# baurst/liso

Hardware: AMD Instinct MI355X
Metric: LISO train-step frames/sec (120k-pt clouds) (higher is better)
Workload: dtype bf16 (detector, BASELINE configs[2]) + f32 via bf16x3 MFMA (SLIM); north_star's 1e-3 on logits / flow is met by `parity_leg` (f32 via bf16x3 MFMA everywhere) and `fp32_exact_leg`, not by the bf16 detector

## Files before the change

include/liso_pillars.h:

```cpp
#ifndef LISO_PILLARS_H
#define LISO_PILLARS_H

#include <stddef.h>
#include <stdint.h>

#ifdef __cplusplus
extern "C" {
#endif

#define LISO_PFN_OUT 64
#define LISO_PILLARS_MAX_BATCH 32
#define LISO_PFN_STATS_DOUBLES 80

typedef struct {
    float x_min, y_min, z_min;
    float vx, vy, vz;
    int gx, gy;
    int max_points;
    int max_voxels;
    int n_channels;
} liso_pillar_cfg;

size_t liso_pillars_voxelize_workspace_bytes(const liso_pillar_cfg* cfg, int batch, int n_total);

int liso_pillars_voxelize_f32(const float* points, const int* offsets_host, int batch, const liso_pillar_cfg* cfg,
                              int* coors, int* num_points, int* slots, int* num_voxels, int* cell_to_voxel,
                              void* workspace, size_t workspace_bytes, void* stream);

size_t liso_pfn_decorate_workspace_bytes(int batch, int max_voxels);
int liso_pfn_decorate_f32(const float* points, const liso_pillar_cfg* cfg, int batch, const int* coors, const int* num_points,
                          const int* slots, const int* num_voxels, int* pt_off, float* feat, int* voxel_cell, void* workspace,
                          size_t workspace_bytes, void* stream);

size_t liso_pfn_partials_bytes(void);
int liso_pfn_bn_prepare_f32(const float* feat, const int* pt_off, const liso_pillar_cfg* cfg, int batch, const int* num_voxels,
                            const float* weight, const float* gamma, const float* beta, float* running_mean,
                            float* running_var, float momentum, float eps, int training, float* bn_out, double* moments,
                            void* partials, void* stream);

int liso_pfn_forward_scatter(const float* feat, const int* pt_off, const int* voxel_cell, const liso_pillar_cfg* cfg, int batch,
                             const int* cell_to_voxel, const float* weight, const float* bn_out, void* canvas, int out_bf16,
                             float* occupancy, void* stream);

int liso_pfn_forward_rows(const float* feat, const int* pt_off, const int* voxel_cell, const liso_pillar_cfg* cfg, int batch,
                          const int* cell_to_voxel, const float* weight, const float* bn_out, void* rows, int out_bf16, int row_base,
                          int* cell_to_row, float* occupancy, void* stream);

int liso_pfn_backward(const float* feat, const int* pt_off, const int* voxel_cell, const liso_pillar_cfg* cfg, int batch,
                      const int* num_voxels, const float* weight, const float* gamma, const float* bn_out,
                      const double* moments, int training, const void* grad_canvas, int grad_bf16, float* grad_weight,
                      float* grad_gamma, float* grad_beta, void* partials, void* stream);

#ifdef __cplusplus
}
#endif
#endif
```

liso_amd/_lib.py:

```python
import ctypes
import os

import torch

_HERE = os.path.dirname(os.path.abspath(__file__))
LIB_PATH = os.path.join(_HERE, "libliso_hip.so")

_lib = None


class LisoHipError(RuntimeError):
    pass


_ERRORS = {-1: "LISO_EINVAL (bad pointer/size)", -2: "LISO_EWORKSPACE (workspace too small)",
           -3: "LISO_ELAUNCH (HIP launch failed)", -4: "LISO_GROUND_ELENGTH (int(67 / delta_R) > 255)"}


def _preload_torch_hip_runtime():
    tl = os.path.join(os.path.dirname(torch.__file__), "lib", "libamdhip64.so")
    if os.path.exists(tl):
        ctypes.CDLL(tl, mode=ctypes.RTLD_GLOBAL)


def lib():
    global _lib
    if _lib is None:
        if not os.path.exists(LIB_PATH):
            raise LisoHipError(
                f"{LIB_PATH} not found: build it with `python -c 'import __graft_entry__ as g; g.build()'` "
                "or `make -C liso_amd/csrc`.  liso_amd has no CPU fallback for device ops.")
        _preload_torch_hip_runtime()
        _lib = ctypes.CDLL(LIB_PATH)
        _declare(_lib)
    return _lib


def check(code, what):
    if code != 0:
        raise LisoHipError(f"{what} failed: {_ERRORS.get(code, code)}")


def stream_ptr(device=None):
    return ctypes.c_void_p(torch.cuda.current_stream(device).cuda_stream)


def ptr(t):
    return ctypes.c_void_p(t.data_ptr())


def multi_copy(pairs):
    import torch

    fast = []
    for d, s_ in pairs:
        if (d.is_cuda and s_.is_cuda and d.device == s_.device and d.dtype == s_.dtype and d.shape == s_.shape and d.is_contiguous()
                and s_.is_contiguous() and (not fast or fast[0][0].device == d.device)):
            if d.numel() and d.data_ptr() != s_.data_ptr():
                fast.append((d, s_))
        else:
            d.copy_(s_, non_blocking=True)
    if len(fast) == 1:
        fast[0][0].copy_(fast[0][1], non_blocking=True)
    elif fast:
        n = len(fast)
        dst = (ctypes.c_void_p * n)(*[d.data_ptr() for d, _ in fast])
        src = (ctypes.c_void_p * n)(*[s_.data_ptr() for _, s_ in fast])
        nb = (ctypes.c_size_t * n)(*[d.numel() * d.element_size() for d, _ in fast])
        with torch.cuda.device(fast[0][0].device):
            check(lib().liso_multi_copy(n, dst, src, nb, stream_ptr()), "multi_copy")


def copy_blocks(jobs):
    import torch

    n = len(jobs)
    if n == 0:
        return
    dst = (ctypes.c_void_p * n)()
    src = (ctypes.c_void_p * n)()
    rows = (ctypes.c_uint * n)()
    rb = (ctypes.c_uint * n)()
    ds = (ctypes.c_size_t * n)()
    ss = (ctypes.c_size_t * n)()

    def rows_view(t):
        assert t.dtype == torch.float32 and t.is_cuda
        if t.dim() == 1:
            assert t.stride(0) == 1 or t.numel() <= 1
            return 1, t.numel(), t.numel()
        inner = 1
        for k in range(t.dim() - 1, 0, -1):
            assert t.shape[k] == 1 or t.stride(k) == inner, (tuple(t.shape), t.stride())
            inner *= t.shape[k]
        return t.shape[0], inner, (t.stride(0) if t.shape[0] > 1 else inner)

    for i, (d, s_) in enumerate(jobs):
        assert tuple(d.shape) == tuple(s_.shape), (tuple(d.shape), tuple(s_.shape))
        r, c, dstr = rows_view(d)
        r2, c2, sstr = rows_view(s_)
        assert (r, c) == (r2, c2)
        dst[i], src[i], rows[i], rb[i], ds[i], ss[i] = d.data_ptr(), s_.data_ptr(), r, 4 * c, 4 * dstr, 4 * sstr
    with torch.cuda.device(jobs[0][0].device):
        check(lib().liso_multi_copy_rows(n, dst, src, rows, rb, ds, ss, stream_ptr()), "multi_copy_rows")


def require_cuda(*tensors):
    for t in tensors:
        if not t.is_cuda:
            raise LisoHipError("device op called with a CPU tensor; liso_amd has no CPU fallback")


_vp, _i, _f, _sz, _lg = ctypes.c_void_p, ctypes.c_int, ctypes.c_float, ctypes.c_size_t, ctypes.c_long
_d = ctypes.c_double

SIGNATURES = {
    "liso_iou3d_overlap_bev_f32": (_i, [_vp, _i, _vp, _i, _vp, _vp]),
    "liso_iou3d_iou_bev_f32": (_i, [_vp, _i, _vp, _i, _vp, _vp]),
    "liso_iou3d_nms_workspace_bytes": (_sz, [_i]),
    "liso_iou3d_nms_f32": (_i, [_vp, _i, _f, _vp, _vp, _vp, _sz, _vp]),
    "liso_iou3d_nms_normal_f32": (_i, [_vp, _i, _f, _vp, _vp, _vp, _sz, _vp]),
    "liso_iou3d_iou_bev_cpu_f32": (_i, [_vp, _i, _vp, _i, _vp]),
    "liso_pillars_voxelize_workspace_bytes": (_sz, [_vp, _i, _i]),
    "liso_pillars_voxelize_f32": (_i, [_vp, _vp, _i, _vp, _vp, _vp, _vp, _vp, _vp, _vp, _sz, _vp]),
    "liso_pfn_partials_bytes": (_sz, []),
    "liso_pfn_decorate_workspace_bytes": (_sz, [_i, _i]),
    "liso_pfn_decorate_f32": (_i, [_vp, _vp, _i, _vp, _vp, _vp, _vp, _vp, _vp, _vp, _vp, _sz, _vp]),
    "liso_pfn_bn_prepare_f32": (_i, [_vp, _vp, _vp, _i, _vp, _vp, _vp, _vp, _vp, _vp, _f, _f, _i, _vp, _vp, _vp, _vp]),
    "liso_pfn_forward_scatter": (_i, [_vp, _vp, _vp, _vp, _i, _vp, _vp, _vp, _vp, _i, _vp, _vp]),
    "liso_pfn_forward_rows": (_i, [_vp, _vp, _vp, _vp, _i, _vp, _vp, _vp, _vp, _i, _i, _vp, _vp, _vp]),
    "liso_pfn_backward": (_i, [_vp, _vp, _vp, _vp, _i, _vp, _vp, _vp, _vp, _vp, _i, _vp, _i, _vp, _vp, _vp, _vp, _vp]),
    "liso_kabsch_workspace_bytes": (_sz, [_vp]),
    "liso_kabsch_trafos_f32": (_i, [_vp, _vp, _vp, _vp, _vp, _vp, _vp, _vp, _vp, _vp, _vp, _sz, _vp]),
    "liso_kabsch_trafos_counted_f32": (_i, [_vp, _vp, _vp, _vp, _vp, _vp, _vp, _vp, _vp, _vp, _vp, _vp, _sz, _vp]),
    "liso_symm_ortho_fwd_f64": (_i, [_vp, _i, _vp, _vp, _vp, _vp, _vp]),
    "liso_symm_ortho_bwd_f64": (_i, [_vp, _vp, _vp, _vp, _i, _vp, _vp]),
    "liso_weighted_moments_workspace_bytes": (_sz, [_i]),
    "liso_weighted_moments_fwd_f32": (_i, [_vp, _vp, _vp, _i, ctypes.c_long, _vp, _vp, _sz, _vp]),
    "liso_weighted_moments_bwd_f32": (_i, [_vp, _vp, _vp, _i, ctypes.c_long, _vp, _vp, _vp, _vp, _vp]),
    "liso_bev_dynamic_flow_workspace_bytes": (_sz, [_i, _i, _i]),
    "liso_bev_dynamic_flow_f32": (_i, [_vp, _i, _vp, _vp, _vp, _i, _vp, _i, _i, _i, _i, _vp, _vp, _vp, _sz, _vp]),
    "liso_odom_inverse_minus_eye_f64": (_i, [_vp, _i, _vp, _vp]),
    "liso_fit_box_z_workspace_bytes": (_sz, [_i, _i]),
    "liso_fit_box_z_f32": (_i, [_vp, _i, _i, _vp, _i, _vp, _i, _vp, _i, _f, _vp, _vp, _vp, _vp, _sz, _vp]),
    "liso_dbscan_components": (_i, [_vp, _vp, _vp, _vp, _vp, _vp, _vp, _vp, _vp]),
    "liso_dbscan_labels": (_i, [_vp, _vp, _vp, _vp, _vp, _vp, _vp, _vp, _vp, _vp]),
    "liso_region_props": (_i, [_vp, _i, _i, _i, _i, _vp, _vp, _vp]),
    "liso_region_props_workspace_bytes": (_sz, [_i, _i, _i, _i]),
    "liso_region_props_ws": (_i, [_vp, _i, _i, _i, _i, _vp, _vp, _vp, _sz, _vp]),
    "liso_corr_lookup_fwd_f32": (_i, [_vp, _vp, _vp, _vp, _vp, _vp]),
    "liso_corr_lookup_fwd_tiled_f32": (_i, [_vp, _vp, _vp, _vp, _vp, _vp]),
    "liso_corr_lookup_bwd_dvol_f32": (_i, [_vp, _vp, _vp, _vp, _vp]),
    "liso_corr_pyramid_fwd_f32": (_i, [_vp, _vp, _vp, _vp]),
    "liso_corr_pyramid_bwd_f32": (_i, [_vp, _vp, _vp, _vp]),
    "liso_corr_bwd_features_workspace_bytes": (_sz, [_vp]),
    "liso_corr_bwd_features_f32": (_i, [_vp, _i, _vp, _vp, _vp, _vp, _vp, _vp, _sz, _vp]),
    "liso_rows_combine_f32": (_i, [_lg, _i, _vp, _lg, _vp, _lg, _vp, _lg, _vp, _lg, _vp, _lg, _i, _vp]),
    "liso_gru_out_rows_train_f32": (_i, [_lg, _i, _vp, _lg, _vp, _vp, _lg, _vp, _lg, _vp]),
    "liso_gru_out_rows_bwd_f32": (_i, [_lg, _i, _vp, _lg, _vp, _vp, _lg, _vp, _lg, _vp, _lg, _vp, _vp, _vp]),
    "liso_gru_in_rows_bwd_f32": (_i, [_lg, _i, _vp, _lg, _vp, _lg, _vp, _vp, _vp, _lg, _vp, _lg, _vp, _vp]),
    "liso_raft_state_step_train_f32": (_i, [_i, _i, _vp, _vp, _vp, _vp, _vp, _vp, _vp, _vp, _vp]),
    "liso_raft_pack_output_grads_f32": (_i, [_lg, _i, _vp, _vp, _vp, _vp]),
    "liso_nearest_point_loss_fwd_f32": (_i, [_vp] * 8),
    "liso_nearest_point_loss_bwd_f32": (_i, [_vp] * 9),
    "liso_slim_decode_weights_fwd": (_i, [_vp] * 6 + [_i] + [_vp] * 4),
    "liso_slim_decode_weights_bwd": (_i, [_vp] * 9),
    "liso_slim_decode_points_fwd": (_i, [_vp] * 9),
    "liso_slim_decode_points_bwd": (_i, [_vp] * 11),
    "liso_slim_loss_workspace_bytes": (_sz, []),
    "liso_slim_static_points_loss_fwd": (_i, [_i, ctypes.c_long, _vp, _i, _vp, _vp, _vp, _vp, _vp, _vp, _sz, _vp]),
    "liso_slim_static_points_loss_bwd": (_i, [_i, ctypes.c_long, _vp, _i, _vp, _vp, _vp, _vp, _vp, _vp, _vp, _vp, _vp]),
    "liso_slim_knn_queries": (_i, [_i, _i, ctypes.c_long, _i, _vp, _i, _vp, _vp, _vp, _vp, _vp]),
    "liso_slim_nearest_point_loss_fwd": (_i, [_vp, _vp, _i, _vp, _vp, _vp, _i, _vp, _vp, _vp, _vp, _vp, _sz, _vp]),
    "liso_slim_nearest_point_loss_bwd": (_i, [_vp, _vp, _i, _vp, _vp, _vp, _i, _vp, _vp, _vp, _vp, _vp, _vp, _vp]),
    "liso_bev_gather_fwd_f32": (_i, [_vp, _vp, ctypes.c_long, _i, ctypes.c_float, _vp, _vp]),
    "liso_bev_gather_bwd_f32": (_i, [_vp, _vp, _vp, _vp, ctypes.c_long, _i, _vp, _vp, _vp]),
    "liso_gru_in_fwd_f32": (_i, [_vp, _vp, _vp, ctypes.c_long, _vp, _vp, _vp, _vp, _vp]),
    "liso_gru_in_bwd_f32": (_i, [_vp, _vp, ctypes.c_long, _vp, _vp, _vp, _vp, _vp, _vp, ctypes.c_long, _vp, _vp]),
    "liso_gru_out_fwd_f32": (_i, [ctypes.c_long, _vp, _vp, _vp, _vp, _vp]),
    "liso_gru_out_bwd_f32": (_i, [ctypes.c_long, _vp, _vp, _vp, _vp, _vp, _vp, _vp, _vp]),
    "liso_gru_in_rows_f32": (_i, [ctypes.c_long, _i, _vp, ctypes.c_long, _vp, ctypes.c_long, _vp, _vp, ctypes.c_long, _vp]),
    "liso_gru_out_rows_f32": (_i, [ctypes.c_long, _i, _vp, ctypes.c_long, _vp, _vp, ctypes.c_long, _vp]),
    "liso_multi_copy": (_i, [_i, _vp, _vp, _vp, _vp]),
    "liso_bev_lin_index": (_i, [_vp, _i, _vp, _i, ctypes.c_long, _i, _i, _vp, _vp]),
    "liso_channel_extrema_workspace_bytes": (_sz, []),
    "liso_channel_extrema_f32": (_i, [_vp, ctypes.c_long, _i, _i, _vp, _vp, _sz, _vp]),
    "liso_bev_plan_tile_lin": (_i, [_vp, _i, ctypes.c_long, _i, _i, _i, _i, _vp, _vp]),
    "liso_bev_plan_rank": (_i, [_vp, _vp, ctypes.c_long, _vp, _vp, _vp]),
    "liso_bev_plan_expand": (_i, [_vp, _vp, _vp, _i, ctypes.c_long, _i, _i, _i, _i, _vp, _vp, _vp, _vp]),
    "liso_raft_state_step_f32": (_i, [_i, _i, _vp, ctypes.c_long, _vp, _vp, _vp, _vp]),
    "liso_raft_upsample_scratch_bytes": (_sz, [_vp]),
    "liso_raft_upsample_outputs_fwd_f32": (_i, [_vp] * 5),
    "liso_raft_upsample_outputs_bwd_f32": (_i, [_vp, _vp, _vp, _sz, _vp, _vp, _vp]),
    "liso_centerloss_workspace_bytes": (_sz, [_vp]),
    "liso_centerloss_fwd_f32": (_i, [_vp] * 17 + [_sz, _vp]),
    "liso_centerloss_bwd_f32": (_i, [_vp] * 21),
    "liso_render_center_targets_f32": (_i, [_vp] * 12),
    "liso_conv_pack_weights_batched": (_i, [_vp, _i, _vp]),
    "liso_conv_pack_weights_placed": (_i, [_vp, _i, _i, _vp]),
    "liso_conv_in_finalize": (_i, [_vp, _i, _i, _i, _i, ctypes.c_long, _vp, _vp, _f, _vp, _vp]),
    "liso_residual_affine_relu_f32": (_i, [_vp, _vp, _vp, _i, _i, _vp, _vp, _vp, _i, _i, _vp, _i, ctypes.c_long, _i, _vp]),
    "liso_scan_workspace_bytes": (_sz, [_i, ctypes.c_long]),
    "liso_scan_inclusive_i32": (_i, [_vp, _i, ctypes.c_long, _vp, _vp, _sz, _vp]),
    "liso_mine_boxes_from_regions": (_i, [_vp, _i, _i, _vp, _i, _vp, _i, _f, _f, _vp, _vp, _vp, _vp, _vp, _vp]),
    "liso_mine_filter_compact": (_i, [_vp] * 21),
    "liso_mine_box_motion": (_i, [_vp, _i, _i, _vp, _vp, _vp, _vp]),
    "liso_mine_nms_workspace_bytes": (_sz, [_i, _i]),
    "liso_mine_nms_prepare": (_i, [_i, _i, _i] + [_vp] * 11 + [_sz, _vp]),
    "liso_mine_nms_finish": (_i, [_i, _i, _i] + [_vp] * 16),
    "liso_adamw_step_f32": (_i, [_vp, _vp, _vp, _vp, _sz] + [ctypes.c_double] * 5 + [ctypes.c_long, _vp]),
    "liso_adamw_step_scaled_f32": (_i, [_vp, _vp, _vp, _vp, _sz] + [ctypes.c_double] * 6 + [ctypes.c_long, _vp]),
    "liso_adamw_pack_table_plan": (_i, [_vp, _i, _sz, _vp, _vp]),
    "liso_adamw_pack_table_fill": (_i, [_vp, _i, _sz, _vp, _sz]),
    "liso_adamw_step_packed_f32": (_i, [_vp, _vp, _vp, _vp, _sz] + [ctypes.c_double] * 6 + [ctypes.c_long, _vp, _i, _vp]),
    "liso_grad_nonfinite_f32": (_i, [_vp, _sz, _vp, _vp]),
    "liso_adamw_step_amp_f32": (_i, [_vp, _vp, _vp, _vp, _sz] + [ctypes.c_double] * 6 + [_vp, _vp]),
    "liso_loss_scale_update": (_i, [_vp, ctypes.c_double, ctypes.c_double, _i, _vp]),
    "liso_rmsprop_step_f32": (_i, [_vp, _vp, _vp, _sz] + [ctypes.c_double] * 4 + [_vp]),
    "liso_multi_copy_rows": (_i, [_i, _vp, _vp, _vp, _vp, _vp, _vp, _vp]),
    "liso_gather_f32": (_i, [_i, _vp, _vp, _vp, _vp]),
    "liso_bn_workspace_bytes": (_sz, [_i]),
    "liso_bn_relu_fwd": (_i, [_vp, _i, ctypes.c_long, _i, _vp, _vp, _vp, _vp, _f, _f, _i, _i, _vp, _vp, _vp, _sz, _vp]),
    "liso_in_workspace_bytes": (_sz, [_i, _i]),
    "liso_in_relu_fwd": (_i, [_vp, _i, _i, ctypes.c_long, _i, _vp, _vp, _f, _i, _vp, _vp, _vp, _sz, _vp]),
    "liso_in_relu_bwd": (_i, [_vp, _vp, _i, _i, ctypes.c_long, _i, _vp, _vp, _i, _vp, _vp, _vp, _vp, _sz, _vp]),
    "liso_in_relu_bwd_sum": (_i, [_vp, _vp, _i, _i, ctypes.c_long, _i, _vp, _vp, _i, _vp, _vp, _vp, _vp, _sz, _vp]),
    "liso_bn_relu_bwd": (_i, [_vp, _vp, _i, ctypes.c_long, _i, _vp, _vp, _i, _i, _vp, _vp, _vp, _vp, _sz, _vp]),
    "liso_bn_relu_bwd_strided": (_i, [_vp, ctypes.c_long, _vp, ctypes.c_long, _i, ctypes.c_long, _i, _vp, _vp, _i, _i, _vp, ctypes.c_long, _vp, _vp, _vp, _sz, _vp]),
    "liso_bn_relu_bwd_chained": (_i, [_vp, ctypes.c_long, _vp, ctypes.c_long, _i, ctypes.c_long, _i, _vp, _vp, _i, _i, _vp, ctypes.c_long, _vp, _vp, _vp, _sz, _vp, _vp]),
    "liso_bn_multi_workspace_bytes": (_sz, [_vp, _i, _i]),
    "liso_bn_relu_bwd_multi": (_i, [_vp, ctypes.c_long, _vp, ctypes.c_long, _vp, ctypes.c_long, _i, ctypes.c_long, _vp, _i, _i, _i, _vp, ctypes.c_long,
                                    _vp, _sz, _vp, _vp, _vp]),
    "liso_bn_relu_bwd_multi_check": (_i, [_vp, _i, _i, _i, ctypes.c_long, ctypes.c_long, ctypes.c_long, ctypes.c_long, ctypes.c_long, _vp]),
    "liso_knn_workspace_bytes": (_sz, [_vp, _i]),
    "liso_knn_build_f32": (_i, [_vp, _vp, _i, _i, _vp, _sz, _vp]),
    "liso_knn_sorted_ids": (_i, [_vp, _vp, _i, _vp, _vp]),
    "liso_knn_query_f32": (_i, [_vp, _vp, _vp, _vp, _i, _vp, _i, _i, _vp, _vp, _i, _vp]),
    "liso_conv_packed_bytes": (_sz, [_i, _i, _i, _i]),
    "liso_conv_pack_weights": (_i, [_vp, _i, _i, _i, _i, _i, _i, _i, _vp, _vp]),
    "liso_conv_stats_rows": (_i, [_vp]),
    "liso_conv_kernel_kind": (_i, [_vp]),
    "liso_conv_forward": (_i, [_vp] * 10),
    "liso_conv_set_option": (_i, [_i, _i]),
    "liso_conv_forward_sparse": (_i, [_vp] * 11),
    "liso_conv_plan_info": (_i, [_vp, _vp]),
    "liso_conv_wgrad_workspace_bytes": (_sz, [_vp]),
    "liso_conv_wgrad": (_i, [_vp, _vp, _vp, _vp, _vp, _i, _i, _vp, _vp, _vp, _sz, _vp]),
    "liso_conv_wgrad_deferred": (_i, [_vp, _vp, _vp, _vp, _vp, _i, _i, _vp, _vp, _vp, _sz, _vp, _vp]),
    "liso_conv_wgrad_reduce": (_i, [_vp, _vp]),
    "liso_conv_wgrad_sparse_workspace_bytes": (_sz, [_vp]),
    "liso_conv_wgrad_sparse_f32": (_i, [_vp, _vp, _vp, _vp, _i, _vp, _vp, _vp, _sz, _vp]),
    "liso_conv_wgrad_smallci_workspace_bytes": (_sz, [_i, _i, _i, _i, _i]),
    "liso_conv_wgrad_smallci_f32": (_i, [_vp, ctypes.c_long, _vp, ctypes.c_long, _i, _i, _i, _i, _i, _vp, _vp, _vp, _sz, _vp]),
    "liso_sparse_conv_stat_groups": (_i, [_i, _i, _i]),
    "liso_sparse_conv_workspace_bytes": (_sz, [_i, _i, _i, _i, _i, _i, _i]),
    "liso_sparse_conv_forward": (_i, [_vp, ctypes.c_long, _i, _vp, _vp, _vp, _i, _i, _i, _i, _i, _i, _i, _vp, _vp, _vp, _vp, _vp, _sz, _vp]),
    "liso_sparse_conv_forward_rows": (_i, [_vp, ctypes.c_long, _i, _vp, ctypes.c_long, _vp, _vp, _vp, _i, _i, _i, _i, _i, _i, _i, _vp, _vp, _vp, _vp, _vp,
                                           _sz, _vp]),
    "liso_sparse_conv_dgrad": (_i, [_vp, ctypes.c_long, _i, _vp, _vp, _i, _i, _i, _i, _i, _i, _vp, ctypes.c_long, _vp, _vp, _sz, _i, _vp]),
    "liso_sparse_stem_workspace_bytes": (_sz, [_i, _i, _i, _i]),
    "liso_sparse_stem_forward_f32": (_i, [_vp, ctypes.c_long, _vp, _vp, _vp, _i, _i, _i, _i, _i, _vp, _vp, _vp, _vp, _sz, _vp]),
    "liso_conv_bn_finalize": (_i, [_vp, _i, _i, _i, ctypes.c_long, _vp, _vp, _vp, _vp, _vp, _f, _f, _vp, _vp]),
    "liso_conv_bn_finalize_merged": (_i, [_vp, _i, _i, _i, ctypes.c_long, _vp, _vp, _vp, _vp, _vp, _f, _f, _vp, _vp, _vp, _i, _i, _vp]),
    "liso_points_in_boxes_workspace_bytes": (_sz, [_vp]),
    "liso_points_in_boxes_f32": (_i, [_vp] * 9 + [_sz, _vp]),
    "liso_match_greedy_f32": (_i, [_vp, ctypes.c_long, ctypes.c_long, _i, _i, _vp, _f, _vp, _vp, _vp, _vp, _vp, _vp, _vp]),
    "liso_fit_boxes_closeness_workspace_bytes": (_sz, [ctypes.c_long, _i]),
    "liso_fit_boxes_closeness_f32": (_i, [_vp, ctypes.c_long, _i, _vp, _vp, _i, _f, _vp, _vp, _vp, _sz, _vp]),
    "liso_bike_rollout_fwd_f32": (_i, [_i, _i, _vp, _vp, _vp, _vp, _f, _f, _f, _vp, _vp]),
    "liso_bike_rollout_bwd_f32": (_i, [_i, _i, _vp, _vp, _vp, _f, _f, _f, _vp, _vp, _vp, _vp, _vp, _vp]),
    "liso_smooth_tracks_jerk_f32": (_i, [_vp, _vp, _i, _i, _i, _f, _f, _vp, _vp]),
    "liso_flow_metrics_state_bytes": (_sz, []),
    "liso_flow_metrics_result_bytes": (_sz, []),
    "liso_flow_metrics_reset": (_i, [_vp, _vp]),
    "liso_flow_metrics_update": (_i, [_vp, _lg, _vp, _lg, _vp, _lg, _i, _vp, _lg, _vp, _lg, _vp, _lg, _vp, _vp, _vp, _vp, _i, _vp, _vp]),
    "liso_flow_metrics_read": (_i, [_vp, _vp, _vp]),
    "liso_det_nms_workspace_bytes": (_sz, [_i, _i]),
    "liso_det_nms_order": (_i, [_i, _i, _vp, _vp, _vp, _f, _vp, _vp, _vp, _sz, _vp]),
    "liso_det_nms_select": (_i, [_i, _i, _vp, _vp, _vp, _f, _i, _i, _vp, _vp, _vp]),
    "liso_det_nms_gather": (_i, [_i, _i, _i, _vp, _vp, _vp, _i, _vp]),
    "liso_ground_jcp_workspace_bytes": (_sz, [_vp]),
    "liso_ground_jcp_f32": (_i, [_vp, _vp, _vp, _vp, _vp, _sz, _vp]),
    "liso_ground_jcp_stages_f32": (_i, [_vp, _vp, _vp, _vp, _vp, _sz, _i, _i, _vp]),
    "liso_ground_cone_f32": (_i, [_i, _i, _i, _vp, _vp, ctypes.c_double, ctypes.c_double, _vp, _vp, _vp]),
    "liso_ground_compact_workspace_bytes": (_sz, [_i, _i]),
    "liso_ground_compact_f32": (_i, [_i, _i, _i, _vp, _vp, _vp, _vp, _vp, _vp, _sz, _vp]),
    "liso_bev_free_mask_workspace_bytes": (_sz, [_i, _i]),
    "liso_bev_free_mask": (_i, [_vp, ctypes.c_long, _i, _i, _i, _vp, _vp, _vp, _sz, _vp]),
    "liso_bev_select_free_cells": (_i, [_vp, _vp, _i, _i, _vp, _i, _vp, _vp]),
    "liso_snippet_paste": (_i, [_vp, ctypes.c_long, _vp, _vp, _vp, _vp, ctypes.c_double, ctypes.c_double, _i, _vp, _vp, _vp, _vp]),
    "liso_sample_transform_f32": (_i, [_i, _i, _i] + [_vp] * 7),
    "liso_sample_transform_poses_f64": (_i, [_i, _vp, _vp, _i, _vp, _i, _vp]),
    "liso_bev_crop_workspace_bytes": (_sz, [_i, _i]),
    "liso_bev_crop_f32": (_i, [_vp] * 14 + [_sz, _vp]),
    "liso_bev_point_maps_workspace_bytes": (_sz, [_i, _i, _i, _i]),
    "liso_bev_point_maps_f32": (_i, [_i] * 5 + [_vp] * 6 + [ctypes.c_double] + [_vp] * 5 + [_sz, _vp]),
    "liso_box_has_points_f32": (_i, [_i] * 4 + [_vp] * 7),
    "liso_filter_boxes": (_i, [_vp] * 6 + [_i] + [_vp] * 3),
    "liso_object_velocity_f64": (_i, [_i, _i] + [_vp] * 5),
    "liso_ignore_region_mask": (_i, [_i] * 4 + [ctypes.c_double] * 2 + [_vp] * 6),
    "liso_render_center_targets_ex_f32": (_i, [_vp] * 15),
    "liso_snippet_cut_workspace_bytes": (_sz, [_i, _i, _i]),
    "liso_snippet_cut_f32": (_i, [_i, _i, _i, _vp, _vp, _vp, _i, _vp, _vp, _lg] + [_vp] * 5 + [_sz, _vp]),
    "liso_track_sequences_workspace_bytes": (_sz, [_i, _i, _i, _i]),
    "liso_track_sequences": (_i, [_i] * 4 + [_vp] * 7 + [ctypes.c_double] + [_vp] * 10 + [_sz, _vp]),
    "liso_track_mining_workspace_bytes": (_sz, [_i] * 5),
    "liso_select_tracks": (_i, [_i] * 5 + [_vp] * 7 + [_i, _f, _d, _d, _i, _d, _d, _i, _d] + [_vp] * 13 + [_vp, _sz, _vp]),
    "liso_refine_tracks_apply": (_i, [_i] * 3 + [_vp] * 12 + [_i, _i, _d] + [_vp] * 7 + [_vp]),
    "liso_export_tracks": (_i, [_i] * 6 + [_vp] * 11 + [_i] + [_vp] * 13 + [_vp, _sz, _vp]),
    "liso_frame_prep_workspace_bytes": (_sz, [_vp]),
    "liso_prepare_tracker_frames": (_i, [_vp] * 27 + [_sz, _vp]),
}


CONV_MAX_TAPS, CONV_MAX_CLASSES, CONV_BF16, CONV_F32X3, CONV_F32, CONV_F16 = 49, 4, 0, 1, 2, 3
ELEM_F32, ELEM_BF16, ELEM_F16 = 0, 1, 2
_ELEM_CODES = {torch.float32: ELEM_F32, torch.bfloat16: ELEM_BF16, torch.float16: ELEM_F16}
LOSS_SCALE_STATE_BYTES = 32


def elem_code(dtype):
    code = _ELEM_CODES.get(dtype)
    if code is None:
        raise TypeError(f"no device kernel takes {dtype} tensors (float32, bfloat16 or float16)")
    return code


def is_half(dtype):
    return elem_code(dtype) != ELEM_F32


def lane_channels(dtype):
    return 8 if is_half(dtype) else 4
CONV_OPT_SHARED_GPU = 1
CONV_OPT_ROLES_CUS = 2


class ConvDesc(ctypes.Structure):
    _fields_ = [("batch", _i), ("hi", _i), ("wi", _i), ("ci", _i), ("x_pix_stride", _i), ("ho", _i), ("wo", _i), ("co", _i),
                ("y_pix_stride", _i), ("y_ch_off", _i), ("hv", _i), ("wv", _i), ("isy", _i), ("isx", _i), ("osy", _i), ("osx", _i),
                ("n_classes", _i), ("class_tap_begin", _i * (CONV_MAX_CLASSES + 1)), ("class_ooy", _i * CONV_MAX_CLASSES),
                ("class_oox", _i * CONV_MAX_CLASSES), ("n_taps", _i), ("tap_dy", _i * CONV_MAX_TAPS), ("tap_dx", _i * CONV_MAX_TAPS),
                ("tap_w", _i * CONV_MAX_TAPS), ("w_taps", _i), ("mode", _i), ("out_f32", _i), ("in_relu", _i), ("out_relu", _i),
                ("in_affine_batch_stride", _i), ("wgrad_co", _i)]


class ConvPackPlacedJob(ctypes.Structure):
    _fields_ = [("src", _vp), ("dst", _vp), ("d0", _i), ("d1", _i), ("kh", _i), ("kw", _i), ("transposed", _i), ("for_dgrad", _i),
                ("mode", _i), ("K", _i), ("N", _i), ("k_offset", _i), ("n_offset", _i)]


class AdamwPackDest(ctypes.Structure):
    _fields_ = [("dst", _vp), ("for_dgrad", _i), ("mode", _i), ("K", _i), ("N", _i), ("k_offset", _i), ("n_offset", _i)]


class AdamwPackItem(ctypes.Structure):
    _fields_ = [("offset", _sz), ("d0", _i), ("d1", _i), ("kh", _i), ("kw", _i), ("transposed", _i), ("n_dest", _i),
                ("dest", AdamwPackDest * 2), ("mirror", _vp), ("mirror_row_stride", _sz)]


class ConvPackJob(ctypes.Structure):
    _fields_ = [("src", _vp), ("dst", _vp), ("d0", _i), ("d1", _i), ("kh", _i), ("kw", _i), ("transposed", _i), ("for_dgrad", _i),
                ("mode", _i)]


class WgradReduceJob(ctypes.Structure):
    _fields_ = [("slab", _vp), ("bias_slab", _vp), ("dw", _vp), ("dbias", _vp), ("cip", ctypes.c_long), ("cop", ctypes.c_long),
                ("splits", _i), ("bias_rows", _i), ("taps", _i), ("ci", _i), ("co", _i), ("transposed", _i)]


BN_MAX_GROUPS = 4


class BnGroup(ctypes.Structure):
    _fields_ = [("c_off", _i), ("c", _i), ("gamma", _vp), ("stats", _vp), ("grad_gamma", _vp), ("grad_beta", _vp)]


class KnnGrid(ctypes.Structure):
    _fields_ = [("x_min", _f), ("y_min", _f), ("cell", _f), ("nx", _i), ("ny", _i), ("z_min", _f), ("z_cell", _f), ("nz", _i)]


class CenterLossCfg(ctypes.Structure):
    _fields_ = [("batch", _i), ("h", _i), ("w", _i), ("res_x", _f), ("res_y", _f), ("z_min", _f), ("z_max", _f),
                ("sup_weight", _f), ("rot_reg_weight", _f)]


class NpLossCfg(ctypes.Structure):
    _fields_ = [("batch", _i), ("n", ctypes.c_long), ("n_b", ctypes.c_long), ("ext", _f * 4), ("fov_mode", _i), ("delta", _f)]


class SlimDecodeCfg(ctypes.Structure):
    _fields_ = [("samples", _i), ("n", ctypes.c_long), ("h", _i), ("w", _i), ("logit_mode", _i * 4), ("static_flow_zero", _i),
                ("dynamic_flow_zero", _i), ("overwrite_flow", _i), ("overwrite_logits", _i), ("non_rigid", _i), ("use_static_aggr", _i),
                ("dyn_grad_scale", _f), ("ext_lo", ctypes.c_double * 2), ("ext_span", ctypes.c_double * 2)]


class SlimDecodeOut(ctypes.Structure):
    FIELDS = ("dis_logit", "dis", "logits", "probs", "staticness", "dynamicness", "groundness", "dyn_flow", "stat_flow", "agg_flow", "saf_flow")
    _fields_ = [(k, _vp) for k in FIELDS] + [("flags", _vp)]


class SlimNpLossCfg(ctypes.Structure):
    _fields_ = [("samples", _i), ("clouds", _i), ("n", ctypes.c_long), ("n_b", ctypes.c_long), ("ext", _f * 4), ("fov_mode", _i), ("delta", _f)]


class BoxPtsCfg(ctypes.Structure):
    _fields_ = [("batch", _i), ("n", ctypes.c_long), ("k", _i), ("point_stride", _i), ("precision", _i), ("dims_bloat", _f)]


class FramePrepCfg(ctypes.Structure):
    _fields_ = [("n_seq", _i), ("max_frames", _i), ("max_box", _i), ("cap", _i), ("n_points", ctypes.c_long), ("point_stride", _i),
                ("n_fov_points", ctypes.c_long), ("fov_stride", _i), ("bev_range_x", _f), ("bev_range_y", _f), ("drop_on_bev_boundaries", _i),
                ("min_points_in_box", _i), ("fov_min_points", _i), ("align", _i), ("no_align_below_m", _d), ("full_align_above_m", _d)]


class GruCfg(ctypes.Structure):
    _fields_ = [("batch", _i), ("ch", _i), ("cx", _i), ("hw", ctypes.c_long)]


class UpsampleCfg(ctypes.Structure):
    _fields_ = [("n_it", _i), ("batch2", _i), ("dirs", _i), ("h", _i), ("w", _i), ("factor", _i), ("flow_scale", _f)]


class MineFilterCfg(ctypes.Structure):
    _fields_ = [("batch", _i), ("k", _i), ("min_points", _i), ("aspect_ratio_max", ctypes.c_double), ("max_box_len_m", ctypes.c_double),
                ("min_box_area_m2", ctypes.c_double), ("min_box_volume_m3", ctypes.c_double), ("park_invalid", _i)]


class DetGatherField(ctypes.Structure):
    _fields_ = [("src", _vp), ("dst", _vp), ("row_elems", _i), ("elem_bytes", _i), ("pad_bits", ctypes.c_uint64)]


class GroundCfg(ctypes.Structure):
    _fields_ = [("batch", _i), ("n_max", _i), ("point_stride", _i), ("width", _i), ("height", _i),
# ... 93 lines not shown
```

liso_amd/csrc/pillars.hip:

```cpp
#include <hip/hip_runtime.h>
#include <stdlib.h>
#include "zero_fill.h"
#include <cstring>
#include <hip/hip_bf16.h>
#include <limits.h>
#include <stdint.h>

#include "../../include/liso_iou3d.h"
#include "../../include/liso_conv.h"
#include "../../include/liso_pillars.h"
#include "dev_common.h"

namespace {

using liso_dev::check_launch;

constexpr int kTile = 1024;
constexpr int kOut = LISO_PFN_OUT;
constexpr int kFP = 12;
constexpr int kMaxPts = 32;
constexpr int kPfnThreads = 256;
constexpr int kPfnGrid = 1024;

struct BatchInfo {
// ... 97 lines not shown
            coors[v * 4 + 1] = 0;
            coors[v * 4 + 2] = within / cfg.gy;
            coors[v * 4 + 3] = within % cfg.gy;
            const int c = count[cell];
            num_points[v] = c < cfg.max_points ? c : cfg.max_points;
        }
    }
    if (tile == bi.tile_off[b + 1] - 1 && threadIdx.x == 0) {
        int tot = base_s;
        for (int w = 0; w < kTile / 64; w++) tot += wsum[w];
        num_voxels[b] = tot < cfg.max_voxels ? tot : cfg.max_voxels;
    }
}

constexpr int kScanTile = 1024;
__global__ __launch_bounds__(kScanTile) void cell_scan_block_kernel(const int* __restrict__ count, size_t cells, int* __restrict__ seg_off,
                                                                    int* __restrict__ block_tot) {
    __shared__ int wsum[kScanTile / 64];
    const size_t i = (size_t)blockIdx.x * kScanTile + threadIdx.x;
    const int lane = threadIdx.x & 63, wave = threadIdx.x >> 6;
    const int v = i < cells ? count[i] : 0;
    int incl = v;
#pragma unroll
    for (int o = 1; o < 64; o <<= 1) {
        const int t = __shfl_up(incl, o);
        if (lane >= o) incl += t;
    }
    if (lane == 63) wsum[wave] = incl;
    __syncthreads();
    int base = 0;
    for (int w = 0; w < wave; w++) base += wsum[w];
    if (i < cells) seg_off[i] = base + incl - v;
    if (threadIdx.x == kScanTile - 1) block_tot[blockIdx.x] = base + incl;
}

__global__ __launch_bounds__(1024) void cell_scan_tot_kernel(int* __restrict__ block_tot, int nblk) {
    __shared__ int wsum[16];
    const int t = threadIdx.x, lane = t & 63, wave = t >> 6;
    int v[4], tot = 0;
#pragma unroll
    for (int k = 0; k < 4; k++) {
        const int q = t * 4 + k;
        v[k] = q < nblk ? block_tot[q] : 0;
        tot += v[k];
    }
    int incl = tot;
#pragma unroll
    for (int o = 1; o < 64; o <<= 1) {
        const int up = __shfl_up(incl, o);
        if (lane >= o) incl += up;
    }
    if (lane == 63) wsum[wave] = incl;
    __syncthreads();
    int base = 0;
    for (int w = 0; w < wave; w++) base += wsum[w];
    int run = base + incl - tot;
#pragma unroll
    for (int k = 0; k < 4; k++) {
        const int q = t * 4 + k;
        if (q < nblk) block_tot[q] = run;
        run += v[k];
    }
}

__global__ __launch_bounds__(256) void seg_fill_kernel(const int* __restrict__ cell_of_point, int n_total, const int* __restrict__ seg_off,
                                                       const int* __restrict__ block_tot, const int* __restrict__ pos_in_cell,
                                                       int* __restrict__ seg) {
    const int i = blockIdx.x * blockDim.x + threadIdx.x;
    if (i >= n_total) return;
    const int c = cell_of_point[i];
    if (c < 0) return;
    seg[seg_off[c] + block_tot[c / kScanTile] + pos_in_cell[i]] = i;
}

constexpr int kSlotRegs = 16;
__device__ __forceinline__ void voxel_slots_one(const int* __restrict__ coors, const int* __restrict__ num_voxels, int max_voxels, int gx, int gy,
                                                const int* __restrict__ seg_off, const int* __restrict__ block_tot,
                                                const int* __restrict__ count, const int* __restrict__ seg, int max_points,
                                                int* __restrict__ slots, long v, int lane) {
    const int b = (int)(v / max_voxels), ord = (int)(v % max_voxels);
    if (ord >= num_voxels[b]) return;
    const int c = (b * gx + coors[v * 4 + 2]) * gy + coors[v * 4 + 3];
    const int off = seg_off[c] + block_tot[c / kScanTile], n = count[c];
    int* out = slots + (size_t)v * max_points;
    if (n <= 64) {
        const int e = lane < n ? seg[off + lane] : 0x7fffffff;
        int r = 0;
        for (int k = 0; k < n; k++) r += __shfl(e, k) < e ? 1 : 0;
        if (lane < n && r < max_points) out[r] = e;
        return;
    }
    int last = -1;
    const int rounds = min(max_points, n);
    if (n <= 64 * kSlotRegs) {
        int x[kSlotRegs];
#pragma unroll
        for (int u = 0; u < kSlotRegs; u++) x[u] = lane + 64 * u < n ? seg[off + lane + 64 * u] : 0x7fffffff;
        for (int r = 0; r < rounds; r++) {
            int m = 0x7fffffff;
#pragma unroll
            for (int u = 0; u < kSlotRegs; u++) m = (x[u] > last && x[u] < m) ? x[u] : m;
#pragma unroll
            for (int o = 32; o > 0; o >>= 1) m = min(m, __shfl_xor(m, o));
            if (lane == 0) out[r] = m;
            last = m;
        }
        return;
    }
    for (int r = 0; r < rounds; r++) {
        int m = 0x7fffffff;
        for (int j = lane; j < n; j += 64) {
            const int x = seg[off + j];
            m = (x > last && x < m) ? x : m;
        }
#pragma unroll
        for (int o = 32; o > 0; o >>= 1) m = min(m, __shfl_xor(m, o));
        if (lane == 0) out[r] = m;
        last = m;
    }
}

__global__ __launch_bounds__(256) void voxel_slots_kernel(const int* __restrict__ coors, const int* __restrict__ num_voxels, int max_voxels,
                                                          int batch, int gx, int gy, const int* __restrict__ seg_off,
                                                          const int* __restrict__ block_tot, const int* __restrict__ count,
                                                          const int* __restrict__ seg, int max_points, int* __restrict__ slots) {
    const int lane = threadIdx.x & 63;
    for (long v = (long)blockIdx.x * 4 + (threadIdx.x >> 6); v < (long)batch * max_voxels; v += (long)gridDim.x * 4)
        voxel_slots_one(coors, num_voxels, max_voxels, gx, gy, seg_off, block_tot, count, seg, max_points, slots, v, lane);
}

struct PfnGeom {
    float vx, vy, x_off, y_off, z_off;
};

__device__ __forceinline__ PfnGeom pfn_geom(const liso_pillar_cfg& c) {
    PfnGeom g;
    g.vx = c.vx; g.vy = c.vy;
    g.x_off = c.vx / 2 + c.x_min;
    g.y_off = c.vy / 2 + c.y_min;
    g.z_off = c.vz / 2 + c.z_min;
    return g;
}

constexpr int kGroup = 4;
constexpr int kStage = kGroup * kMaxPts;

__device__ __forceinline__ int kept_points(const int* __restrict__ num_points, const int* __restrict__ num_voxels, int max_voxels,
                                           int rows, int v) {
    if (v >= rows) return 0;
    const int b = v / max_voxels;
    return (v - b * max_voxels) < num_voxels[b] ? num_points[v] : 0;
}

__global__ __launch_bounds__(1024) void pfn_scan_block_kernel(const int* __restrict__ num_points, const int* __restrict__ num_voxels,
                                                              int max_voxels, int rows, int* __restrict__ pt_off,
                                                              int* __restrict__ block_tot) {
    __shared__ int wsum[16];
    const int i = blockIdx.x * 1024 + threadIdx.x;
    const int lane = threadIdx.x & 63, wave = threadIdx.x >> 6;
    const int v = kept_points(num_points, num_voxels, max_voxels, rows, i);
    int incl = v;
    for (int off = 1; off < 64; off <<= 1) {
        const int t = __shfl_up(incl, off);
        if (lane >= off) incl += t;
    }
    if (lane == 63) wsum[wave] = incl;
    __syncthreads();
    int base = 0;
    for (int w = 0; w < wave; w++) base += wsum[w];
    if (i < rows) pt_off[i] = base + incl - v;
    if (threadIdx.x == 1023) block_tot[blockIdx.x] = base + incl;
}

__global__ __launch_bounds__(1024) void pfn_scan_tot_kernel(int* __restrict__ block_tot, int nblocks) {
    __shared__ int wsum[16];
    const int lane = threadIdx.x & 63, wave = threadIdx.x >> 6;
    const int v = (int)threadIdx.x < nblocks ? block_tot[threadIdx.x] : 0;
    int incl = v;
    for (int off = 1; off < 64; off <<= 1) {
        const int t = __shfl_up(incl, off);
        if (lane >= off) incl += t;
    }
    if (lane == 63) wsum[wave] = incl;
    __syncthreads();
    int base = 0;
    for (int w = 0; w < wave; w++) base += wsum[w];
    if ((int)threadIdx.x < nblocks) block_tot[threadIdx.x] = base + incl - v;
    if ((int)threadIdx.x == nblocks - 1) block_tot[nblocks] = base + incl;
}

__global__ __launch_bounds__(1024) void pfn_scan_add_kernel(int* __restrict__ pt_off, int rows, const int* __restrict__ block_tot,
                                                            int nblocks) {
    const int i = blockIdx.x * 1024 + threadIdx.x;
    if (i < rows) pt_off[i] += block_tot[blockIdx.x];
    if (i == 0) pt_off[rows] = block_tot[nblocks];
}

template <int C>
__global__ __launch_bounds__(256) void pfn_decorate_kernel(const float* __restrict__ pts, liso_pillar_cfg cfg, int rows,
                                                           const int* __restrict__ coors, const int* __restrict__ num_points,
                                                           const int* __restrict__ slots, const int* __restrict__ num_voxels,
                                                           const int* __restrict__ pt_off, float* __restrict__ feat,
                                                           int* __restrict__ voxel_cell) {
#pragma clang fp contract(off)
    constexpr int F = C + 6;
    const long t = (long)blockIdx.x * blockDim.x + threadIdx.x;
    const int v = (int)(t >> 5), s = (int)(t & 31);
    if (v >= rows) return;
    const int num = kept_points(num_points, num_voxels, cfg.max_voxels, rows, v);
    const int xi = coors[v * 4 + 2], yi = coors[v * 4 + 3];
    if (s == 0) voxel_cell[v] = num > 0 ? ((v / cfg.max_voxels) * cfg.gx + xi) * cfg.gy + yi : -1;
    float p[C];
#pragma unroll
    for (int k = 0; k < C; k++) p[k] = 0.f;
    if (s < num) {
        const int idx = slots[(size_t)v * cfg.max_points + s];
        const float* q = pts + (size_t)idx * C;
        if constexpr (C == 4) {
            const float4 tt = *reinterpret_cast<const float4*>(q);
            p[0] = tt.x; p[1] = tt.y; p[2] = tt.z; p[3] = tt.w;
        } else {
#pragma unroll
            for (int k = 0; k < C; k++) p[k] = q[k];
        }
    }
    float sx = p[0], sy = p[1], sz = p[2];
#pragma unroll
    for (int o = 16; o > 0; o >>= 1) {
        sx += __shfl_xor(sx, o);
        sy += __shfl_xor(sy, o);
        sz += __shfl_xor(sz, o);
    }
    if (s >= num) return;
    const PfnGeom g = pfn_geom(cfg);
    const float fn = (float)num;
    const float mx = sx / fn, my = sy / fn, mz = sz / fn;
    const float fcx = p[0] - ((float)yi * g.vx + g.x_off);
    const float fcy = p[1] - ((float)xi * g.vy + g.y_off);
    const float fcz = p[2] - (0.f + g.z_off);
    float f[kFP];
#pragma unroll
    for (int k = 0; k < kFP; k++) f[k] = 0.f;
    f[0] = fcx; f[1] = fcy; f[2] = fcz;
#pragma unroll
    for (int k = 3; k < C; k++) f[k] = p[k];
    f[C + 0] = p[0] - mx; f[C + 1] = p[1] - my; f[C + 2] = p[2] - mz;
    f[C + 3] = fcx; f[C + 4] = fcy; f[C + 5] = fcz;
    f[F] = 1.f;
    float4* row = reinterpret_cast<float4*>(feat + ((size_t)pt_off[v] + s) * kFP);
    row[0] = make_float4(f[0], f[1], f[2], f[3]);
    row[1] = make_float4(f[4], f[5], f[6], f[7]);
    row[2] = make_float4(f[8], f[9], f[10], f[11]);
}

template <int C>
__global__ __launch_bounds__(kPfnThreads) void pfn_stats_kernel(const float* __restrict__ feat, const int* __restrict__ pt_off,
                                                                int rows, double* __restrict__ partials) {
    constexpr int F = C + 6, D = F + 1, NP = D * (D + 1) / 2;
    __shared__ __attribute__((aligned(16))) float tile[kPfnThreads / 64][64][kFP];
    __shared__ double red[kPfnThreads / 64][LISO_PFN_STATS_DOUBLES];
    const int lane = threadIdx.x & 63, wave = threadIdx.x >> 6;
    int pj[2] = {0, 0}, pk[2] = {0, 0};
    {
        int idx = 0;
        for (int j = 0; j < D; j++)
            for (int k = j; k < D; k++, idx++) {
                if (idx == lane) { pj[0] = j; pk[0] = k; }
                if (idx == lane + 64) { pj[1] = j; pk[1] = k; }
            }
    }
    const long n = pt_off[rows];
    const long waves = (long)gridDim.x * (kPfnThreads / 64);
    const long per = ((n + waves - 1) / waves + 63) / 64 * 64;
    const long w_id = (long)blockIdx.x * (kPfnThreads / 64) + wave;
    const long r0 = w_id * per, r1 = r0 + per < n ? r0 + per : n;
    double acc0 = 0.0, acc1 = 0.0;
    for (long base = r0; base < r1; base += 64) {
        const int cnt = (int)(r1 - base < 64 ? r1 - base : 64);
        const float4* src = reinterpret_cast<const float4*>(feat + (size_t)base * kFP);
        float4* dst = reinterpret_cast<float4*>(&tile[wave][0][0]);
        for (int i = lane; i < cnt * 3; i += 64) dst[i] = src[i];
        __builtin_amdgcn_wave_barrier();
        for (int s = 0; s < cnt; s++) {
            const float* f = tile[wave][s];
            acc0 += (double)f[pj[0]] * (double)f[pk[0]];
            if (lane + 64 < NP) acc1 += (double)f[pj[1]] * (double)f[pk[1]];
        }
        __builtin_amdgcn_wave_barrier();
    }
    red[wave][lane] = acc0;
    if (lane + 64 < LISO_PFN_STATS_DOUBLES) red[wave][lane + 64] = lane + 64 < NP ? acc1 : 0.0;
    __syncthreads();
    if (threadIdx.x < LISO_PFN_STATS_DOUBLES) {
        double s = 0.0;
        for (int w = 0; w < kPfnThreads / 64; w++) s += red[w][threadIdx.x];
        partials[(size_t)blockIdx.x * LISO_PFN_STATS_DOUBLES + threadIdx.x] = threadIdx.x < NP ? s : 0.0;
    }
}

__device__ __forceinline__ int pair_index(int j, int k, int D) {
    return j * D - j * (j - 1) / 2 + (k - j);
}

template <int C>
__global__ __launch_bounds__(1024) void pfn_bn_finalize_kernel(const double* __restrict__ partials, int nblocks,
                                                               const int* __restrict__ num_voxels, int batch,
                                                               int max_points, const float* __restrict__ weight,
                                                               const float* __restrict__ gamma,
                                                               const float* __restrict__ beta,
                                                               float* __restrict__ running_mean,
                                                               float* __restrict__ running_var, float momentum,
                                                               float eps, float* __restrict__ bn_out,
                                                               double* __restrict__ moments) {
    constexpr int F = C + 6, D = F + 1;
    constexpr int NS = LISO_PFN_STATS_DOUBLES, CH = 1024 / NS;
    __shared__ double part[CH][NS];
    __shared__ double mom[NS];
    const int e = threadIdx.x % NS, chunk = threadIdx.x / NS;
    if (chunk < CH) {
        double s = 0.0;
        const int per = (nblocks + CH - 1) / CH;
        const int lo = chunk * per, hi = lo + per < nblocks ? lo + per : nblocks;
        int blk = lo;
        for (; blk + 16 <= hi; blk += 16) {
            double v[16];
#pragma unroll
            for (int j = 0; j < 16; j++) v[j] = partials[(size_t)(blk + j) * NS + e];
#pragma unroll
            for (int j = 0; j < 16; j++) s += v[j];
        }
        for (; blk < hi; blk++) s += partials[(size_t)blk * NS + e];
        part[chunk][e] = s;
    }
    __syncthreads();
    if (threadIdx.x < NS) {
        double t = 0.0;
        for (int c = 0; c < CH; c++) t += part[c][threadIdx.x];
        mom[threadIdx.x] = t;
        moments[threadIdx.x] = t;
    }
    __syncthreads();
    __shared__ double rows_sq[kOut][F + 1], rows_sum[kOut][F + 1];
    if (threadIdx.x < kOut * F) {
        const int c = threadIdx.x / F, j = threadIdx.x % F;
        const double wj = (double)weight[c * F + j];
        double q = 0.0;
        for (int k = 0; k < F; k++) {
            const int a = j <= k ? j : k, bb = j <= k ? k : j;
            q += wj * (double)weight[c * F + k] * mom[pair_index(a, bb, D)];
        }
        rows_sq[c][j] = q;
        rows_sum[c][j] = wj * mom[pair_index(j, D - 1, D)];
    }
    __syncthreads();
    if (threadIdx.x < kOut) {
        const int c = threadIdx.x;
        long long P = 0;
        for (int b = 0; b < batch; b++) P += num_voxels[b];
        const double M = (double)P * (double)max_points;
        double sum = 0.0, sq = 0.0;
        for (int j = 0; j < F; j++) {
            sum += rows_sum[c][j];
            sq += rows_sq[c][j];
        }
        double mean = 0.0, var = 0.0;
        if (M > 0.0) {
            mean = sum / M;
            var = sq / M - mean * mean;
            if (var < 0.0) var = 0.0;
        }
        const double invstd = 1.0 / sqrt(var + (double)eps);
        const float scale = (float)((double)gamma[c] * invstd);
        bn_out[c] = scale;
        bn_out[kOut + c] = (float)((double)beta[c] - mean * (double)gamma[c] * invstd);
        bn_out[2 * kOut + c] = (float)mean;
        bn_out[3 * kOut + c] = (float)invstd;
        if (M > 1.0) {
            const double mo = (double)momentum;
            running_mean[c] = (float)((1.0 - mo) * (double)running_mean[c] + mo * mean);
            running_var[c] = (float)((1.0 - mo) * (double)running_var[c] + mo * (var * M / (M - 1.0)));
        }
    }
}

__global__ void pfn_bn_eval_kernel(const float* __restrict__ gamma, const float* __restrict__ beta,
                                   const float* __restrict__ running_mean, const float* __restrict__ running_var,
                                   float eps, float* __restrict__ bn_out) {
    const int c = threadIdx.x;
    if (c >= kOut) return;
    const float invstd = 1.f / sqrtf(running_var[c] + eps);
    bn_out[c] = gamma[c] * invstd;
    bn_out[kOut + c] = beta[c] - running_mean[c] * gamma[c] * invstd;
    bn_out[2 * kOut + c] = running_mean[c];
    bn_out[3 * kOut + c] = invstd;
}

template <typename T> __device__ __forceinline__ void store_out(T* p, float v);
template <> __device__ __forceinline__ void store_out<float>(float* p, float v) { *p = v; }
template <> __device__ __forceinline__ void store_out<__hip_bfloat16>(__hip_bfloat16* p, float v) { *p = __float2bfloat16(v); }
template <typename T> __device__ __forceinline__ float load_in(const T* p);
template <> __device__ __forceinline__ float load_in<float>(const float* p) { return *p; }
template <> __device__ __forceinline__ float load_in<__hip_bfloat16>(const __hip_bfloat16* p) { return __bfloat162float(*p); }
template <> __device__ __forceinline__ void store_out<_Float16>(_Float16* p, float v) { *p = (_Float16)v; }
template <> __device__ __forceinline__ float load_in<_Float16>(const _Float16* p) { return (float)*p; }

__device__ __forceinline__ void stage_rows(const float* __restrict__ feat, const int* __restrict__ pt_off, int rows, int v0, int lane,
                                           float (*frow)[kFP], int (&off)[kGroup + 1]) {
    int o = 0;
    if (lane <= kGroup) { const int v = v0 + lane; o = pt_off[v < rows ? v : rows]; }
#pragma unroll
    for (int g = 0; g <= kGroup; g++) off[g] = __shfl(o, g);
    const int total = off[kGroup] - off[0];
    const float4* src = reinterpret_cast<const float4*>(feat + (size_t)off[0] * kFP);
    float4* dst = reinterpret_cast<float4*>(&frow[0][0]);
    for (int i = lane; i < total * 3; i += 64) dst[i] = src[i];
}

constexpr int kCellsPerBlock = 256;

template <int C, typename OutT, bool ROWS>
__global__ __launch_bounds__(kPfnThreads) void pfn_forward_kernel(const float* __restrict__ feat, const int* __restrict__ pt_off,
                                                                  const int* __restrict__ voxel_cell, int rows, int max_points,
                                                                  long total_cells, int zero_blocks,
                                                                  const int* __restrict__ cell_to_voxel,
                                                                  const float* __restrict__ weight, const float* __restrict__ bn,
                                                                  OutT* __restrict__ canvas, float* __restrict__ occupancy,
                                                                  int* __restrict__ map_out, int row_base) {
    constexpr int F = C + 6;
    constexpr int kChunks = kOut * (int)sizeof(OutT) / 16;
    __shared__ __attribute__((aligned(16))) float frow[kPfnThreads / 64][kStage][kFP];
    __shared__ int vox[kCellsPerBlock];
    const int tid = threadIdx.x, lane = tid & 63, wave = tid >> 6;
    const int pillar_blocks = (int)gridDim.x - zero_blocks;
    if ((int)blockIdx.x >= pillar_blocks) {
        const long cell0 = (long)((int)blockIdx.x - pillar_blocks) * kCellsPerBlock;
        const long cell = cell0 + tid;
        int v1 = 0;
        if (cell < total_cells) {
            v1 = cell_to_voxel[cell];
            occupancy[cell] = v1 > 0 ? 1.f : 0.f;
            if constexpr (ROWS) map_out[cell] = v1 > 0 ? v1 + row_base : 0;
        }
        if constexpr (ROWS) return;
        vox[tid] = v1;
        __syncthreads();
        const uint4 z = make_uint4(0u, 0u, 0u, 0u);
        uint4* base = reinterpret_cast<uint4*>(canvas + (size_t)cell0 * kOut);
        for (int id = tid; id < kCellsPerBlock * kChunks; id += kPfnThreads) {
            const int cl = id / kChunks;
            if (cell0 + cl < total_cells && vox[cl] == 0) base[id] = z;
        }
        return;
    }
    float w[F];
#pragma unroll
    for (int k = 0; k < F; k++) w[k] = weight[lane * F + k];
    const float scale = bn[lane], shift = bn[kOut + lane];
    const float pad_val = fmaxf(shift, 0.f);
    const int wave_id = (int)blockIdx.x * (kPfnThreads / 64) + wave;
    const int n_waves = pillar_blocks * (kPfnThreads / 64);
    for (int v0 = wave_id * kGroup; v0 < rows; v0 += n_waves * kGroup) {
        int off[kGroup + 1];
        stage_rows(feat, pt_off, rows, v0, lane, frow[wave], off);
        int cell_l = -1;
        if (lane < kGroup && v0 + lane < rows) cell_l = voxel_cell[v0 + lane];
        __builtin_amdgcn_wave_barrier();
#pragma unroll
        for (int g = 0; g < kGroup; g++) {
            const int num = off[g + 1] - off[g];
            const int cell = __shfl(cell_l, g);
            if (num <= 0 || cell < 0) continue;
            float best = num < max_points ? pad_val : 0.f;
            const int r0 = off[g] - off[0];
            for (int s = 0; s < num; s++) {
                const float4* f4 = reinterpret_cast<const float4*>(frow[wave][r0 + s]);
                const float4 a = f4[0], b = f4[1], c4 = f4[2];
                const float f[kFP] = {a.x, a.y, a.z, a.w, b.x, b.y, b.z, b.w, c4.x, c4.y, c4.z, c4.w};
                float x = 0.f;
#pragma unroll
                for (int k = 0; k < F; k++) x = fmaf(w[k], f[k], x);
                best = fmaxf(best, fmaxf(fmaf(x, scale, shift), 0.f));
            }
            store_out<OutT>(canvas + (size_t)(ROWS ? v0 + g : cell) * kOut + lane, best);
        }
        __builtin_amdgcn_wave_barrier();
    }
}

template <int C, typename GT>
__global__ __launch_bounds__(kPfnThreads) void pfn_backward_kernel(const float* __restrict__ feat, const int* __restrict__ pt_off,
                                                                   const int* __restrict__ voxel_cell, int rows, int max_points,
                                                                   const float* __restrict__ weight, const float* __restrict__ bn,
                                                                   const GT* __restrict__ grad_canvas,
                                                                   float* __restrict__ partials) {
    constexpr int F = C + 6, NA = F + 2;
    __shared__ __attribute__((aligned(16))) float frow[kPfnThreads / 64][kStage][kFP];
    __shared__ float red[kPfnThreads / 64][NA][kOut];
    const int lane = threadIdx.x & 63, wave = threadIdx.x >> 6;
    float w[F], acc[NA];
#pragma unroll
    for (int k = 0; k < F; k++) w[k] = weight[lane * F + k];
#pragma unroll
    for (int k = 0; k < NA; k++) acc[k] = 0.f;
    const float scale = bn[lane], shift = bn[kOut + lane], mean = bn[2 * kOut + lane], invstd = bn[3 * kOut + lane];
    const float pad_val = fmaxf(shift, 0.f);
    const int wave_id = (int)blockIdx.x * (kPfnThreads / 64) + wave;
    const int n_waves = (int)gridDim.x * (kPfnThreads / 64);
    for (int v0 = wave_id * kGroup; v0 < rows; v0 += n_waves * kGroup) {
        int off[kGroup + 1];
        stage_rows(feat, pt_off, rows, v0, lane, frow[wave], off);
        int cell_l = -1;
        if (lane < kGroup && v0 + lane < rows) cell_l = voxel_cell[v0 + lane];
        __builtin_amdgcn_wave_barrier();
#pragma unroll
        for (int g = 0; g < kGroup; g++) {
            const int num = off[g + 1] - off[g];
            const int cell = __shfl(cell_l, g);
            if (num <= 0 || cell < 0) continue;
            const int r0 = off[g] - off[0];
            float best = -1.f, best_x = 0.f;
            int best_s = -1;
            for (int s = 0; s < num; s++) {
                const float* f = frow[wave][r0 + s];
                float x = 0.f;
#pragma unroll
                for (int k = 0; k < F; k++) x = fmaf(w[k], f[k], x);
                const float y = fmaxf(fmaf(x, scale, shift), 0.f);
                if (y > best) { best = y; best_s = s; best_x = x; }
            }
            if (num < max_points && pad_val > best) { best = pad_val; best_s = -1; best_x = 0.f; }
            const float gy = load_in<GT>(grad_canvas + (size_t)cell * kOut + lane);
            const float dz = best > 0.f ? gy : 0.f;
            if (best_s >= 0) {
                const float* f = frow[wave][r0 + best_s];
#pragma unroll
                for (int k = 0; k < F; k++) acc[k] = fmaf(dz, f[k], acc[k]);
            }
            acc[F] += dz;
            acc[F + 1] = fmaf(dz, (best_x - mean) * invstd, acc[F + 1]);
        }
        __builtin_amdgcn_wave_barrier();
    }
#pragma unroll
    for (int k = 0; k < NA; k++) red[wave][k][lane] = acc[k];
    __syncthreads();
    for (int idx = threadIdx.x; idx < NA * kOut; idx += kPfnThreads) {
        const int k = idx / kOut, c = idx % kOut;
        float s = 0.f;
        for (int wv = 0; wv < kPfnThreads / 64; wv++) s += red[wv][k][c];
        partials[((size_t)blockIdx.x * NA + k) * kOut + c] = s;
    }
}

template <int NA>
__global__ __launch_bounds__(1024) void pfn_backward_reduce_kernel(const float* __restrict__ partials, int nblocks,
                                                                   double* __restrict__ tot) {
    __shared__ double part[16][kOut];
    const int k = blockIdx.x, c = threadIdx.x & 63, chunk = threadIdx.x >> 6;
    const int per = (nblocks + 15) / 16;
    const int lo = chunk * per, hi = lo + per < nblocks ? lo + per : nblocks;
    double s = 0.0;
    {
        int blk = lo;
        for (; blk + 8 <= hi; blk += 8) {
            float v[8];
#pragma unroll
            for (int j = 0; j < 8; j++) v[j] = partials[((size_t)(blk + j) * NA + k) * kOut + c];
#pragma unroll
            for (int j = 0; j < 8; j++) s += (double)v[j];
        }
        for (; blk < hi; blk++) s += (double)partials[((size_t)blk * NA + k) * kOut + c];
    }
    part[chunk][c] = s;
    __syncthreads();
    if (chunk == 0) {
        double t = 0.0;
        for (int q = 0; q < 16; q++) t += part[q][c];
        tot[k * kOut + c] = t;
    }
}

template <int C>
__global__ __launch_bounds__(64) void pfn_backward_finalize_kernel(const double* __restrict__ tot,
                                                                   const int* __restrict__ num_voxels, int batch,
                                                                   int max_points, const float* __restrict__ weight,
                                                                   const float* __restrict__ gamma,
                                                                   const float* __restrict__ bn,
                                                                   const double* __restrict__ moments, int training,
                                                                   float* __restrict__ grad_weight,
                                                                   float* __restrict__ grad_gamma,
                                                                   float* __restrict__ grad_beta) {
    constexpr int F = C + 6, D = F + 1;
    const int c = threadIdx.x;
    if (c >= kOut) return;
    const double dbeta = tot[F * kOut + c], dgamma = tot[(F + 1) * kOut + c];
    grad_beta[c] = (float)dbeta;
    grad_gamma[c] = (float)dgamma;
    const double invstd = (double)bn[3 * kOut + c], mean = (double)bn[2 * kOut + c];
    const double gi = (double)gamma[c] * invstd;
    if (!training) {
        for (int k = 0; k < F; k++) grad_weight[c * F + k] = (float)(gi * tot[k * kOut + c]);
        return;
    }
    long long P = 0;
    for (int b = 0; b < batch; b++) P += num_voxels[b];
    const double M = (double)P * (double)max_points;
    double w[F];
    for (int k = 0; k < F; k++) w[k] = (double)weight[c * F + k];
    for (int k = 0; k < F; k++) {
        const double Fk = moments[pair_index(k, D - 1, D)];
        double xf = 0.0;
        for (int j = 0; j < F; j++) {
            const int a = j <= k ? j : k, bb = j <= k ? k : j;
            xf += w[j] * moments[pair_index(a, bb, D)];
        }
        const double xhat_f = invstd * (xf - mean * Fk);
        const double dw = M > 0.0 ? gi * (tot[k * kOut + c] - dbeta / M * Fk - dgamma / M * xhat_f) : 0.0;
        grad_weight[c * F + k] = (float)dw;
    }
}

inline bool cfg_ok(const liso_pillar_cfg* c, int batch) {
    return c && batch >= 1 && batch <= LISO_PILLARS_MAX_BATCH && c->gx > 0 && c->gy > 0 && c->max_points >= 1 &&
           c->max_points <= kMaxPts && c->max_voxels >= 1 && c->n_channels >= 3 && c->n_channels <= 5;
}

inline BatchInfo make_batch(const int* off, int batch) {
    BatchInfo bi;
    bi.tile_off[0] = 0;
    for (int b = 0; b <= LISO_PILLARS_MAX_BATCH; b++) bi.off[b] = off[b <= batch ? b : batch];
    for (int b = 0; b < LISO_PILLARS_MAX_BATCH; b++) {
        const int n = b < batch ? off[b + 1] - off[b] : 0;
        bi.tile_off[b + 1] = bi.tile_off[b] + (n + kTile - 1) / kTile;
    }
    return bi;
}

inline int pfn_grid(int rows) {
    const int need = (rows + kPfnThreads / 64 - 1) / (kPfnThreads / 64);
    return need < kPfnGrid ? (need > 0 ? need : 1) : kPfnGrid;
}

}

extern "C" {

size_t liso_pillars_voxelize_workspace_bytes(const liso_pillar_cfg* cfg, int batch, int n_total) {
    if (!cfg_ok(cfg, batch) || n_total < 0) return 0;
    const size_t cells = (size_t)batch * cfg->gx * cfg->gy;
    const size_t tiles = (size_t)(n_total + kTile - 1) / kTile + batch;
    if (cells > (size_t)4096 * kScanTile) return 0;
    return (3 * cells + 3 * (size_t)n_total + tiles + 64 + 4096) * sizeof(int) + 256;
}

int liso_pillars_voxelize_f32(const float* points, const int* offsets_host, int batch, const liso_pillar_cfg* cfg,
                              int* coors, int* num_points, int* slots, int* num_voxels, int* cell_to_voxel,
                              void* workspace, size_t workspace_bytes, void* stream) {
    if (!cfg_ok(cfg, batch) || !offsets_host) return LISO_EINVAL;
    const int n_total = offsets_host[batch];
    if (n_total < 0 || offsets_host[0] != 0) return LISO_EINVAL;
    for (int b = 0; b < batch; b++)
        if (offsets_host[b + 1] < offsets_host[b]) return LISO_EINVAL;
    if (!coors || !num_points || !slots || !num_voxels || !cell_to_voxel || !workspace || (n_total > 0 && !points))
        return LISO_EINVAL;
    if ((size_t)batch * cfg->gx * cfg->gy > (size_t)4096 * kScanTile) return LISO_EINVAL;
    if (workspace_bytes < liso_pillars_voxelize_workspace_bytes(cfg, batch, n_total)) return LISO_EWORKSPACE;
    hipStream_t st = (hipStream_t)stream;
    const size_t cells = (size_t)batch * cfg->gx * cfg->gy;
    int* count = (int*)workspace;
    int* first_enc = count + cells;
    int* cell_of_point = first_enc + cells;
    int* tile_count = cell_of_point + n_total;
    const size_t tiles_cap = (size_t)(n_total + kTile - 1) / kTile + batch;
    int* seg_off = tile_count + tiles_cap + 32;
    int* pos_in_cell = seg_off + cells;
    int* seg = pos_in_cell + n_total;
    int* block_tot = seg + n_total;
    const BatchInfo bi = make_batch(offsets_host, batch);
    const int tiles = bi.tile_off[batch];
    if (liso_zero::zero_async(count, 2 * cells * sizeof(int), st) != hipSuccess) return LISO_ELAUNCH;
    if (liso_zero::zero_async(cell_to_voxel, cells * sizeof(int), st) != hipSuccess) return LISO_ELAUNCH;
    if (liso_zero::zero_async(num_voxels, batch * sizeof(int), st) != hipSuccess) return LISO_ELAUNCH;
    if (n_total == 0) return LISO_OK;
    const int nb = (n_total + 255) / 256;
    hipLaunchKernelGGL(assign_kernel, dim3(nb), dim3(256), 0, st, points, n_total, cfg->n_channels, bi, batch, *cfg,
                       cell_of_point, count, first_enc, pos_in_cell);
    hipLaunchKernelGGL(tile_count_kernel, dim3(tiles), dim3(kTile), 0, st, cell_of_point, first_enc, bi, batch,
                       tile_count);
    hipLaunchKernelGGL(rank_kernel, dim3(tiles), dim3(kTile), 0, st, cell_of_point, first_enc, count, bi, batch, *cfg,
                       tile_count, coors, num_points, cell_to_voxel, num_voxels);
    const int scan_blocks = (int)((cells + kScanTile - 1) / kScanTile);
    cell_scan_block_kernel<<<scan_blocks, kScanTile, 0, st>>>(count, cells, seg_off, block_tot);
    cell_scan_tot_kernel<<<1, 1024, 0, st>>>(block_tot, scan_blocks);
    seg_fill_kernel<<<nb, 256, 0, st>>>(cell_of_point, n_total, seg_off, block_tot, pos_in_cell, seg);
    const long n_wave = (long)batch * cfg->max_voxels;
    voxel_slots_kernel<<<(unsigned)((n_wave + 3) / 4), 256, 0, st>>>(coors, num_voxels, cfg->max_voxels, batch, cfg->gx, cfg->gy, seg_off,
                                                                   block_tot, count, seg, cfg->max_points, slots);
    return check_launch();
}

size_t liso_pfn_partials_bytes(void) {
    const size_t stats = (size_t)kPfnGrid * LISO_PFN_STATS_DOUBLES * sizeof(double);
    const size_t bwd = (size_t)kPfnGrid * (11 + 2) * kOut * sizeof(float) + (11 + 2) * kOut * sizeof(double);
    return stats > bwd ? stats : bwd;
}

size_t liso_pfn_decorate_workspace_bytes(int batch, int max_voxels) {
    if (batch < 1 || max_voxels < 1) return 0;
    return ((size_t)(batch * (long)max_voxels + 1023) / 1024 + 2) * sizeof(int);
}

int liso_pfn_decorate_f32(const float* points, const liso_pillar_cfg* cfg, int batch, const int* coors, const int* num_points,
                          const int* slots, const int* num_voxels, int* pt_off, float* feat, int* voxel_cell, void* workspace,
                          size_t workspace_bytes, void* stream) {
    if (!cfg_ok(cfg, batch) || !coors || !num_points || !slots || !num_voxels || !pt_off || !feat || !voxel_cell || !workspace)
        return LISO_EINVAL;
    if (workspace_bytes < liso_pfn_decorate_workspace_bytes(batch, cfg->max_voxels)) return LISO_EWORKSPACE;
    const int rows = batch * cfg->max_voxels;
    const int nsb = (rows + 1023) / 1024;
    if (nsb > 1024) return LISO_EINVAL;
    hipStream_t st = (hipStream_t)stream;
    int* block_tot = (int*)workspace;
    pfn_scan_block_kernel<<<nsb, 1024, 0, st>>>(num_points, num_voxels, cfg->max_voxels, rows, pt_off, block_tot);
    pfn_scan_tot_kernel<<<1, 1024, 0, st>>>(block_tot, nsb);
    pfn_scan_add_kernel<<<nsb, 1024, 0, st>>>(pt_off, rows, block_tot, nsb);
    const unsigned grid = (unsigned)(((long)rows * 32 + 255) / 256);
    switch (cfg->n_channels) {
        case 3: pfn_decorate_kernel<3><<<grid, 256, 0, st>>>(points, *cfg, rows, coors, num_points, slots, num_voxels, pt_off, feat, voxel_cell); break;
        case 4: pfn_decorate_kernel<4><<<grid, 256, 0, st>>>(points, *cfg, rows, coors, num_points, slots, num_voxels, pt_off, feat, voxel_cell); break;
        default: pfn_decorate_kernel<5><<<grid, 256, 0, st>>>(points, *cfg, rows, coors, num_points, slots, num_voxels, pt_off, feat, voxel_cell); break;
    }
    return check_launch();
}

int liso_pfn_bn_prepare_f32(const float* feat, const int* pt_off, const liso_pillar_cfg* cfg, int batch, const int* num_voxels,
                            const float* weight, const float* gamma, const float* beta, float* running_mean,
                            float* running_var, float momentum, float eps, int training, float* bn_out, double* moments,
                            void* partials, void* stream) {
    if (!cfg_ok(cfg, batch) || !gamma || !beta || !running_mean || !running_var || !bn_out) return LISO_EINVAL;
    hipStream_t st = (hipStream_t)stream;
    if (!training) {
        pfn_bn_eval_kernel<<<1, 64, 0, st>>>(gamma, beta, running_mean, running_var, eps, bn_out);
        return check_launch();
    }
    if (!feat || !pt_off || !num_voxels || !weight || !moments || !partials) return LISO_EINVAL;
    const int rows = batch * cfg->max_voxels;
    const int grid = kPfnGrid;
#define LISO_PREP(CC)                                                                                                     \
    do {                                                                                                                  \
        pfn_stats_kernel<CC><<<grid, kPfnThreads, 0, st>>>(feat, pt_off, rows, (double*)partials);                           \
        pfn_bn_finalize_kernel<CC><<<1, 1024, 0, st>>>((const double*)partials, grid, num_voxels, batch, cfg->max_points,    \
                                                      weight, gamma, beta, running_mean, running_var, momentum, eps, bn_out, \
                                                      moments);                                                           \
    } while (0)
    switch (cfg->n_channels) {
        case 3: LISO_PREP(3); break;
        case 4: LISO_PREP(4); break;
        default: LISO_PREP(5); break;
    }
#undef LISO_PREP
    return check_launch();
}

static int pfn_forward_launch(const float* feat, const int* pt_off, const int* voxel_cell, const liso_pillar_cfg* cfg, int batch,
                              const int* cell_to_voxel, const float* weight, const float* bn_out, void* canvas, int out_bf16,
                              float* occupancy, int* map_out, int row_base, bool compact, void* stream) {
    if (!cfg_ok(cfg, batch) || !feat || !pt_off || !voxel_cell || !cell_to_voxel || !weight || !bn_out || !canvas || !occupancy)
        return LISO_EINVAL;
    if (out_bf16 != LISO_ELEM_F32 && out_bf16 != LISO_ELEM_BF16 && out_bf16 != LISO_ELEM_F16) return LISO_EINVAL;
    hipStream_t st = (hipStream_t)stream;
    const long cells = (long)batch * cfg->gx * cfg->gy;
    const int rows = batch * cfg->max_voxels;
    const int zero_blocks = (int)((cells + kCellsPerBlock - 1) / kCellsPerBlock);
    const int groups = (rows + kGroup - 1) / kGroup;
    int pfn_blocks = (groups + kPfnThreads / 64 - 1) / (kPfnThreads / 64);
    if (pfn_blocks > 4096) pfn_blocks = 4096;
    const unsigned grid = (unsigned)(zero_blocks + pfn_blocks);
#define LISO_FWD_(CC, T, R) pfn_forward_kernel<CC, T, R><<<grid, kPfnThreads, 0, st>>>(feat, pt_off, voxel_cell, rows, cfg->max_points, cells, zero_blocks, cell_to_voxel, weight, bn_out, (T*)canvas, occupancy, map_out, row_base)
#define LISO_FWD(CC, T) do { if (compact) LISO_FWD_(CC, T, true); else LISO_FWD_(CC, T, false); } while (0)
    switch (cfg->n_channels * 3 + out_bf16) {
        case 9: LISO_FWD(3, float); break;
        case 10: LISO_FWD(3, __hip_bfloat16); break;
        case 11: LISO_FWD(3, _Float16); break;
        case 12: LISO_FWD(4, float); break;
        case 13: LISO_FWD(4, __hip_bfloat16); break;
        case 14: LISO_FWD(4, _Float16); break;
        case 15: LISO_FWD(5, float); break;
        case 16: LISO_FWD(5, __hip_bfloat16); break;
        default: LISO_FWD(5, _Float16); break;
    }
#undef LISO_FWD
#undef LISO_FWD_
    return check_launch();
}

int liso_pfn_forward_scatter(const float* feat, const int* pt_off, const int* voxel_cell, const liso_pillar_cfg* cfg, int batch,
                             const int* cell_to_voxel, const float* weight, const float* bn_out, void* canvas, int out_bf16,
                             float* occupancy, void* stream) {
    return pfn_forward_launch(feat, pt_off, voxel_cell, cfg, batch, cell_to_voxel, weight, bn_out, canvas, out_bf16, occupancy, nullptr,
                              0, false, stream);
}

int liso_pfn_forward_rows(const float* feat, const int* pt_off, const int* voxel_cell, const liso_pillar_cfg* cfg, int batch,
                          const int* cell_to_voxel, const float* weight, const float* bn_out, void* rows, int out_bf16, int row_base,
                          int* cell_to_row, float* occupancy, void* stream) {
    if (!cell_to_row || row_base < 0 || (long)row_base + (long)batch * (cfg ? cfg->max_voxels : 0) >= (1L << 31)) return LISO_EINVAL;
    return pfn_forward_launch(feat, pt_off, voxel_cell, cfg, batch, cell_to_voxel, weight, bn_out, rows, out_bf16, occupancy, cell_to_row,
                              row_base, true, stream);
}

int liso_pfn_backward(const float* feat, const int* pt_off, const int* voxel_cell, const liso_pillar_cfg* cfg, int batch,
                      const int* num_voxels, const float* weight, const float* gamma, const float* bn_out,
                      const double* moments, int training, const void* grad_canvas, int grad_bf16, float* grad_weight,
                      float* grad_gamma, float* grad_beta, void* partials, void* stream) {
    if (!cfg_ok(cfg, batch) || !feat || !pt_off || !voxel_cell || !num_voxels || !weight || !gamma || !bn_out || !grad_canvas ||
        !grad_weight || !grad_gamma || !grad_beta || !partials || (training && !moments))
        return LISO_EINVAL;
    if (grad_bf16 != LISO_ELEM_F32 && grad_bf16 != LISO_ELEM_BF16 && grad_bf16 != LISO_ELEM_F16) return LISO_EINVAL;
    hipStream_t st = (hipStream_t)stream;
    const int rows = batch * cfg->max_voxels;
    const int grid = pfn_grid((rows + kGroup - 1) / kGroup);
#define LISO_BWD(CC, T)                                                                                              \
    do {                                                                                                             \
        constexpr int NA_ = CC + 8;                                                                                  \
        double* tot_ = (double*)((float*)partials + (size_t)kPfnGrid * (11 + 2) * kOut);                             \
        pfn_backward_kernel<CC, T><<<grid, kPfnThreads, 0, st>>>(feat, pt_off, voxel_cell, rows, cfg->max_points,     \
                                                                 weight, bn_out, (const T*)grad_canvas,             \
                                                                 (float*)partials);                                  \
        pfn_backward_reduce_kernel<NA_><<<NA_, 1024, 0, st>>>((const float*)partials, grid, tot_);                    \
        pfn_backward_finalize_kernel<CC><<<1, 64, 0, st>>>(tot_, num_voxels, batch, cfg->max_points, weight, gamma,   \
                                                           bn_out, moments, training, grad_weight, grad_gamma,       \
                                                           grad_beta);                                               \
    } while (0)
    switch (cfg->n_channels * 3 + grad_bf16) {
        case 9: LISO_BWD(3, float); break;
        case 10: LISO_BWD(3, __hip_bfloat16); break;
        case 11: LISO_BWD(3, _Float16); break;
        case 12: LISO_BWD(4, float); break;
        case 13: LISO_BWD(4, __hip_bfloat16); break;
        case 14: LISO_BWD(4, _Float16); break;
        case 15: LISO_BWD(5, float); break;
        case 16: LISO_BWD(5, __hip_bfloat16); break;
        default: LISO_BWD(5, _Float16); break;
    }
#undef LISO_BWD
    return check_launch();
}

}
```

liso_amd/networks/pcl_to_feature_grid/pcl_to_feature_grid.py:

```python
import ctypes

import numpy as np
import torch
from torch import nn

from liso_amd import _lib as L


class PFNLayer(nn.Module):

    def __init__(self, in_channels, out_channels, norm_cfg):
        super().__init__()
        self.units = out_channels
        self.norm = nn.BatchNorm1d(out_channels, eps=norm_cfg["eps"], momentum=norm_cfg["momentum"])
        self.linear = nn.Linear(in_channels, out_channels, bias=False)


class PillarFeatureNet(nn.Module):

    def __init__(self, in_channels, feat_channels, voxel_size, point_cloud_range, norm_cfg):
        super().__init__()
        assert len(feat_channels) == 1, "the LISO call site uses a single PFN layer (pcl_to_feature_grid.py:41-48)"
        self.in_channels = in_channels + 6
        self.pfn_layers = nn.ModuleList([PFNLayer(self.in_channels, feat_channels[0], norm_cfg)])
        self.voxel_size = voxel_size
        self.point_cloud_range = point_cloud_range


def voxelize_raw(points, offsets, pcfg):
    L.require_cuda(points)
    lib = L.lib()
    dev = points.device
    B = len(offsets) - 1
    n_total = int(offsets[-1])
    rows = B * pcfg.max_voxels
    i32 = dict(dtype=torch.int32, device=dev)
    coors = torch.empty((rows, 4), **i32)
    num_points = torch.empty((rows,), **i32)
    slots = torch.empty((rows, pcfg.max_points), **i32)
    num_voxels = torch.empty((B,), **i32)
    cell_to_voxel = torch.empty((B * pcfg.gx * pcfg.gy,), **i32)
    ws_bytes = lib.liso_pillars_voxelize_workspace_bytes(ctypes.byref(pcfg), B, n_total)
    ws = torch.empty(ws_bytes, dtype=torch.uint8, device=dev)
    off = (ctypes.c_int * (B + 1))(*[int(o) for o in offsets])
    with torch.cuda.device(dev):
        L.check(lib.liso_pillars_voxelize_f32(L.ptr(points), off, B, ctypes.byref(pcfg), L.ptr(coors),
                                              L.ptr(num_points), L.ptr(slots), L.ptr(num_voxels),
                                              L.ptr(cell_to_voxel), L.ptr(ws), ws_bytes, L.stream_ptr()),
                "pillars_voxelize")
    return coors, num_points, slots, num_voxels, cell_to_voxel


def decorate_rows(points, pcfg, B, coors, num_points, slots, num_voxels):
    lib = L.lib()
    dev = points.device
    rows = B * pcfg.max_voxels
    pt_off = torch.empty(rows + 1, dtype=torch.int32, device=dev)
    feat = torch.empty((max(points.shape[0], 1), 12), dtype=torch.float32, device=dev)
    voxel_cell = torch.empty(rows, dtype=torch.int32, device=dev)
    nbytes = lib.liso_pfn_decorate_workspace_bytes(B, pcfg.max_voxels)
    ws = torch.empty(nbytes, dtype=torch.uint8, device=dev)
    with torch.cuda.device(dev):
        L.check(L.TIMER.launch("pfn_decorate", lambda: lib.liso_pfn_decorate_f32(
            L.ptr(points), ctypes.byref(pcfg), B, L.ptr(coors), L.ptr(num_points), L.ptr(slots), L.ptr(num_voxels), L.ptr(pt_off),
            L.ptr(feat), L.ptr(voxel_cell), L.ptr(ws), nbytes, L.stream_ptr()), units=points.shape[0] * (points.shape[1] * 4 + 48)), "pfn_decorate")
    return pt_off, feat, voxel_cell


def pillar_prep(points, offsets, pcfg):
    B = len(offsets) - 1
    coors, num_points, slots, num_voxels, cell_to_voxel = voxelize_raw(points, offsets, pcfg)
    pt_off, feat, voxel_cell = decorate_rows(points, pcfg, B, coors, num_points, slots, num_voxels)
    return pt_off, feat, voxel_cell, num_voxels, cell_to_voxel


def _pfn_statistics(weight, gamma, beta, running_mean, running_var, points, offsets, pcfg, training, momentum, eps, prep):
    L.require_cuda(points, weight)
    lib = L.lib()
    dev = points.device
    B = len(offsets) - 1
    if prep is None:
        prep = pillar_prep(points, offsets, pcfg)
    pt_off, feat, _, num_voxels, _ = prep
    weight = weight.contiguous().float()
    with torch.cuda.device(dev):
        bn_out = torch.empty(4 * 64, dtype=torch.float32, device=dev)
        moments = torch.empty(80, dtype=torch.float64, device=dev)
        partials = torch.empty(lib.liso_pfn_partials_bytes(), dtype=torch.uint8, device=dev)
        L.check(lib.liso_pfn_bn_prepare_f32(L.ptr(feat), L.ptr(pt_off), ctypes.byref(pcfg), B, L.ptr(num_voxels),
                                            L.ptr(weight), L.ptr(gamma), L.ptr(beta), L.ptr(running_mean),
                                            L.ptr(running_var), float(momentum), float(eps), int(training),
                                            L.ptr(bn_out), L.ptr(moments), L.ptr(partials), L.stream_ptr()), "pfn_bn_prepare")
    return prep, weight, bn_out, moments


class _PillarFeatureScatter(torch.autograd.Function):

    @staticmethod
    def forward(ctx, weight, gamma, beta, running_mean, running_var, points, offsets, pcfg, training, momentum, eps,
                out_dtype, out=None, prep=None):
        code = L.elem_code(out_dtype)
        lib = L.lib()
        dev = points.device
        B = len(offsets) - 1
        prep, weight, bn_out, moments = _pfn_statistics(weight, gamma, beta, running_mean, running_var, points, offsets, pcfg, training,
                                                        momentum, eps, prep)
        pt_off, feat, voxel_cell, num_voxels, cell_to_voxel = prep
        with torch.cuda.device(dev):
            st = L.stream_ptr()
            if out is not None:
                canvas, occupancy = out
                assert canvas.shape == (B, pcfg.gx, pcfg.gy, 64) and canvas.dtype == out_dtype and canvas.is_contiguous()
                assert occupancy.shape == (B, 1, pcfg.gx, pcfg.gy) and occupancy.is_contiguous()
            else:
                canvas = torch.empty((B, pcfg.gx, pcfg.gy, 64), dtype=out_dtype, device=dev)
                occupancy = torch.empty((B, 1, pcfg.gx, pcfg.gy), dtype=torch.float32, device=dev)
            L.check(L.TIMER.launch("pfn_forward_scatter", lambda: lib.liso_pfn_forward_scatter(
                L.ptr(feat), L.ptr(pt_off), L.ptr(voxel_cell), ctypes.byref(pcfg), B, L.ptr(cell_to_voxel), L.ptr(weight),
                L.ptr(bn_out), L.ptr(canvas), code, L.ptr(occupancy), st),
                units=points.numel() * 4 + canvas.numel() * canvas.element_size() + occupancy.numel() * 4),
                "pfn_forward_scatter")
        ctx.save_for_backward(feat, pt_off, voxel_cell, num_voxels, weight, gamma, bn_out, moments)
        ctx.pcfg, ctx.B, ctx.training = pcfg, B, bool(training)
        ctx.mark_non_differentiable(occupancy)
        return canvas.permute(0, 3, 1, 2), occupancy

    @staticmethod
    def backward(ctx, grad_canvas, _grad_occ):
        feat, pt_off, voxel_cell, num_voxels, weight, gamma, bn_out, moments = ctx.saved_tensors
        lib = L.lib()
        dev = feat.device
        g = grad_canvas.permute(0, 2, 3, 1)
        if g.dtype not in (torch.float32, torch.bfloat16, torch.float16):
            g = g.float()
        g = g.contiguous()
        F = weight.shape[1]
        gw = torch.empty((64, F), dtype=torch.float32, device=dev)
        gg = torch.empty(64, dtype=torch.float32, device=dev)
        gb = torch.empty(64, dtype=torch.float32, device=dev)
        partials = torch.empty(lib.liso_pfn_partials_bytes(), dtype=torch.uint8, device=dev)
        with torch.cuda.device(dev):
            L.check(lib.liso_pfn_backward(L.ptr(feat), L.ptr(pt_off), L.ptr(voxel_cell), ctypes.byref(ctx.pcfg), ctx.B,
                                          L.ptr(num_voxels), L.ptr(weight), L.ptr(gamma), L.ptr(bn_out), L.ptr(moments),
                                          int(ctx.training), L.ptr(g), L.elem_code(g.dtype), L.ptr(gw), L.ptr(gg),
                                          L.ptr(gb), L.ptr(partials), L.stream_ptr()), "pfn_backward")
        return gw, gg, gb, None, None, None, None, None, None, None, None, None, None, None


@torch.no_grad()
def pillar_rows(weight, gamma, beta, running_mean, running_var, points, offsets, pcfg, training, momentum, eps, out_dtype, out=None,
                prep=None):
    from liso_amd.utils.mfma_conv import PillarCanvas

    code = L.elem_code(out_dtype)
    lib = L.lib()
    dev = points.device
    B = len(offsets) - 1
    prep, weight, bn_out, _ = _pfn_statistics(weight, gamma, beta, running_mean, running_var, points, offsets, pcfg, training, momentum,
                                              eps, prep)
    pt_off, feat, voxel_cell, num_voxels, cell_to_voxel = prep
    if out is None:
        out = PillarCanvas.empty(B, (pcfg.gx, pcfg.gy), pcfg.max_voxels, out_dtype, dev)
    R = B * pcfg.max_voxels
    assert tuple(out.shape) == (B, 64, pcfg.gx, pcfg.gy) and out.dtype == out_dtype and out.max_voxels == pcfg.max_voxels
    assert out.row_base + R <= out.rows.shape[0]
    rows = out.rows[out.row_base:out.row_base + R]
    with torch.cuda.device(dev):
        st = L.stream_ptr()
        cells = B * pcfg.gx * pcfg.gy
        L.check(L.TIMER.launch("pfn_forward_scatter", lambda: lib.liso_pfn_forward_rows(
            L.ptr(feat), L.ptr(pt_off), L.ptr(voxel_cell), ctypes.byref(pcfg), B, L.ptr(cell_to_voxel), L.ptr(weight),
            L.ptr(bn_out), L.ptr(rows), code, out.row_base, L.ptr(out.cell_map), L.ptr(out.occupancy), st),
            units=points.numel() * 4 + cells * 12),
            "pfn_forward_rows")
    return out


class PointsPillarFeatureNetWrapper(nn.Module):
    def __init__(self, cfg) -> None:
        super().__init__()
        self.cfg = cfg
        z_cut = cfg.data.setdefault("z_pillar_cutoff_value", 5.0)
        assert z_cut > 0.0, z_cut
        half = np.append(np.array(cfg.data.bev_range_m) / 2.0, z_cut)
        pc_range = np.concatenate([-half, half], axis=0)
        voxel_size = np.append(np.array(cfg.data.bev_range_m) / np.array(cfg.data.img_grid_size), 2 * z_cut)
        self.max_num_points, self.max_voxels = 20, 40000
        if "use_lidar_intensity" in cfg.data:
            num_input_channels = [3, 4][cfg.data.use_lidar_intensity]
        else:
            num_input_channels = 3
        if cfg.data.setdefault("num_point_channels", None):
            num_input_channels = int(cfg.data.num_point_channels)
            assert num_input_channels in (3, 4, 5), num_input_channels
        self.num_input_channels = num_input_channels
        crf = cfg.network.centerpoint.setdefault("channel_reduction_factor", 1)
        assert 64 // crf == 64, "the fused gfx950 PFN kernel is built for 64 output channels"
        self.pts_voxel_encoder = PillarFeatureNet(
            in_channels=num_input_channels, feat_channels=[64 // crf], voxel_size=voxel_size,
            point_cloud_range=pc_range, norm_cfg={"type": "BN1d", "eps": 0.001, "momentum": 0.01})
        self.voxel_size, self.pc_range = voxel_size, pc_range
        self.grid = tuple(int(g) for g in cfg.data.img_grid_size)
        self.out_dtype = torch.float32

    def _pcfg(self, n_channels):
        c = L.PillarCfg()
        c.x_min, c.y_min, c.z_min = (float(np.float32(v)) for v in self.pc_range[:3])
        c.vx, c.vy, c.vz = (float(np.float32(v)) for v in self.voxel_size)
        c.gx, c.gy = self.grid
        c.max_points, c.max_voxels, c.n_channels = self.max_num_points, self.max_voxels, n_channels
        return c

    @staticmethod
    def _cat(points):
        assert isinstance(points, (list, tuple)), type(points)
        offsets = [0]
        for p in points:
            assert p.dim() == 2, p.shape
            offsets.append(offsets[-1] + p.shape[0])
        cat = torch.cat([p.float() for p in points], dim=0).contiguous()
        return cat, offsets

    @torch.no_grad()
    def voxelize(self, points):
        cat, offsets = self._cat(points)
        pcfg = self._pcfg(cat.shape[1])
        return self._compact(cat, pcfg, len(points), voxelize_raw(cat, offsets, pcfg))

    @staticmethod
    def _compact(cat, pcfg, B, vox):
        coors, num_points, slots, num_voxels, _ = vox
        nv = num_voxels.cpu().tolist()
        rows = torch.cat([torch.arange(b * pcfg.max_voxels, b * pcfg.max_voxels + nv[b], device=cat.device)
                          for b in range(B)])
        sl = slots[rows].long()
        valid = torch.arange(pcfg.max_points, device=cat.device)[None, :] < num_points[rows][:, None]
        vox = torch.where(valid[..., None], cat[sl.clamp(min=0, max=max(cat.shape[0] - 1, 0))],
                          torch.zeros((), device=cat.device))
        return vox, num_points[rows], coors[rows]

    @torch.no_grad()
    def prepare(self, pts):
        cat, offsets = self._cat(pts)
        return (cat, offsets, pillar_prep(cat, offsets, self._pcfg(cat.shape[1])))

    def extract_pts_feat(self, pts, out=None, prep=None, compact=False):
        L.elem_code(self.out_dtype)
        if prep is not None:
            cat, offsets, prep = prep
        else:
            cat, offsets = self._cat(pts)
        C = cat.shape[1]
        assert C == self.num_input_channels, (C, self.num_input_channels)
        lyr = self.pts_voxel_encoder.pfn_layers[0]
        training = self.training and lyr.norm.training
        if training and lyr.norm.track_running_stats:
            lyr.norm.num_batches_tracked += 1
        if compact:
            assert not torch.is_grad_enabled(), "the compact canvas has no backward: inference only"
            canvas = pillar_rows(lyr.linear.weight, lyr.norm.weight, lyr.norm.bias, lyr.norm.running_mean, lyr.norm.running_var, cat,
                                 offsets, self._pcfg(C), training, lyr.norm.momentum, lyr.norm.eps, self.out_dtype, out, prep)
            return canvas, canvas.occupancy
        x, occ = _PillarFeatureScatter.apply(lyr.linear.weight, lyr.norm.weight, lyr.norm.bias, lyr.norm.running_mean,
                                             lyr.norm.running_var, cat, offsets, self._pcfg(C), training,
                                             lyr.norm.momentum, lyr.norm.eps, self.out_dtype, out, prep)
        return x, occ

    def forward(self, pcl_t0, img_t0=None, out=None, prep=None, compact=False):
        return self.extract_pts_feat(pcl_t0, out=out, prep=prep, compact=compact)
```

liso_amd/trainer.py:

```python
import collections
import contextlib
import ctypes
import os

import torch
import torch.distributed as dist

from liso_amd import _lib as L

from liso_amd.losses.centerpoint_loss import centerpoint_loss, rotation_vec_on_unit_circle
from liso_amd.networks.simple_net.simple_net import BoxLearner
from liso_amd.utils import graph_capture as GC
from liso_amd.utils import tensor_tree as TT


def get_optimizer_scheduler(cfg, box_predictor, total_steps=None, flat=False):
    if flat:
        from liso_amd.utils.flat_adamw import FlatAdamW

        opt = FlatAdamW(box_predictor.parameters(), lr=cfg.optimization.learning_rate, weight_decay=0.01)
    else:
        opt = torch.optim.AdamW(box_predictor.parameters(), lr=cfg.optimization.learning_rate, weight_decay=0.01)
    common = dict(optimizer=opt, max_lr=cfg.optimization.learning_rate, pct_start=0.4, base_momentum=0.85, max_momentum=0.95,
                  div_factor=10.0)
    source = cfg.data.setdefault("train_on_box_source", "gt")
    if source == "gt":
        sched = torch.optim.lr_scheduler.OneCycleLR(total_steps=(total_steps or cfg.optimization.num_training_steps) + 2, **common)
    elif source == "mined":
        assert cfg.optimization.rounds.active, "assuming this"
        rounds = cfg.optimization.rounds
        sched = torch.optim.lr_scheduler.OneCycleLR(
            total_steps=(total_steps or rounds.steps_per_round * rounds.drop_net_weights_every_nth_round) + 2, final_div_factor=10,
            **common)
    else:
        raise NotImplementedError(source)
    return opt, sched


def get_slim_optimizer_scheduler(slim_cfg, params, flat=False):
    from liso_amd.utils.learning_rate import get_polynomial_decay_schedule_with_warmup

    if slim_cfg.optimizer == "rmsprop" and flat:
        from liso_amd.utils.flat_adamw import FlatRMSprop

        opt = FlatRMSprop(list(params), lr=slim_cfg.learning_rate.initial)
    elif slim_cfg.optimizer == "rmsprop":
        opt = torch.optim.RMSprop(params, lr=slim_cfg.learning_rate.initial)
    elif slim_cfg.optimizer == "adam":
        opt = torch.optim.Adam(params, lr=slim_cfg.learning_rate.initial)
    else:
        raise AssertionError("only rmsprop/adam supported")
    sched = get_polynomial_decay_schedule_with_warmup(
        optimizer=opt, num_warmup_steps=slim_cfg.learning_rate.warm_up.step_length,
        num_training_steps=slim_cfg.iterations.train, lr_end=slim_cfg.learning_rate.initial * 0.05)
    return opt, sched


def gather_gradients(device, params, add=False):
    jobs = []
    for p_, flat in params:
        g = p_.grad
        p_.grad = flat
        if g is None or g is flat:
            continue
        if add or g.dtype != torch.float32 or g.stride() != flat.stride() or g.shape != flat.shape:
            flat.add_(g) if add else flat.copy_(g)
            continue
        jobs.append((g, flat))
    if not jobs:
        return []
    n = len(jobs)
    src = (ctypes.c_void_p * n)(*[g.data_ptr() for g, _ in jobs])
    dst = (ctypes.c_void_p * n)(*[f.data_ptr() for _, f in jobs])
    cnt = (ctypes.c_size_t * n)(*[g.numel() for g, _ in jobs])
    with torch.cuda.device(device):
        L.check(L.lib().liso_gather_f32(n, src, dst, cnt, L.stream_ptr()), "gather_f32")
    return [g for g, _ in jobs]


_SIDE_STREAMS = {}


def side_stream(device, role, priority=0):
    key = (device.index if device.index is not None else torch.cuda.current_device(), role)
    if key not in _SIDE_STREAMS:
        _SIDE_STREAMS[key] = (torch.cuda.Stream(device=device, priority=priority), priority)
    st, made_with = _SIDE_STREAMS[key]
    assert priority == made_with, f"side stream {role!r} exists with priority {made_with}, requested with {priority}"
    return st


def _prepare_device(device, exact):
    from liso_amd.utils import mfma_conv as MC

    if exact is not None:
        MC.set_fp32_mode("exact" if exact else "x3")
    if device.type == "cuda":
        MC._sparse_flag(device)


def _broadcast_replicas(net):
    for t in list(net.parameters()) + list(net.buffers()):
        dist.broadcast(t.data, src=0)


@contextlib.contextmanager
def _captured_training_pass(tr, canvases, second_half=False):
    from liso_amd.utils import mfma_conv as MC

    if not second_half:
        tr._flat_grad.zero_()
        for c in canvases:
            c.grad = None
        opt_packs = getattr(tr, "_opt_packs", None) if MC.optimizer_packs_enabled() else None
        if opt_packs is not None:
            tr._step_packs = dict(opt_packs.panels)
            if opt_packs.leftover_jobs:
                tr._step_packs.update(MC.batched_pack(opt_packs.leftover_jobs))
            tr._step_merged = opt_packs.merged
        else:
            tr._step_packs = MC.batched_pack(tr._pack_jobs) if tr._pack_jobs else None
            tr._step_merged = None
    MC.set_step_packs(tr._step_packs, getattr(tr, "_step_merged", None))
    gathered = tr._gather_params or []
    for p_, _ in gathered:
        p_.grad = None
    try:
        yield
    finally:
        MC.set_step_packs(None)
        tr._gather_keepalive = gather_gradients(tr.device, gathered, second_half)


class DetectorTrainer:
    def __init__(self, cfg, device, compute_dtype=torch.float32, total_steps=None, fused_loss=None, use_graph=False, exact=None,
                 grad_buckets=None, loss_scale="default"):
        from liso_amd.losses import fused_centerpoint

        self.cfg, self.device = cfg, device
        _prepare_device(device, exact)
        self.use_graph = bool(use_graph) and device.type == "cuda"
        self._graph, self._graph2, self._graph_sig = None, None, None
        self._opt_packs = None
        self.fused_loss = (fused_centerpoint.supports(cfg) and device.type == "cuda") if fused_loss is None else fused_loss
        self.net = BoxLearner(cfg).to(device)
        self.net.model.set_compute_dtype(compute_dtype)
        if self.use_graph and not self.fused_loss:
            from liso_amd.utils.graph_safety import require_node_replay

            require_node_replay("DetectorTrainer(use_graph=True) without the fused loss")
        self.model = self.net
        self.world = dist.get_world_size() if dist.is_available() and dist.is_initialized() else 1
        self.optimizer, self.lr_scheduler = get_optimizer_scheduler(cfg, self.net, total_steps, flat=device.type == "cuda")
        self.loss_scaler = None
        if loss_scale == "default":
            loss_scale = "dynamic" if compute_dtype == torch.float16 else None
        if loss_scale is not None:
            if compute_dtype != torch.float16:
                raise ValueError(f"loss scaling is for fp16 training (compute_dtype {compute_dtype})")
            if device.type != "cuda":
                raise ValueError("fp16 training runs on the device kernels only")
            from liso_amd.utils.loss_scale import DeviceLossScale

            if loss_scale == "dynamic":
                self.loss_scaler = DeviceLossScale(device)
            elif isinstance(loss_scale, (int, float)) and not isinstance(loss_scale, bool):
                self.loss_scaler = DeviceLossScale(device, init_scale=float(loss_scale), dynamic=False)
            else:
                raise ValueError(f"loss_scale: 'dynamic', a number or None, got {loss_scale!r}")
            self.optimizer.loss_scale = self.loss_scaler
        if self.world > 1 and not self.use_graph:
            self.model = torch.nn.parallel.DistributedDataParallel(
                self.net, device_ids=[device.index] if device.type == "cuda" else None, bucket_cap_mb=64,
                broadcast_buffers=False, gradient_as_bucket_view=device.type != "cuda")
        self.n_grad_buckets = 1
        if self.use_graph:
            self._flat_grad = self.optimizer.flat_grad
            if self.world > 1:
                _broadcast_replicas(self.net)
                self.optimizer.grad_scale = 1.0 / self.world
                self._setup_gradient_buckets(grad_buckets)
            elif grad_buckets == 2:
                self._setup_gradient_buckets(2)
        from liso_amd.networks.centerpoint.fused_bn import defer_batch_counters
        self._bn_counters = defer_batch_counters(self.net.model.rpn) + defer_batch_counters(self.net.model.center_head)

    def _setup_gradient_buckets(self, grad_buckets):
        from liso_amd.utils import mfma_conv as MC

        rpn = self.net.model.rpn
        if grad_buckets is None:
            grad_buckets = int(os.environ.get("LISO_GRAD_BUCKETS", "2"))
        if grad_buckets < 2 or len(rpn.blocks) < 2 or not hasattr(self.optimizer, "offsets"):
            return
        first = next(rpn.blocks[1].parameters())
        split = self.optimizer.offsets[id(first)]
        order = [id(p_) for p_ in self.net.parameters() if p_.requires_grad]
        assert all(self.optimizer.offsets[i] < split for i in order[:order.index(id(first))])
        assert all(self.optimizer.offsets[i] >= split for i in order[order.index(id(first)):])
        self._bucket_split = int(split)
        self._grad_cut = MC.GradCut()
        self.n_grad_buckets = 2

    def _reduce_gradients(self, rest_of_backward):
        if getattr(self, "skip_collective", False):
            rest_of_backward()
            return
        if self.n_grad_buckets < 2:
            rest_of_backward()
            dist.all_reduce(self._flat_grad)
            return
        w1 = dist.all_reduce(self._flat_grad[self._bucket_split:], async_op=True)
        rest_of_backward()
        w2 = dist.all_reduce(self._flat_grad[:self._bucket_split], async_op=True)
        w1.wait()
        w2.wait()

    def loss(self, pcls, targets, canvas=None):
        if self.model.training:
            from liso_amd.networks.centerpoint.fused_bn import step_batch_counters
            step_batch_counters(self._bn_counters)
        cfg = self.cfg
        sup = cfg.loss.supervised.supervised_on_clusters
        gt_maps = {a: targets[a] for a in sup.attrs}
        mask = targets["center_bool_mask"]
        if self.fused_loss:
            from liso_amd.losses.fused_centerpoint import fused_centerpoint_loss

            _, _, raw, _ = self.model(None, pcls, None, centermaps_gt=None, decode=False, canvas=canvas)
            total, losses = fused_centerpoint_loss(
                cfg=cfg, raw_box_maps=raw, gt_maps=gt_maps, gt_center_mask=mask,
                ignore_region_is_true_mask=targets.get("ignore_region_is_true_mask", None),
                pillar_center_coors_m=self.net.pillar_center_coors_m)
            return total, losses, None
        pred_boxes, decoded, activated, aux = self.model(None, pcls, None, centermaps_gt=None)
        ignore = targets.get("ignore_region_is_true_mask", torch.zeros_like(mask))
        losses = centerpoint_loss(loss_cfg=cfg.loss, raw_activated_pred_box_maps=activated, decoded_pred_box_maps=decoded,
                                  gt_maps=gt_maps, gt_center_mask=mask,
                                  rotation_loss_weights_map=torch.ones_like(gt_maps["probs"]),
                                  box_prediction_cfg=cfg.box_prediction, ignore_region_is_true_mask=ignore)
        total = 0.0
        for v in losses.values():
            total = total + sup.weight * v
        rr = cfg.box_prediction.rotation_representation
        if rr.method == "vector":
            total = total + rotation_vec_on_unit_circle(activated) * rr.regul_weight
        return total, losses, pred_boxes

    def step(self, pcls, targets, prep=None):
        self.model.train()
        if self.use_graph:
            return self._graph_step(pcls, targets, prep)
        self.optimizer.zero_grad(set_to_none=True)
        total, losses, _ = self.loss(pcls, targets)
        self._backward(total)
        self.optimizer.step()
        self.lr_scheduler.step()
        return total.detach()

    def _backward(self, total):
        if self.loss_scaler is None:
            total.backward()
        else:
            total.backward(self.loss_scaler.seed)

    def loss_scale_stats(self):
        return None if self.loss_scaler is None else self.loss_scaler.stats()

    def eager_pass(self, pcls, targets):
        self.model.train()
        saved = [p.grad for p in self.net.parameters()]
        for p in self.net.parameters():
            p.grad = None
        ctx = self.model.no_sync() if hasattr(self.model, "no_sync") else contextlib.nullcontext()
        with GC.frozen_buffers(self.net, keep=lambda k, v: "running" in k or "num_batches" in k), ctx:
            total, _, _ = self.loss(pcls, targets)
            self._backward(total)
        for p, g in zip(self.net.parameters(), saved):
            p.grad = g
        return total.detach()

    def _pillars(self, pcls, out=None, prep=None):
        return self.net.model.pfn(pcl_t0=pcls, img_t0=None, out=out, prep=prep)

    def _capture(self, pcls, targets):
        from liso_amd.utils import mfma_conv as MC

        dev = self.device
        with GC.frozen_buffers(self.net) as restore:
            with torch.no_grad():
                bev, occ = self._pillars(pcls)
            self._static_bev = bev.detach().clone().requires_grad_(True)
            self._static_occ = occ.detach().clone()
            self._static_targets = {k: v.to(dev).clone() for k, v in targets.items()}
            side = side_stream(dev, "flow")
            self._graph2, self._pack_jobs, self._gather_params = None, [], None
            cut = self._grad_cut if self.n_grad_buckets == 2 else None
            rpn = self.net.model.rpn

            def body(part=None):
                with _captured_training_pass(self, [self._static_bev], second_half=part == 2):
                    MC.set_direct_grads(True, keep_touched=part == 2)
                    try:
                        if part in (None, 1):
                            rpn.grad_cut = cut
                            try:
                                total, _, _ = self.loss(None, self._static_targets, canvas=(self._static_bev, self._static_occ))
                            finally:
                                rpn.grad_cut = None
                            self._backward(total)
                            self._body_loss = total.detach()
                        if cut is not None and part in (None, 2):
                            cut.finish()
                    finally:
                        MC.set_direct_grads(False, keep_touched=True)
                return self._body_loss

            def after_first_pass():
                in_place = MC.direct_touched()
                outside = {id(p_) for p_ in self.net.model.pfn.parameters()}
                self._gather_params = [(p_, p_.grad) for p_ in self.net.parameters()
                                       if p_.requires_grad and p_.grad is not None and id(p_) not in in_place and id(p_) not in outside]

            if self._opt_packs is not None:
                self._opt_packs.ensure_current()
            GC.warm_up(body, side, pack_jobs=self._pack_jobs, after_first=after_first_pass, restore=restore)
            self._attach_optimizer_packs(MC.recorded_merged_jobs())
            if cut is None:
                self._graph, self._static_loss = GC.capture(body, side)
            else:
                self._graph, self._static_loss = GC.capture(lambda: body(1), side)
                self._graph2, _ = GC.capture(lambda: body(2), side, pool=self._graph.pool())

    def _attach_optimizer_packs(self, merged_jobs):
        from liso_amd.utils import mfma_conv as MC
        from liso_amd.utils.flat_adamw import FlatAdamW

        if self._opt_packs is not None or not MC.optimizer_packs_enabled() or not self._pack_jobs:
            return
        if not isinstance(self.optimizer, FlatAdamW) or self.optimizer.loss_scale is not None:
            return
        from liso_amd.utils.optimizer_packs import OptimizerPacks

        self._opt_packs = OptimizerPacks(self.optimizer, self._pack_jobs, merged_jobs)
        self.optimizer.attach_packs(self._opt_packs)

    def _graph_step(self, pcls, targets, prep=None):
        tsig = targets.shapes() if isinstance(targets, _BatchedTargets) else tuple((k, tuple(v.shape), v.dtype) for k, v in sorted(targets.items()))
        from liso_amd.utils import mfma_conv as MC

        sig = (len(pcls), tsig, MC.optimizer_packs_enabled())
        if self._graph is None or sig != self._graph_sig:
            self._graph = None
            self._capture(pcls, targets)
            self._graph_sig = sig
        bev, occ = self._pillars(pcls, out=(self._static_bev.detach().permute(0, 2, 3, 1), self._static_occ), prep=prep)
        with torch.no_grad():
            stage = []
            if isinstance(targets, _BatchedTargets):
                off = {}
                for t in targets.per_sample:
                    for k, v in t.items():
                        o = off.get(k, 0)
                        stage.append((self._static_targets[k][o:o + v.shape[0]], v))
                        off[k] = o + v.shape[0]
            else:
                for k, v in targets.items():
                    stage.append((self._static_targets[k], v))
            L.multi_copy(stage)
        if self._opt_packs is not None and sig[2]:
            self._opt_packs.ensure_current()
        self._graph.replay()

        def rest_of_backward():
            if self._graph2 is not None:
                self._graph2.replay()
            if bev.requires_grad:
                bev.backward(self._static_bev.grad)

        if self.world > 1:
            self._reduce_gradients(rest_of_backward)
        else:
            rest_of_backward()
        self.optimizer.step()
        self.lr_scheduler.step()
        return self._static_loss.clone()


class SlimTrainer:

    def __init__(self, cfg, device, num_train_samples=1000, use_graph=False, exact=None):
        from liso_amd.slim.model.slim import SLIM

        _prepare_device(device, exact)
        self.cfg, self.slim_cfg, self.device = cfg, cfg.SLIM, device
        self.net = SLIM(cfg, num_train_samples=num_train_samples).to(device)
        self.model = self.net
        self.use_graph = bool(use_graph) and device.type == "cuda"
        self.world = dist.get_world_size() if dist.is_available() and dist.is_initialized() else 1
        if self.world > 1 and not self.use_graph:
            self.model = torch.nn.parallel.DistributedDataParallel(
                self.net, device_ids=[device.index] if device.type == "cuda" else None, bucket_cap_mb=64,
                broadcast_buffers=False, gradient_as_bucket_view=True)
        flat = device.type == "cuda" and self.model is self.net
        self.optimizer, self.lr_scheduler = get_slim_optimizer_scheduler(self.slim_cfg, self.net.parameters(), flat=flat)
        self._flat_opt = hasattr(self.optimizer, "flat_grad")
        import numpy as np
        half = 0.5 * np.array(cfg.data.bev_range_m, dtype=np.float32)
        self.bev_extent = np.concatenate([-half, half], axis=0)
        self._graph, self._graph_sig = None, None
        if self.use_graph:
            from liso_amd.utils.graph_safety import require_node_replay

            require_node_replay("SlimTrainer(use_graph=True)")
            self.net.raft_network.defer_update_block_wgrad = "direct"
            params = [p for p in self.net.parameters() if p.requires_grad]
            if self._flat_opt:
                self._flat_grad = self.optimizer.flat_grad
            else:
                self._flat_grad = torch.zeros(sum(p.numel() for p in params), dtype=torch.float32, device=device)
                off = 0
                for p in params:
                    p.grad = self._flat_grad[off:off + p.numel()].view_as(p)
                    off += p.numel()
            outside = {id(p) for p in self.net.raft_network.pp_layer.parameters()} if hasattr(self.net.raft_network, "pp_layer") else set()
            self._gather_params = [(p, p.grad) for p in params if id(p) not in outside]
            if self.world > 1:
                _broadcast_replicas(self.net)

    def _inputs(self, sample_t0, sample_t1):
        pc1, m1 = sample_t0["pcl_ta"]["pcl"].to(self.device), sample_t0["pcl_ta"]["pcl_is_valid"].to(self.device)
        pc2, m2 = sample_t1["pcl_ta"]["pcl"].to(self.device), sample_t1["pcl_ta"]["pcl_is_valid"].to(self.device)
        return pc1, m1, pc2, m2

    def loss(self, sample_t0, sample_t1, all_valid=None, canvases=None, gather_plan=None):
        from liso_amd.slim.slim_loss.knn_graph import KnnIndex
        from liso_amd.slim.slim_loss.slim_loss_adaptor import selfsupervisedSlimSingleScaleLoss

        pc1, m1, pc2, m2 = self._inputs(sample_t0, sample_t1)
        if all_valid is None:
            all_valid = (bool(m1.all()), bool(m2.all()))
        ext = [float(v) for v in self.bev_extent]
        idx1 = [KnnIndex(pc1[b][:, :3], extent=ext, all_rows_finite=True) for b in range(pc1.shape[0])] if all_valid[0] else None
        idx2 = [KnnIndex(pc2[b][:, :3], extent=ext, all_rows_finite=True) for b in range(pc2.shape[0])] if all_valid[1] else None
        if canvases is None:
            preds_fw, preds_bw = self.model(sample_t0, sample_t1, None)
        else:
            preds_fw, preds_bw = self.model(sample_t0, sample_t1, None, canvases=canvases, gather_plan=gather_plan)
        kw = dict(moving_thresh_module=self.net.moving_dynamicness_threshold, loss_cfg=self.slim_cfg.losses.unsupervised,
                  model_cfg=self.slim_cfg.model, bev_extent=self.bev_extent, metrics_collector={})
        stacked = getattr(self.net, "stacked_predictions", None)
        if stacked is not None and not self.slim_cfg.model.use_static_aggr_flow_for_aggr_flow:
            sfw, sbw, n_it = stacked
            rep = lambda t: t.repeat(n_it, *([1] * (t.dim() - 1)))
            total = n_it * selfsupervisedSlimSingleScaleLoss(
                pc1=rep(pc1), valid_mask_pc1=rep(m1), pc2=rep(pc2), valid_mask_pc2=rep(m2), pred_fw=sfw, pred_bw=sbw,
                knn_index_pc1=None if idx1 is None else idx1 * n_it, knn_index_pc2=None if idx2 is None else idx2 * n_it, **kw)
            return total, preds_fw, preds_bw
        total = torch.zeros(1, device=self.device)
        for pfw, pbw in zip(preds_fw, preds_bw):
            total = total + selfsupervisedSlimSingleScaleLoss(pc1=pc1, valid_mask_pc1=m1, pc2=pc2, valid_mask_pc2=m2, pred_fw=pfw,
                                                              pred_bw=pbw, knn_index_pc1=idx1, knn_index_pc2=idx2, **kw)
        return total, preds_fw, preds_bw

    def step(self, sample_t0, sample_t1, eager=False, update=True):
        self.model.train()
        if self.use_graph and not eager:
            return self._graph_step(sample_t0, sample_t1)
        total, _, _ = self.loss(sample_t0, sample_t1)
        if self.use_graph:
            self._flat_grad.zero_()
        else:
            self.optimizer.zero_grad(set_to_none=True)
        if not update:
            with self.model.no_sync() if hasattr(self.model, "no_sync") else contextlib.nullcontext():
                total.backward()
            return total.detach()
        total.backward()
        self._reduce_and_update()
        return total.detach()

    def eval_model(self, val_batches, max_iterations=None):
        from liso_amd.slim.validation import run_eval_on_this_dataset

        was_training = self.net.training
        self.net.eval()
        try:
            return run_eval_on_this_dataset(self.net, val_batches, max_iterations=max_iterations)
        finally:
            self.net.train(was_training)

    def _reduce_and_update(self):
        if self.use_graph and self.world > 1:
            dist.all_reduce(self._flat_grad)
            self._flat_grad.div_(self.world)
        self.optimizer.step()
        self.lr_scheduler.step()

    def _capture(self, sample_t0, sample_t1, all_valid):
        self._static = TT.tree_map((sample_t0, sample_t1), lambda t: t.to(self.device).clone())
        s0, s1 = self._static
        with GC.frozen_buffers(self.net) as restore:
            with torch.no_grad():
                canv = self._pillars(sample_t0, sample_t1)
            self._static_canv = tuple(c.detach().clone() for c in canv)
            leaves = [self._static_canv[i].requires_grad_(True) for i in (0, 2)]
            self._static_plan = None
            meta = getattr(self.net, "gather_plan_meta", None)
            if meta is None:
                with torch.no_grad():
                    self.net(s0, s1, None, canvases=self._static_canv)
                meta = getattr(self.net, "gather_plan_meta", None)
            if meta is not None:
                self._static_plan = self.net.build_gather_plan(s0, s1, *meta)
                self._static_plan.lin64
            thr = self.net.moving_dynamicness_threshold
            defer = self.world > 1 and bool(self.slim_cfg.model.use_static_aggr_flow_for_aggr_flow)
            self._thr_items = None

            def body():
                with _captured_training_pass(self, leaves):
                    thr._defer = [] if defer else None
                    try:
                        total, _, _ = self.loss(s0, s1, all_valid, canvases=self._static_canv, gather_plan=self._static_plan)
                        total.backward()
                    finally:
                        self._thr_items, thr._defer = thr._defer, None
                return total.detach()

            self._pack_jobs = []
            self._graph, self._static_loss = GC.capture(body, side_stream(self.device, "flow"), warm_ups=2, pack_jobs=self._pack_jobs,
                                                        restore=restore)

    def capture(self, sample_t0, sample_t1):
        _, m1, _, m2 = self._inputs(sample_t0, sample_t1)
        all_valid = (bool(m1.all()), bool(m2.all()))
        sig = (TT.tree_signature((sample_t0, sample_t1)), all_valid)
        if self._graph is None or sig != self._graph_sig:
            self._graph = None
            self._capture(sample_t0, sample_t1, all_valid)
            self._graph_sig = sig
            return True
        return False

    def _pillars(self, sample_t0, sample_t1):
        from liso_amd.slim.model.slim import get_network_input_pcls

        dev = self.device
        return self.net.raft_network.encode_pillars(get_network_input_pcls(self.cfg, sample_t0, "ta", to_device=dev),
                                                    get_network_input_pcls(self.cfg, sample_t1, "ta", to_device=dev))

    def _graph_step(self, sample_t0, sample_t1):
        if not self.capture(sample_t0, sample_t1):
            TT.tree_copy_(self._static, (sample_t0, sample_t1))
        canv = self._pillars(sample_t0, sample_t1)
        with torch.no_grad():
            for d, c in zip(self._static_canv, canv):
                d.copy_(c.detach(), non_blocking=True)
            if self._static_plan is not None:
                fresh = self.net.build_gather_plan(sample_t0, sample_t1, *self.net.gather_plan_meta)
                for name in ("lin", "sorted_lin", "order", "seg_rank"):
                    getattr(self._static_plan, name).copy_(getattr(fresh, name), non_blocking=True)
                self._static_plan.lin64.copy_(fresh.lin, non_blocking=True)
        self._graph.replay()
        if self._thr_items:
            with torch.no_grad():
                self.net.moving_dynamicness_threshold.apply_deferred(self._thr_items)
        live = [(canv[i], self._static_canv[i].grad) for i in (0, 2) if canv[i].requires_grad]
        if live:
            torch.autograd.backward([c for c, _ in live], [g for _, g in live])
        self._reduce_and_update()
        return self._static_loss.clone()


class _Prefetched:
    __slots__ = ("pair", "flow", "done", "targets", "boxes", "cluster_count")

    def __init__(self, pair, flow, done, targets=None, boxes=None, cluster_count=None):
        self.pair, self.flow, self.done = pair, flow, done
        self.targets, self.boxes, self.cluster_count = targets, boxes, cluster_count

    def is_for(self, pair):
        return self.pair[0] is pair[0] and self.pair[1] is pair[1]


class _BatchedTargets(dict):

    def __init__(self, per_sample):
        super().__init__()
        self.per_sample = list(per_sample)
        for k in self.per_sample[0]:
            dict.__setitem__(self, k, None)

    def __getitem__(self, k):
        v = dict.__getitem__(self, k)
        if v is None:
            v = torch.cat([t[k] for t in self.per_sample], dim=0)
            dict.__setitem__(self, k, v)
        return v

    def get(self, k, default=None):
        return self[k] if k in self else default

    def items(self):
        return [(k, self[k]) for k in self.keys()]

    def values(self):
        return [self[k] for k in self.keys()]

    def shapes(self):
        rows = {k: sum(t[k].shape[0] for t in self.per_sample) for k in self.per_sample[0]}
        return tuple((k, (rows[k],) + tuple(v.shape[1:]), v.dtype) for k, v in sorted(self.per_sample[0].items()))


class LisoLoopTrainer:

    def __init__(self, cfg, device, compute_dtype=torch.float32, total_steps=None, slim_state_dict=None, use_graph=False,
                 overlap=False, infer_batch=2, flow_ahead=0, exact=None):
        from liso_amd.networks.flow_cluster_detector.flow_cluster_detector import FlowClusterDetector
        from liso_amd.slim.model.slim import SLIM

        self.cfg, self.device = cfg, device
        _prepare_device(device, exact)
        self.use_graph = bool(use_graph) and device.type == "cuda"
        self._graph_infer = self.use_graph and use_graph in (True, "infer")
        self._graph_det = self.use_graph and use_graph in (True, "detector")
        self._graph_mine = self.use_graph and use_graph is True
        sync = lambda: torch.cuda.synchronize(device)
        self._infer_graphs, self._mine_graphs = GC.GraphLRU(sync), GC.GraphLRU(sync)
        tcfg = cfg.data.tracking_cfg
        self.infer_point_bucket = int(tcfg.setdefault("infer_point_bucket", 8192))
        self.max_infer_graphs = int(tcfg.setdefault("max_infer_graphs", 8))
        self.max_mine_graphs = int(tcfg.setdefault("max_mine_graphs", 6))
        self.mine_capture_budget = int(tcfg.setdefault("mine_capture_budget", 24))
        self.mine_capture_window = int(tcfg.setdefault("mine_capture_window", 400))
        self.mine_captures, self.mine_eager_fallbacks = 0, 0
        self._mine_calls, self._mine_capture_calls, self._mine_fallback_warned = 0, [], False
        self._views = collections.OrderedDict()
        self.overlap = bool(overlap) and device.type == "cuda"
        self.infer_batch, self.flow_ahead = int(infer_batch), int(flow_ahead)
        self.box_capacity, self.capacity_overflows = int(cfg.data.tracking_cfg.setdefault("flow_cluster_capacity", 64)), 0
        self._flow_stream, self._mine_stream, self._main_used_static = None, None, None
        self._inputs_ready = None
        self._flows, self._mined = [], []
        self.slim = SLIM(cfg, num_train_samples=1000).to(device)
        if slim_state_dict is not None:
            self.slim.load_state_dict(slim_state_dict)
        self.slim.eval()
        for p_ in self.slim.parameters():
            p_.requires_grad_(False)
        self.cluster_detector = FlowClusterDetector(cfg).to(device)
        self.detector = DetectorTrainer(cfg, device, compute_dtype=compute_dtype, total_steps=total_steps, use_graph=self._graph_det)
        if device.type == "cuda":
            self._flow_stream = side_stream(device, "flow")
            self._mine_stream = side_stream(device, "mine0", priority=-1)
            n_mine = max(1, int(os.environ.get("LISO_MINE_STREAMS", "1")))
            self._mine_streams = [self._mine_stream] + [side_stream(device, f"mine{k}", priority=-1) for k in range(1, n_mine)]
            self._mine_turn = 0
        self.infer_cus = 0
        if device.type == "cuda" and self.overlap:
            n_cu = torch.cuda.get_device_properties(device).multi_processor_count
            self.infer_cus = int(os.environ.get("LISO_INFER_CUS", str(n_cu // 2)))
            if self.infer_cus >= n_cu:
                self.infer_cus = 0
        self._pillar_prep = None
        self._prep_ahead = os.environ.get("LISO_PREP_AHEAD", "1") != "0"
        self.pre_nms, self.post_nms = tcfg.max_num_boxes_before_nms, tcfg.max_num_boxes_after_nms
        self.nms_iou = cfg.setdefault("nms_iou_threshold", 0.1)

    @torch.no_grad()
    def mine_boxes(self, sample_t0, sample_t1):
        flow = self._infer_flow(sample_t0, sample_t1)
        _, boxes = self._targets_from_flow(sample_t0, flow)
        return boxes, flow

    _stack_samples = staticmethod(TT.tree_stack)

    def _pad_loss_cloud(self, sample):
        pa, bk = sample["pcl_ta"], self.infer_point_bucket
        n = pa["pcl"].shape[1]
        pad = (-n) % bk if bk > 1 else 0
# ... 382 lines not shown
```

liso_amd/utils/mfma_conv.py:

```python
import ctypes
import os
import weakref

import torch

from liso_amd import _lib as L


def on_device(x):
    if not x.is_cuda:
        return False
    L.elem_code(x.dtype)
    return True


class ConvSpec:

    def __init__(self, kh, kw, stride=1, padding=0, transposed=False):
        self.kh, self.kw, self.stride, self.padding, self.transposed = int(kh), int(kw), int(stride), int(padding), bool(transposed)

    @staticmethod
    def of(conv):
        st = conv.stride[0] if isinstance(conv.stride, (tuple, list)) else conv.stride
        pd = conv.padding[0] if isinstance(conv.padding, (tuple, list)) else conv.padding
# ... 415 lines not shown
    B, ho, wo, co = gv.shape
    _, ci, hi, wi = x_shape
    out_dtype = out_dtype or dy.dtype
    out_f32 = out_dtype == torch.float32
    build = gather_desc if spec.transposed else scatter_desc
    d = build(spec, B, ho, wo, co, gps, hi, wi, ci, ci, 0, mode, out_f32, False, False)
    alloc = torch.zeros if getattr(d, "sparse_output", False) else torch.empty
    if not spec.transposed and ((ho - 1) * spec.stride - spec.padding + spec.kh < hi or (wo - 1) * spec.stride - spec.padding + spec.kw < wi):
        alloc = torch.zeros
    dx = alloc((B, hi, wi, ci), dtype=out_dtype, device=dy.device)
    if packed is None:
        packed = pack_weights(weight, spec, True, mode)
    with torch.cuda.device(dy.device):
        L.check(L.TIMER.launch(_timer_name(mode, "dgrad", d), lambda: L.lib().liso_conv_forward(
            ctypes.byref(d), L.ptr(gv), L.ptr(packed), None, None, None, L.ptr(dx), None, None, L.stream_ptr()), units=_flops(d), nbytes=_bytes(d)),
            "conv_dgrad")
    return dx.permute(0, 3, 1, 2)


class WgradReduceJob:

    def __init__(self, job, ws, dw, db, device):
        self.job, self.ws, self.dw, self.db, self.device, self.done = job, ws, dw, db, device, False

    def ride(self):
        assert not self.done
        self.done = True
        return ctypes.byref(self.job)

    def flush(self):
        if not self.done:
            self.done = True
            with torch.cuda.device(self.device):
                L.check(L.lib().liso_conv_wgrad_reduce(ctypes.byref(self.job), L.stream_ptr()), "conv_wgrad_reduce")


_DEFER_WGRAD_REDUCE = True


def set_deferred_wgrad_reduce(on):
    global _DEFER_WGRAD_REDUCE
    prev, _DEFER_WGRAD_REDUCE = _DEFER_WGRAD_REDUCE, bool(on)
    return prev


def conv_wgrad(x, dy, weight_shape, spec, in_scale=None, in_shift=None, in_relu=False, want_bias=True, out_dw=None, out_db=None,
               co_true=None, defer_reduce=False):
    L.require_cuda(x, dy)
    if (x.shape[1] == 4 and x.dtype == torch.float32 and not spec.transposed and spec.stride == 1 and spec.kh == spec.kw and spec.kh in (5, 7)
            and spec.padding == spec.kh // 2 and in_scale is None and tuple(weight_shape[1:]) == (4, spec.kh, spec.kw)):
        res = _conv_wgrad_smallci(x, dy, weight_shape, spec, want_bias, out_dw, out_db, co_true)
        if res is not None:
            return (*res, None) if defer_reduce else res
    mode = _mode(x.dtype)
    if dy.dtype != x.dtype:
        dy = dy.to(x.dtype)
    if co_true is None:
        co_true = dy.shape[1]
        dy, _ = _pad_out_channels(dy, None, spec, _vec(mode))
    xv, xps = as_nhwc(x, _vec(mode))
    gv, gps = as_nhwc(dy, _vec(mode))
    B, hi, wi, ci = xv.shape
    _, ho, wo, co = gv.shape
    build = scatter_desc if spec.transposed else gather_desc
    d = build(spec, B, hi, wi, ci, xps, ho, wo, co, co, 0, mode, True, in_relu, False)
    if co != co_true:
        d = L.ConvDesc.from_buffer_copy(d)
        d.wgrad_co = co_true
    lib = L.lib()
    nbytes = lib.liso_conv_wgrad_workspace_bytes(ctypes.byref(d))
    if nbytes == 0:
        return None
    ws = torch.empty(nbytes, dtype=torch.uint8, device=x.device)
    dw = out_dw if out_dw is not None else torch.empty(weight_shape, dtype=torch.float32, device=x.device)
    db = (out_db if out_db is not None else torch.empty(co_true, dtype=torch.float32, device=x.device)) if want_bias else None
    args = (ctypes.byref(d), L.ptr(xv), L.ptr(in_scale) if in_scale is not None else None,
            L.ptr(in_shift) if in_shift is not None else None, L.ptr(gv), gps, int(spec.transposed), L.ptr(dw),
            L.ptr(db) if db is not None else None, L.ptr(ws), nbytes)
    with torch.cuda.device(x.device):
        if defer_reduce:
            job = L.WgradReduceJob()
            L.check(L.TIMER.launch(_timer_name(mode, "wgrad"), lambda: lib.liso_conv_wgrad_deferred(*args, ctypes.byref(job), L.stream_ptr()),
                                   units=_flops(d), nbytes=_bytes(d, True)), "conv_wgrad_deferred")
            return dw, db, WgradReduceJob(job, ws, dw, db, x.device)
        L.check(L.TIMER.launch(_timer_name(mode, "wgrad"), lambda: lib.liso_conv_wgrad(*args, L.stream_ptr()),
                               units=_flops(d), nbytes=_bytes(d, True)), "conv_wgrad")
    return dw, db


def _conv_wgrad_smallci(x, dy, weight_shape, spec, want_bias, out_dw, out_db, co_true):
    if dy.dtype != torch.float32:
        dy = dy.float()
    xv, xps = as_nhwc(x, 4)
    gv, gps = as_nhwc(dy, 4)
    B, hi, wi, _ = xv.shape
    co = co_true if co_true is not None else gv.shape[3]
    if gv.shape[1:3] != (hi, wi) or weight_shape[0] != co:
        return None
    lib = L.lib()
    nbytes = lib.liso_conv_wgrad_smallci_workspace_bytes(B, hi, wi, co, spec.kh)
    if nbytes == 0:
        return None
    ws = torch.empty(nbytes, dtype=torch.uint8, device=x.device)
    dw = out_dw if out_dw is not None else torch.empty(weight_shape, dtype=torch.float32, device=x.device)
    db = (out_db if out_db is not None else torch.empty(co, dtype=torch.float32, device=x.device)) if want_bias else None
    with torch.cuda.device(x.device):
        L.check(L.TIMER.launch("conv_wgrad_smallci", lambda: lib.liso_conv_wgrad_smallci_f32(
            L.ptr(xv), xps, L.ptr(gv), gps, B, hi, wi, co, spec.kh, L.ptr(dw), L.ptr(db) if db is not None else None, L.ptr(ws), nbytes,
            L.stream_ptr()), units=2.0 * B * hi * wi * co * 4 * spec.kh * spec.kw), "conv_wgrad_smallci")
    return dw, db


def conv_wgrad_sparse(x, occupancy, dy, weight_shape, spec, want_bias=True):
    L.require_cuda(x, dy, occupancy)
    if x.dtype != torch.float32 or spec.transposed or occupancy.dtype != torch.float32:
        return None
    if dy.dtype != torch.float32:
        dy = dy.float()
    xv, xps = as_nhwc(x, 4)
    gv, gps = as_nhwc(dy, 4)
    B, hi, wi, ci = xv.shape
    _, ho, wo, co = gv.shape
    occ = occupancy.contiguous()
    if occ.numel() != B * hi * wi:
        return None
    d = gather_desc(spec, B, hi, wi, ci, xps, ho, wo, co, co, 0, _mode(x.dtype), True, False, False)
    lib = L.lib()
    nbytes = lib.liso_conv_wgrad_sparse_workspace_bytes(ctypes.byref(d))
    if nbytes == 0:
        return None
    ws = torch.empty(nbytes, dtype=torch.uint8, device=x.device)
    dw = torch.empty(weight_shape, dtype=torch.float32, device=x.device)
    db = torch.empty(co, dtype=torch.float32, device=x.device) if want_bias else None
    with torch.cuda.device(x.device):
        L.check(L.TIMER.launch("conv_wgrad_sparse", lambda: lib.liso_conv_wgrad_sparse_f32(
            ctypes.byref(d), L.ptr(xv), L.ptr(occ), L.ptr(gv), gps, L.ptr(dw), L.ptr(db) if db is not None else None, L.ptr(ws), nbytes,
            L.stream_ptr()), units=_flops(d), nbytes=_bytes(d, True)), "conv_wgrad_sparse")
    return dw, db


def supported(x, weight, spec):
    if not x.is_cuda or x.dtype not in (torch.bfloat16, torch.float16, torch.float32):
        return False
    vec = L.lane_channels(x.dtype)
    ci = x.shape[1]
    co = weight.shape[1] if spec.transposed else weight.shape[0]
    if ci % vec or spec.kh * spec.kw > L.CONV_MAX_TAPS:
        return False
    if spec.transposed and (spec.kh != spec.stride or spec.padding != 0):
        return False
    return co >= 1


class BnFold:

    def __init__(self, groups, relu=True, training=True):
        self.groups, self.relu, self.training = list(groups), bool(relu), bool(training)
        self._ss = None
        self.deferred = None
        self.merged = None

    @property
    def channels(self):
        return sum(g["gamma"].shape[0] for g in self.groups)

    def scale_shift(self):
        if self._ss is None:
            if len(self.groups) == 1:
                st, C = self.groups[0]["stats"], self.groups[0]["gamma"].shape[0]
                self._ss = (st[:C], st[C:2 * C])
            else:
                self._ss = (torch.cat([g["stats"][:g["gamma"].shape[0]] for g in self.groups]).contiguous(),
                            torch.cat([g["stats"][g["gamma"].shape[0]:2 * g["gamma"].shape[0]] for g in self.groups]).contiguous())
        return self._ss

    def use_merged(self, buf, total):
        assert total == self.channels and buf.numel() == 5 * total
        self.merged = (buf, total)
        self._ss = (buf[:total], buf[total:2 * total])

    def group(self, k):
        return BnFold([self.groups[k]], self.relu, self.training)

    @staticmethod
    def cat(folds):
        assert all(f.relu == folds[0].relu and f.training == folds[0].training for f in folds)
        return BnFold([g for f in folds for g in f.groups], folds[0].relu, folds[0].training)

    def params(self):
        return [t for g in self.groups for t in (g["gamma"], g["beta"])]


def merged_stats_wanted(taps):
    return _JOINT_BN_BACKWARD and all(d[1].training or not d[1].track_running_stats for _, _, d in taps)


def finalize_bn(stats_partial, n_pixels, bn, stats_shift=None, channel_offset=0, merged=None):
    C = bn.num_features
    stats = torch.empty(4 * C, dtype=torch.float32, device=stats_partial.device)
    rows, _, cop = stats_partial.shape
    mom = bn.momentum if bn.momentum is not None else 0.1
    track = bn.track_running_stats and bn.training
    part = ctypes.c_void_p(stats_partial.data_ptr() + 4 * channel_offset)
    with torch.cuda.device(stats_partial.device):
        args = (part, rows, C, cop, int(n_pixels), L.ptr(stats_shift) if stats_shift is not None else None,
                L.ptr(bn.weight), L.ptr(bn.bias), L.ptr(bn.running_mean) if track else None, L.ptr(bn.running_var) if track else None,
                float(mom), float(bn.eps), L.ptr(stats))
        if merged is not None:
            buf, total, off = merged
            L.check(L.lib().liso_conv_bn_finalize_merged(*args, L.ptr(buf), ctypes.c_void_p(buf.data_ptr() + 16 * total), total, off,
                                                         L.stream_ptr()), "conv_bn_finalize_merged")
        else:
            L.check(L.lib().liso_conv_bn_finalize(*args, L.stream_ptr()), "conv_bn_finalize")
    return BnFold([{"stats": stats, "gamma": bn.weight, "beta": bn.bias}], True, True)


def eval_bn_fold(bn, relu=True):
    with torch.no_grad():
        invstd = torch.rsqrt(bn.running_var.float() + bn.eps)
        scale = bn.weight.detach().float() * invstd
        shift = bn.bias.detach().float() - bn.running_mean.float() * scale
        stats = torch.cat([scale, shift, bn.running_mean.float(), invstd]).contiguous()
    return BnFold([{"stats": stats, "gamma": bn.weight, "beta": bn.bias}], relu, False)


_DIRECT_GRADS = False
_DIRECT_TOUCHED = set()


def set_direct_grads(on, keep_touched=False):
    global _DIRECT_GRADS
    _DIRECT_GRADS = bool(on)
    if not keep_touched:
        _DIRECT_TOUCHED.clear()


def direct_touched():
    return set(_DIRECT_TOUCHED)


def _direct_target(p):
    if not _DIRECT_GRADS or not isinstance(p, torch.nn.Parameter):
        return None
    g = p.grad
    if g is None or g.dtype != torch.float32 or not g.is_contiguous() or g.shape != p.shape or id(p) in _DIRECT_TOUCHED:
        return None
    _DIRECT_TOUCHED.add(id(p))
    return g


def _bn_backward_prelude(gs, x_raw, groups, table=None):
    vec, views = L.lane_channels(x_raw.dtype), []
    for t in (x_raw, *gs):
        if t.dtype != x_raw.dtype:
            t = t.to(x_raw.dtype)
        v, s = _rows_view(t, vec)
        if table is not None and (v is None or (views and v.shape != views[0][0].shape)):
            return None
        views.append((v, s) if v is not None else (t.permute(0, 2, 3, 1).contiguous(), t.shape[1]))
    dev, lib = x_raw.device, L.lib()
    targets = []
    for grp in groups:
        C = grp["gamma"].shape[0]
        tg, tb = _direct_target(grp["gamma"]), _direct_target(grp["beta"])
        direct = tg is not None and tb is not None
        targets.append((tg if direct else torch.empty(C, dtype=torch.float32, device=dev),
                        tb if direct else torch.empty(C, dtype=torch.float32, device=dev), direct))
    if table is None:
        tab, nbytes = None, lib.liso_bn_workspace_bytes(groups[0]["gamma"].shape[0])
    else:
        tab = (L.BnGroup * len(groups))()
        for row, grp, (off, c), (gg, gb, _) in zip(tab, groups, table, targets):
            row.c_off, row.c = off, c
            row.gamma, row.stats, row.grad_gamma, row.grad_beta = grp["gamma"].data_ptr(), grp["stats"].data_ptr(), gg.data_ptr(), gb.data_ptr()
        nbytes = lib.liso_bn_multi_workspace_bytes(tab, len(groups), len(gs))
    return views, targets, tab, torch.empty(nbytes, dtype=torch.uint8, device=dev)


def _bn_backward_group(g, x_raw, grp, relu, training, out=None, job=None):
    C = grp["gamma"].shape[0]
    ((xv, xs), (gv, gs)), ((gg, gb, direct),), _, ws = _bn_backward_prelude([g], x_raw, [grp])
    M = xv.numel() // C
    dxv, ds = _rows_view(out, L.lane_channels(xv.dtype)) if out is not None else (None, 0)
    if dxv is None:
        dxv, ds = torch.empty(xv.shape, dtype=xv.dtype, device=xv.device), C
    if (xs, gs, ds) == (C, C, C):
        xs = gs = ds = 0
    riding = job is not None and not job.done
    with torch.cuda.device(xv.device):
        L.check(L.TIMER.launch("bn_bwd", lambda: L.lib().liso_bn_relu_bwd_chained(
            L.ptr(gv), gs, L.ptr(xv), xs, L.elem_code(xv.dtype), M, C, L.ptr(grp["gamma"]), L.ptr(grp["stats"]), int(training), int(relu),
            L.ptr(dxv), ds, L.ptr(gg), L.ptr(gb), L.ptr(ws), ws.numel(), job.ride() if riding else None, L.stream_ptr()),
            units=5 * M * C * xv.element_size()), "bn_relu_bwd_chained")
    return dxv.permute(0, 3, 1, 2), (None if direct else gg), (None if direct else gb)


_JOINT_BN_BACKWARD = True


def set_joint_bn_backward(on):
    global _JOINT_BN_BACKWARD
    prev, _JOINT_BN_BACKWARD = _JOINT_BN_BACKWARD, bool(on)
    return prev


def bn_group_table(Cs, vec):
    if not 1 <= len(Cs) <= L.BN_MAX_GROUPS:
        return None
    table, off = [], 0
    for c in Cs:
        if c <= 0 or c > 256 or c % vec:
            return None
        table.append((off, c))
        off += c
    return table


def _bn_backward_grouped(gs, x_raw, fold, jobs=()):
    Cs = [grp["gamma"].shape[0] for grp in fold.groups]
    table = bn_group_table(Cs, L.lane_channels(x_raw.dtype))
    if table is None or x_raw.shape[1] != sum(Cs) or not 1 <= len(gs) <= 2:
        return None
    pre = _bn_backward_prelude(gs, x_raw, fold.groups, table)
    if pre is None:
        return None
    ((xv, xs), (ga, gsa), *second), targets, tab, ws = pre
    gb, gsb = second[0] if second else (None, 0)
    M, Ct = xv.numel() // xv.shape[3], xv.shape[3]
    dxv = torch.empty(xv.shape, dtype=xv.dtype, device=xv.device)
    riding = [j for j in jobs if not j.done][:2]
    with torch.cuda.device(xv.device):
        L.check(L.TIMER.launch("bn_bwd", lambda: L.lib().liso_bn_relu_bwd_multi(
            L.ptr(ga), gsa, L.ptr(gb) if gb is not None else None, gsb, L.ptr(xv), xs, L.elem_code(xv.dtype), M, tab, len(Cs),
            int(fold.training), int(fold.relu), L.ptr(dxv), Ct, L.ptr(ws), ws.numel(), *[j.ride() for j in riding], *[None] * (2 - len(riding)),
            L.stream_ptr()), units=(3 + 2 * len(gs)) * M * Ct * xv.element_size()), "bn_relu_bwd_multi")
    return dxv.permute(0, 3, 1, 2), [None if direct else t for gg, gb_, direct in targets for t in (gg, gb_)]


def _bn_backward(gs, x_raw, fold, jobs=(), out=None, shared=False):
    jobs = [j for j in jobs if j is not None]
    Cs = [grp["gamma"].shape[0] for grp in fold.groups]
    assert out is None or (len(gs), len(Cs)) == (1, 1)
    if len(gs) <= 2 and (shared or (len(Cs) > 1 and sum(Cs) > 256 and _JOINT_BN_BACKWARD)):
        res = _bn_backward_grouped(gs, x_raw, fold, jobs)
        if res is not None:
            return res
    if len(gs) > 1:
        dx, grads = None, [None] * (2 * len(Cs))
        for g in gs:
            d, gr = _bn_backward([g], x_raw, fold, jobs)
            dx = d if dx is None else dx + d
            grads = [b if a is None else (a if b is None else a + b) for a, b in zip(grads, gr)]
        return dx, grads
    g, job = gs[0], next((j for j in jobs if not j.done), None)
    if len(Cs) == 1:
        dx, gg, gb = _bn_backward_group(g, x_raw, fold.groups[0], fold.relu, fold.training, out=out, job=job)
        return dx, [gg, gb]
    if sum(Cs) > 256:
        B, _, H, W = x_raw.shape
        dx_full = torch.empty((B, H, W, sum(Cs)), dtype=x_raw.dtype, device=x_raw.device).permute(0, 3, 1, 2)
        grads, a = [], 0
        for k, C in enumerate(Cs):
            dx, gr = _bn_backward([g[:, a:a + C]], x_raw[:, a:a + C], fold.group(k), jobs, out=dx_full[:, a:a + C])
            if dx.data_ptr() != dx_full[:, a:a + C].data_ptr():
                dx_full[:, a:a + C].copy_(dx)
            grads += gr
            a += C
        return dx_full, grads
    if fold.merged is not None:
        buf, total = fold.merged
        gam, stats = buf[4 * total:], buf[:4 * total]
    else:
        gam = torch.cat([grp["gamma"].detach() for grp in fold.groups])
        stats = torch.cat([grp["stats"][k * c:(k + 1) * c] for k in range(4) for grp, c in zip(fold.groups, Cs)])
    dx, gg, gb = _bn_backward_group(g, x_raw, {"gamma": gam, "beta": None, "stats": stats}, fold.relu, fold.training, job=job)
    grads, a = [], 0
    for c in Cs:
        grads += [gg[a:a + c], gb[a:a + c]]
        a += c
    return dx, grads


class _SharedFold(torch.autograd.Function):
    @staticmethod
    def forward(ctx, x_raw, node, n, *fold_params):
        ctx.node, ctx.n, ctx.n_fold_params = node, n, len(fold_params)
        ctx.save_for_backward(x_raw)
        return tuple(torch.ops.aten.alias(x_raw) for _ in range(n))

    @staticmethod
    def backward(ctx, *gs):
        (x_raw,) = ctx.saved_tensors
        fold, jobs = ctx.node["fold"], ctx.node["jobs"]
        gs = [g for g in gs if g is not None]
        try:
            dx, grads = _bn_backward(gs, x_raw, fold, jobs, shared=True) if gs else (None, [None] * ctx.n_fold_params)
        finally:
            for j in jobs:
                j.flush()
            jobs.clear()
        return (dx, None, None, *grads)


def shared_fold(x_raw, fold, n=2):
    vec = L.lane_channels(x_raw.dtype)
    if (not _JOINT_BN_BACKWARD or fold is None or not fold.training or fold.deferred is not None or not torch.is_grad_enabled()
            or not x_raw.requires_grad or not x_raw.is_cuda or _rows_view(x_raw, vec)[0] is None
            or bn_group_table([g["gamma"].shape[0] for g in fold.groups], vec) is None):
        return None
    node = {"fold": fold, "jobs": []}
    outs = _SharedFold.apply(x_raw, node, int(n), *fold.params())
    held = BnFold(fold.groups, fold.relu, fold.training)
    held._ss, held.merged, held.deferred = fold.scale_shift(), fold.merged, node
    return list(outs), held


class _FusedConv(torch.autograd.Function):
    @staticmethod
    def forward(ctx, x_raw, weight, bias, meta, *fold_params):
        spec, fold = meta["spec"], meta["fold"]
        sc, sh = fold.scale_shift() if fold is not None else (None, None)
        occ = meta.get("occupancy") if fold is None else None
        res = None
        if occ is not None and meta.get("out_dtype") in (None, x_raw.dtype):
            res = _sparse_stem(x_raw, occ, weight, bias, spec, "batch" if meta.get("want_stats", False) else "none",
                               meta.get("out_relu", False), stats_shift=meta.get("stats_shift"))
        sparse_ws = None
        if res is not None:
            y, part, sparse_ws = res
        else:
            y, part = conv_forward(x_raw, weight, bias, spec, sc, sh, in_relu=fold.relu if fold is not None else False,
                                   out_relu=meta.get("out_relu", False), out_dtype=meta.get("out_dtype"),
                                   want_stats=meta.get("want_stats", False), stats_shift=meta.get("stats_shift"), occupancy=occ,
                                   out=meta.get("out"))
        meta["stats_partial"] = part
        relu = bool(meta.get("out_relu", False))
        ctx.save_for_backward(x_raw, weight, y if relu else None)
        ctx.meta = {"spec": spec, "fold": fold, "has_bias": bias is not None, "n_fold_params": len(fold_params), "relu": relu,
                    "bias_param": bias if isinstance(bias, torch.nn.Parameter) else None, "occupancy": occ, "sparse_ws": sparse_ws}
        return y

    @staticmethod
    def backward(ctx, dy):
        x_raw, weight, y = ctx.saved_tensors
        spec, fold = ctx.meta["spec"], ctx.meta["fold"]
        if dy.dtype != x_raw.dtype:
            dy = dy.to(x_raw.dtype)
        if ctx.meta["relu"]:
            dy = torch.ops.aten.threshold_backward(dy, y, 0.0)
        sc, sh = fold.scale_shift() if fold is not None else (None, None)
        dw = db = dx = job = None
        fold_grads = [None] * ctx.meta["n_fold_params"]
        co_true = dy.shape[1]
        if co_true % _vec(_mode(dy.dtype)):
            dy, _ = _pad_out_channels(dy, None, spec, _vec(_mode(dy.dtype)))
        want_dx = ctx.needs_input_grad[0] or any(ctx.needs_input_grad[4:])
        if ctx.needs_input_grad[1] or (ctx.meta["has_bias"] and ctx.needs_input_grad[2]):
            tw = _direct_target(weight)
            tb = _direct_target(ctx.meta["bias_param"]) if tw is not None and ctx.meta["has_bias"] else None
            if ctx.meta["has_bias"] and tb is None:
                tw = None
            res = None
            if ctx.meta.get("occupancy") is not None and co_true == dy.shape[1]:
                res = conv_wgrad_sparse(x_raw, ctx.meta["occupancy"], dy, tuple(weight.shape), spec, want_bias=ctx.meta["has_bias"])
                tw = None if res is not None else tw
            if res is None:
                defer = _DEFER_WGRAD_REDUCE and dy.is_cuda and fold is not None and want_dx
                res = conv_wgrad(x_raw, dy, tuple(weight.shape), spec, sc, sh, in_relu=fold.relu if fold is not None else False,
                                 want_bias=ctx.meta["has_bias"], out_dw=tw, out_db=tb, co_true=co_true, defer_reduce=defer)
                if defer and res is not None:
                    job, res = res[2], res[:2]
            if res is None:
                raise NotImplementedError(f"liso_amd: no device weight-gradient kernel for {tuple(weight.shape)} stride {spec.stride} "
                                          f"on {tuple(x_raw.shape)} {x_raw.dtype}")
            else:
                dw, db = res
                if tw is not None and dw is tw:
                    dw, db = None, None
        try:
            if want_dx:
                g = None
                if ctx.meta.get("occupancy") is not None and fold is None and co_true == dy.shape[1]:
                    g = _sparse_dgrad(dy, ctx.meta["occupancy"], weight, spec, tuple(x_raw.shape), x_raw.dtype, lists=ctx.meta.get("sparse_ws"))
                if g is None:
                    g = conv_dgrad(dy, weight, spec, tuple(x_raw.shape))
                if fold is not None and fold.deferred is not None:
                    dx = g
                    if job is not None and dw is None:
                        fold.deferred["jobs"].append(job)
                        job = None
                elif fold is not None:
                    dx, fold_grads = _bn_backward([g], x_raw, fold, [job])
                else:
                    dx = g
        finally:
            if job is not None:
                job.flush()
        if dw is not None:
            dw = dw.to(weight.dtype)
        if db is not None:
            db = db.to(weight.dtype)
        return (dx, dw, db, None, *fold_grads)


def fused_conv(x_raw, fold, conv, out_bn=None, out_dtype=None, out_relu=False, spec=None, occupancy=None, out=None, merged_stats=None):
    convs = list(conv) if isinstance(conv, (list, tuple)) else [conv]
    bns = (list(out_bn) if isinstance(out_bn, (list, tuple)) else [out_bn]) if out_bn is not None else None
    spec = spec or ConvSpec.of(convs[0])
    if len(convs) == 1:
        weight, bias = convs[0].weight, convs[0].bias
    elif torch.is_grad_enabled() and any(c.weight.requires_grad for c in convs):
        static = merged_static("cat", [c.weight for c in convs]) if convs[0].bias is not None else None
        if static is not None:
            weight, bias = MergedFilters.apply(static, len(convs), *[c.weight for c in convs], *[c.bias for c in convs])
        else:
            weight = torch.cat([c.weight for c in convs], dim=0)
            bias = torch.cat([c.bias for c in convs], dim=0) if convs[0].bias is not None else None
            if bias is not None:
                note_merged_filter("cat", weight, [c.weight for c in convs], [c.bias for c in convs])
    else:
        key = tuple((id(c), c.weight._version, c.weight.data_ptr(), None if c.bias is None else c.bias._version) for c in convs)
        hit = getattr(convs[0], "_liso_merged_weights", None)
        if hit is None or hit[0] != key:
            w = torch.nn.Parameter(torch.cat([c.weight.detach() for c in convs], dim=0), requires_grad=False)
            b = torch.cat([c.bias.detach() for c in convs], dim=0) if convs[0].bias is not None else None
            hit = convs[0]._liso_merged_weights = (key, w, b)
        weight, bias = hit[1], hit[2]
    training_bn = bns is not None and (bns[0].training or not bns[0].track_running_stats)
    meta = {"spec": spec, "fold": fold, "out_dtype": out_dtype, "want_stats": training_bn, "out_relu": out_relu, "occupancy": occupancy,
            "out": out if occupancy is None else None}
    if training_bn and len(bns) == 1 and bns[0].track_running_stats:
        meta["stats_shift"] = bns[0].running_mean
    params = fold.params() if fold is not None and fold.deferred is None else []
    y = _FusedConv.apply(x_raw, weight, bias, meta, *params)
    if bns is None:
        return y, None
    if not training_bn:
        return y, BnFold.cat([eval_bn_fold(b, relu=True) for b in bns])
    n = y.shape[0] * y.shape[2] * y.shape[3]
    folds, off = [], 0
    total = sum(b.num_features for b in bns)
    own = torch.empty(5 * total, dtype=torch.float32, device=y.device) if len(bns) > 1 and _JOINT_BN_BACKWARD else None
    for b in bns:
        if b.training and b.track_running_stats and not getattr(b, "_liso_counter_deferred", False):
            b.num_batches_tracked += 1
        merged = (own, total, off) if own is not None else (merged_stats if len(bns) == 1 else None)
        folds.append(finalize_bn(meta["stats_partial"], n, b, meta.get("stats_shift"), channel_offset=off, merged=merged))
        off += b.num_features
    out_fold = BnFold.cat(folds)
    if own is not None:
        out_fold.use_merged(own, total)
    return y, out_fold


class InFold:

    def __init__(self, stats, channels, relu=True):
        self.stats, self.channels, self.relu = stats, int(channels), bool(relu)

    @property
    def scale(self):
        return self.stats

    @property
    def shift(self):
        return self.stats[:, self.channels:]

    @property
    def stride(self):
        return 4 * self.channels


def _norm_kind(norm):
    if isinstance(norm, torch.nn.Sequential) and len(norm) == 0:
        return "none"
    if isinstance(norm, torch.nn.InstanceNorm2d) and not norm.track_running_stats:
        return "instance"
    return None


@torch.no_grad()
def conv_in(x_raw, fold, conv, norm, relu=True, spec=None, occupancy=None):
    spec = spec or ConvSpec.of(conv)
    kind = _norm_kind(norm)
    kw = {}
    if fold is not None:
        kw = dict(in_scale=fold.scale, in_shift=fold.shift, in_relu=fold.relu, affine_batch_stride=fold.stride)
    compact = isinstance(x_raw, PillarCanvas)
    if compact:
        assert fold is None
        occupancy = x_raw.occupancy if occupancy is None else occupancy
    if fold is None and occupancy is not None:
        res = _sparse_stem(x_raw, occupancy, conv.weight, conv.bias, spec, kind, relu)
        if res is None and compact:
            x_raw = x_raw.dense()
        if res is not None:
            y, part, _ = res
            if kind == "none":
                return y, None
            return y, _in_fold_from_partial(y, part, norm, relu)
        kw["occupancy"] = occupancy
    if kind == "none":
        y, _ = conv_forward(x_raw, conv.weight, conv.bias, spec, out_relu=relu, **kw)
        return y, None
    y, part = conv_forward(x_raw, conv.weight, conv.bias, spec, want_stats=True, **kw)
    return y, _in_fold_from_partial(y, part, norm, relu)
# ... 322 lines not shown
```

Measured before the change: 1057.

## Fold PFN batch-norm derivation into scatter kernel and lean backward tail

```diff
diff --git a/include/liso_pillars.h b/include/liso_pillars.h
--- a/include/liso_pillars.h
+++ b/include/liso_pillars.h
@@ -38,6 +38,13 @@
                             float* running_var, float momentum, float eps, int training, float* bn_out, double* moments,
                             void* partials, void* stream);
 
+int liso_pfn_moments_f64(const float* feat, const int* pt_off, const liso_pillar_cfg* cfg, int batch, double* moments, void* partials,
+                         void* stream);
+int liso_pfn_forward_scatter_bn(const float* feat, const int* pt_off, const int* voxel_cell, const liso_pillar_cfg* cfg, int batch,
+                                const int* num_voxels, const int* cell_to_voxel, const double* moments, const float* weight,
+                                const float* gamma, const float* beta, float* running_mean, float* running_var, float momentum,
+                                float eps, int fold, float* bn_out, void* canvas, int out_bf16, float* occupancy, void* stream);
+
 int liso_pfn_forward_scatter(const float* feat, const int* pt_off, const int* voxel_cell, const liso_pillar_cfg* cfg, int batch,
                              const int* cell_to_voxel, const float* weight, const float* bn_out, void* canvas, int out_bf16,
                              float* occupancy, void* stream);
@@ -51,6 +58,11 @@
                       const double* moments, int training, const void* grad_canvas, int grad_bf16, float* grad_weight,
                       float* grad_gamma, float* grad_beta, void* partials, void* stream);
 
+int liso_pfn_backward_tail(const float* feat, const int* pt_off, const int* voxel_cell, const liso_pillar_cfg* cfg, int batch,
+                           const int* num_voxels, const float* weight, const float* gamma, const float* bn_out,
+                           const double* moments, int training, const void* grad_canvas, int grad_bf16, float* grad_weight,
+                           float* grad_gamma, float* grad_beta, int merged, int accumulate, void* partials, void* stream);
+
 #ifdef __cplusplus
 }
 #endif
diff --git a/liso_amd/_lib.py b/liso_amd/_lib.py
--- a/liso_amd/_lib.py
+++ b/liso_amd/_lib.py
@@ -130,6 +130,9 @@
     "liso_pfn_forward_scatter": (_i, [_vp, _vp, _vp, _vp, _i, _vp, _vp, _vp, _vp, _i, _vp, _vp]),
     "liso_pfn_forward_rows": (_i, [_vp, _vp, _vp, _vp, _i, _vp, _vp, _vp, _vp, _i, _i, _vp, _vp, _vp]),
     "liso_pfn_backward": (_i, [_vp, _vp, _vp, _vp, _i, _vp, _vp, _vp, _vp, _vp, _i, _vp, _i, _vp, _vp, _vp, _vp, _vp]),
+    "liso_pfn_moments_f64": (_i, [_vp, _vp, _vp, _i, _vp, _vp, _vp]),
+    "liso_pfn_forward_scatter_bn": (_i, [_vp, _vp, _vp, _vp, _i, _vp, _vp, _vp, _vp, _vp, _vp, _vp, _vp, _f, _f, _i, _vp, _vp, _i, _vp, _vp]),
+    "liso_pfn_backward_tail": (_i, [_vp, _vp, _vp, _vp, _i, _vp, _vp, _vp, _vp, _vp, _i, _vp, _i, _vp, _vp, _vp, _i, _i, _vp, _vp]),
     "liso_kabsch_workspace_bytes": (_sz, [_vp]),
     "liso_kabsch_trafos_f32": (_i, [_vp, _vp, _vp, _vp, _vp, _vp, _vp, _vp, _vp, _vp, _vp, _sz, _vp]),
     "liso_kabsch_trafos_counted_f32": (_i, [_vp, _vp, _vp, _vp, _vp, _vp, _vp, _vp, _vp, _vp, _vp, _vp, _sz, _vp]),
diff --git a/liso_amd/csrc/pillars.hip b/liso_amd/csrc/pillars.hip
--- a/liso_amd/csrc/pillars.hip
+++ b/liso_amd/csrc/pillars.hip
@@ -423,20 +423,11 @@
     return j * D - j * (j - 1) / 2 + (k - j);
 }
 
-template <int C>
-__global__ __launch_bounds__(1024) void pfn_bn_finalize_kernel(const double* __restrict__ partials, int nblocks,
-                                                               const int* __restrict__ num_voxels, int batch,
-                                                               int max_points, const float* __restrict__ weight,
-                                                               const float* __restrict__ gamma,
-                                                               const float* __restrict__ beta,
-                                                               float* __restrict__ running_mean,
-                                                               float* __restrict__ running_var, float momentum,
-                                                               float eps, float* __restrict__ bn_out,
-                                                               double* __restrict__ moments) {
-    constexpr int F = C + 6, D = F + 1;
-    constexpr int NS = LISO_PFN_STATS_DOUBLES, CH = 1024 / NS;
-    __shared__ double part[CH][NS];
-    __shared__ double mom[NS];
+constexpr int kMomNS = LISO_PFN_STATS_DOUBLES, kMomCH = 1024 / kMomNS;
+
+__device__ __forceinline__ void merge_moments(const double* __restrict__ partials, int nblocks, double (*part)[kMomNS], double* mom,
+                                              double* __restrict__ moments) {
+    constexpr int NS = kMomNS, CH = kMomCH;
     const int e = threadIdx.x % NS, chunk = threadIdx.x / NS;
     if (chunk < CH) {
         double s = 0.0;
@@ -461,9 +452,23 @@
         moments[threadIdx.x] = t;
     }
     __syncthreads();
-    __shared__ double rows_sq[kOut][F + 1], rows_sum[kOut][F + 1];
-    if (threadIdx.x < kOut * F) {
-        const int c = threadIdx.x / F, j = threadIdx.x % F;
+}
+
+struct PfnBnArgs {
+    const int* num_voxels;
+    const float *weight, *gamma, *beta;
+    float *running_mean, *running_var;
+    float momentum, eps;
+    int batch, max_points;
+};
+
+template <int C>
+__device__ __forceinline__ void derive_bn(const double* mom, double (*rows_sq)[C + 7], double (*rows_sum)[C + 7], const PfnBnArgs& a,
+                                          float* __restrict__ bn_out, float* bn_lds) {
+    constexpr int F = C + 6, D = F + 1;
+    const float* __restrict__ weight = a.weight;
+    for (int t = threadIdx.x; t < kOut * F; t += blockDim.x) {
+        const int c = t / F, j = t % F;
         const double wj = (double)weight[c * F + j];
         double q = 0.0;
         for (int k = 0; k < F; k++) {
@@ -476,9 +481,14 @@
     __syncthreads();
     if (threadIdx.x < kOut) {
         const int c = threadIdx.x;
+        const float* __restrict__ gamma = a.gamma;
+        const float* __restrict__ beta = a.beta;
+        float* __restrict__ running_mean = a.running_mean;
+        float* __restrict__ running_var = a.running_var;
+        const float eps = a.eps, momentum = a.momentum;
         long long P = 0;
-        for (int b = 0; b < batch; b++) P += num_voxels[b];
-        const double M = (double)P * (double)max_points;
+        for (int b = 0; b < a.batch; b++) P += a.num_voxels[b];
+        const double M = (double)P * (double)a.max_points;
         double sum = 0.0, sq = 0.0;
         for (int j = 0; j < F; j++) {
             sum += rows_sum[c][j];
@@ -492,16 +502,52 @@
         }
         const double invstd = 1.0 / sqrt(var + (double)eps);
         const float scale = (float)((double)gamma[c] * invstd);
-        bn_out[c] = scale;
-        bn_out[kOut + c] = (float)((double)beta[c] - mean * (double)gamma[c] * invstd);
-        bn_out[2 * kOut + c] = (float)mean;
-        bn_out[3 * kOut + c] = (float)invstd;
-        if (M > 1.0) {
-            const double mo = (double)momentum;
-            running_mean[c] = (float)((1.0 - mo) * (double)running_mean[c] + mo * mean);
-            running_var[c] = (float)((1.0 - mo) * (double)running_var[c] + mo * (var * M / (M - 1.0)));
-        }
-    }
+        const float shift = (float)((double)beta[c] - mean * (double)gamma[c] * invstd);
+        if (bn_lds) {
+            bn_lds[c] = scale;
+            bn_lds[kOut + c] = shift;
+            bn_lds[2 * kOut + c] = (float)mean;
+            bn_lds[3 * kOut + c] = (float)invstd;
+        }
+        if (bn_out) {
+            bn_out[c] = scale;
+            bn_out[kOut + c] = shift;
+            bn_out[2 * kOut + c] = (float)mean;
+            bn_out[3 * kOut + c] = (float)invstd;
+            if (M > 1.0) {
+                const double mo = (double)momentum;
+                running_mean[c] = (float)((1.0 - mo) * (double)running_mean[c] + mo * mean);
+                running_var[c] = (float)((1.0 - mo) * (double)running_var[c] + mo * (var * M / (M - 1.0)));
+            }
+        }
+    }
+    __syncthreads();
+}
+
+template <int C>
+__global__ __launch_bounds__(1024) void pfn_bn_finalize_kernel(const double* __restrict__ partials, int nblocks, PfnBnArgs a,
+                                                               float* __restrict__ bn_out, double* __restrict__ moments) {
+    __shared__ double part[kMomCH][kMomNS];
+    __shared__ double mom[kMomNS];
+    __shared__ double rows_sq[kOut][C + 7], rows_sum[kOut][C + 7];
+    merge_moments(partials, nblocks, part, mom, moments);
+    derive_bn<C>(mom, rows_sq, rows_sum, a, bn_out, nullptr);
+}
+
+__global__ __launch_bounds__(1024) void pfn_moments_merge_kernel(const double* __restrict__ partials, int nblocks,
+                                                                 double* __restrict__ moments) {
+    __shared__ double part[kMomCH][kMomNS];
+    __shared__ double mom[kMomNS];
+    merge_moments(partials, nblocks, part, mom, moments);
+}
+
+template <int C>
+__global__ __launch_bounds__(256) void pfn_bn_derive_kernel(const double* __restrict__ moments, PfnBnArgs a, float* __restrict__ bn_out) {
+    __shared__ double mom[kMomNS];
+    __shared__ double rows_sq[kOut][C + 7], rows_sum[kOut][C + 7];
+    if (threadIdx.x < kMomNS) mom[threadIdx.x] = moments[threadIdx.x];
+    __syncthreads();
+    derive_bn<C>(mom, rows_sq, rows_sum, a, bn_out, nullptr);
 }
 
 __global__ void pfn_bn_eval_kernel(const float* __restrict__ gamma, const float* __restrict__ beta,
@@ -539,17 +585,19 @@
 
 constexpr int kCellsPerBlock = 256;
 
-template <int C, typename OutT, bool ROWS>
+template <int C, typename OutT, bool ROWS, bool DERIVE = false>
 __global__ __launch_bounds__(kPfnThreads) void pfn_forward_kernel(const float* __restrict__ feat, const int* __restrict__ pt_off,
                                                                   const int* __restrict__ voxel_cell, int rows, int max_points,
                                                                   long total_cells, int zero_blocks,
                                                                   const int* __restrict__ cell_to_voxel,
-                                                                  const float* __restrict__ weight, const float* __restrict__ bn,
+                                                                  const float* __restrict__ weight, const float* bn,
                                                                   OutT* __restrict__ canvas, float* __restrict__ occupancy,
-                                                                  int* __restrict__ map_out, int row_base) {
+                                                                  int* __restrict__ map_out, int row_base,
+                                                                  const double* __restrict__ moments = nullptr, PfnBnArgs bn_args = PfnBnArgs()) {
     constexpr int F = C + 6;
     constexpr int kChunks = kOut * (int)sizeof(OutT) / 16;
     __shared__ __attribute__((aligned(16))) float frow[kPfnThreads / 64][kStage][kFP];
+    static_assert(sizeof(frow) >= 2 * sizeof(double) * kOut * (C + 7), "derive_bn's scratch lives in the staging rows");
     __shared__ int vox[kCellsPerBlock];
     const int tid = threadIdx.x, lane = tid & 63, wave = tid >> 6;
     const int pillar_blocks = (int)gridDim.x - zero_blocks;
@@ -573,13 +621,33 @@
         }
         return;
     }
-    float w[F];
-#pragma unroll
-    for (int k = 0; k < F; k++) w[k] = weight[lane * F + k];
-    const float scale = bn[lane], shift = bn[kOut + lane];
-    const float pad_val = fmaxf(shift, 0.f);
     const int wave_id = (int)blockIdx.x * (kPfnThreads / 64) + wave;
     const int n_waves = pillar_blocks * (kPfnThreads / 64);
+    float scale, shift;
+    if constexpr (DERIVE) {
+        __shared__ double mom[kMomNS];
+        __shared__ float bn_lds[4 * kOut];
+        const long per_block = (kPfnThreads / 64) * kGroup, step = (long)n_waves * kGroup;
+        const double m = tid < kMomNS ? moments[tid] : 0.0;
+        int any = 0;
+        for (long r0 = (long)blockIdx.x * per_block + tid * step; r0 < rows; r0 += kPfnThreads * step) {
+            const long r1 = r0 + per_block < rows ? r0 + per_block : rows;
+            any |= pt_off[r1] > pt_off[r0];
+        }
+        if (tid < kMomNS) mom[tid] = m;
+        if (!__syncthreads_or(any) && blockIdx.x != 0) return;
+        double (*rows_sq)[C + 7] = reinterpret_cast<double (*)[C + 7]>(&frow[0][0][0]);
+        derive_bn<C>(mom, rows_sq, rows_sq + kOut, bn_args, blockIdx.x == 0 ? const_cast<float*>(bn) : nullptr, bn_lds);
+        scale = bn_lds[lane];
+        shift = bn_lds[kOut + lane];
+    } else {
+        scale = bn[lane];
+        shift = bn[kOut + lane];
+    }
+    float w[F];
+#pragma unroll
+    for (int k = 0; k < F; k++) w[k] = weight[lane * F + k];
+    const float pad_val = fmaxf(shift, 0.f);
     for (int v0 = wave_id * kGroup; v0 < rows; v0 += n_waves * kGroup) {
         int off[kGroup + 1];
         stage_rows(feat, pt_off, rows, v0, lane, frow[wave], off);
@@ -608,7 +676,14 @@
     }
 }
 
-template <int C, typename GT>
+constexpr int kTailCh = 4;
+template <int NA, bool GROUPED>
+__device__ __forceinline__ size_t bwd_partial_index(int blk, int grid, int k, int c) {
+    if constexpr (GROUPED) return ((((size_t)(c / kTailCh) * grid + blk) * NA) + k) * kTailCh + c % kTailCh;
+    return ((size_t)blk * NA + k) * kOut + c;
+}
+
+template <int C, typename GT, bool GROUPED = false>
 __global__ __launch_bounds__(kPfnThreads) void pfn_backward_kernel(const float* __restrict__ feat, const int* __restrict__ pt_off,
                                                                    const int* __restrict__ voxel_cell, int rows, int max_points,
                                                                    const float* __restrict__ weight, const float* __restrict__ bn,
@@ -669,8 +744,25 @@
         const int k = idx / kOut, c = idx % kOut;
         float s = 0.f;
         for (int wv = 0; wv < kPfnThreads / 64; wv++) s += red[wv][k][c];
-        partials[((size_t)blockIdx.x * NA + k) * kOut + c] = s;
-    }
+        partials[bwd_partial_index<NA, GROUPED>(blockIdx.x, gridDim.x, k, c)] = s;
+    }
+}
+
+template <int NA, bool GROUPED>
+__device__ __forceinline__ double bwd_chunk_sum(const float* __restrict__ partials, int nblocks, int k, int c, int chunk) {
+    const int per = (nblocks + 15) / 16;
+    const int lo = chunk * per, hi = lo + per < nblocks ? lo + per : nblocks;
+    double s = 0.0;
+    int blk = lo;
+    for (; blk + 8 <= hi; blk += 8) {
+        float v[8];
+#pragma unroll
+        for (int j = 0; j < 8; j++) v[j] = partials[bwd_partial_index<NA, GROUPED>(blk + j, nblocks, k, c)];
+#pragma unroll
+        for (int j = 0; j < 8; j++) s += (double)v[j];
+    }
+    for (; blk < hi; blk++) s += (double)partials[bwd_partial_index<NA, GROUPED>(blk, nblocks, k, c)];
+    return s;
 }
 
 template <int NA>
@@ -678,21 +770,7 @@
                                                                    double* __restrict__ tot) {
     __shared__ double part[16][kOut];
     const int k = blockIdx.x, c = threadIdx.x & 63, chunk = threadIdx.x >> 6;
-    const int per = (nblocks + 15) / 16;
-    const int lo = chunk * per, hi = lo + per < nblocks ? lo + per : nblocks;
-    double s = 0.0;
-    {
-        int blk = lo;
-        for (; blk + 8 <= hi; blk += 8) {
-            float v[8];
-#pragma unroll
-            for (int j = 0; j < 8; j++) v[j] = partials[((size_t)(blk + j) * NA + k) * kOut + c];
-#pragma unroll
-            for (int j = 0; j < 8; j++) s += (double)v[j];
-        }
-        for (; blk < hi; blk++) s += (double)partials[((size_t)blk * NA + k) * kOut + c];
-    }
-    part[chunk][c] = s;
+    part[chunk][c] = bwd_chunk_sum<NA, false>(partials, nblocks, k, c, chunk);
     __syncthreads();
     if (chunk == 0) {
         double t = 0.0;
@@ -701,30 +779,35 @@
     }
 }
 
+struct PfnTailArgs {
+    const int* num_voxels;
+    const float *weight, *gamma, *bn;
+    const double* moments;
+    float *grad_weight, *grad_gamma, *grad_beta;
+    int batch, max_points, training;
+    int accumulate;
+};
+
+__device__ __forceinline__ void put_grad(float* p, float g, int accumulate) { *p = accumulate ? *p + g : g; }
+
 template <int C>
-__global__ __launch_bounds__(64) void pfn_backward_finalize_kernel(const double* __restrict__ tot,
-                                                                   const int* __restrict__ num_voxels, int batch,
-                                                                   int max_points, const float* __restrict__ weight,
-                                                                   const float* __restrict__ gamma,
-                                                                   const float* __restrict__ bn,
-                                                                   const double* __restrict__ moments, int training,
-                                                                   float* __restrict__ grad_weight,
-                                                                   float* __restrict__ grad_gamma,
-                                                                   float* __restrict__ grad_beta) {
+__device__ __forceinline__ void bwd_finalize_channel(const double* tot, int ts, int c, const PfnTailArgs& a) {
     constexpr int F = C + 6, D = F + 1;
-    const int c = threadIdx.x;
-    if (c >= kOut) return;
-    const double dbeta = tot[F * kOut + c], dgamma = tot[(F + 1) * kOut + c];
-    grad_beta[c] = (float)dbeta;
-    grad_gamma[c] = (float)dgamma;
-    const double invstd = (double)bn[3 * kOut + c], mean = (double)bn[2 * kOut + c];
-    const double gi = (double)gamma[c] * invstd;
-    if (!training) {
-        for (int k = 0; k < F; k++) grad_weight[c * F + k] = (float)(gi * tot[k * kOut + c]);
+    const float* __restrict__ weight = a.weight;
+    const double* __restrict__ moments = a.moments;
+    float* grad_weight = a.grad_weight;
+    const int max_points = a.max_points;
+    const double dbeta = tot[F * ts], dgamma = tot[(F + 1) * ts];
+    put_grad(a.grad_beta + c, (float)dbeta, a.accumulate);
+    put_grad(a.grad_gamma + c, (float)dgamma, a.accumulate);
+    const double invstd = (double)a.bn[3 * kOut + c], mean = (double)a.bn[2 * kOut + c];
+    const double gi = (double)a.gamma[c] * invstd;
+    if (!a.training) {
+        for (int k = 0; k < F; k++) put_grad(grad_weight + c * F + k, (float)(gi * tot[k * ts]), a.accumulate);
         return;
     }
     long long P = 0;
-    for (int b = 0; b < batch; b++) P += num_voxels[b];
+    for (int b = 0; b < a.batch; b++) P += a.num_voxels[b];
     const double M = (double)P * (double)max_points;
     double w[F];
     for (int k = 0; k < F; k++) w[k] = (double)weight[c * F + k];
@@ -732,13 +815,38 @@
         const double Fk = moments[pair_index(k, D - 1, D)];
         double xf = 0.0;
         for (int j = 0; j < F; j++) {
-            const int a = j <= k ? j : k, bb = j <= k ? k : j;
-            xf += w[j] * moments[pair_index(a, bb, D)];
+            const int lo = j <= k ? j : k, hi = j <= k ? k : j;
+            xf += w[j] * moments[pair_index(lo, hi, D)];
         }
         const double xhat_f = invstd * (xf - mean * Fk);
-        const double dw = M > 0.0 ? gi * (tot[k * kOut + c] - dbeta / M * Fk - dgamma / M * xhat_f) : 0.0;
-        grad_weight[c * F + k] = (float)dw;
-    }
+        const double dw = M > 0.0 ? gi * (tot[k * ts] - dbeta / M * Fk - dgamma / M * xhat_f) : 0.0;
+        put_grad(grad_weight + c * F + k, (float)dw, a.accumulate);
+    }
+}
+
+template <int C>
+__global__ __launch_bounds__(64) void pfn_backward_finalize_kernel(const double* __restrict__ tot, PfnTailArgs a) {
+    const int c = threadIdx.x;
+    if (c < kOut) bwd_finalize_channel<C>(tot + c, kOut, c, a);
+}
+
+template <int C>
+__global__ __launch_bounds__((C + 8) * kTailCh * 16) void pfn_backward_tail_kernel(const float* __restrict__ partials, int nblocks,
+                                                                                   PfnTailArgs a) {
+    constexpr int NA = C + 8, KC = NA * kTailCh;
+    __shared__ double part[16][KC];
+    __shared__ double tot[KC];
+    const int t = threadIdx.x, chunk = t / KC, kc = t % KC;
+    const int c0 = (int)blockIdx.x * kTailCh;
+    part[chunk][kc] = bwd_chunk_sum<NA, true>(partials, nblocks, kc / kTailCh, c0 + kc % kTailCh, chunk);
+    __syncthreads();
+    if (t < KC) {
+        double s = 0.0;
+        for (int q = 0; q < 16; q++) s += part[q][t];
+        tot[t] = s;
+    }
+    __syncthreads();
+    if (t < kTailCh) bwd_finalize_channel<C>(tot + t, kTailCh, c0 + t, a);
 }
 
 inline bool cfg_ok(const liso_pillar_cfg* c, int batch) {
@@ -867,12 +975,11 @@
     if (!feat || !pt_off || !num_voxels || !weight || !moments || !partials) return LISO_EINVAL;
     const int rows = batch * cfg->max_voxels;
     const int grid = kPfnGrid;
+    const PfnBnArgs a = {num_voxels, weight, gamma, beta, running_mean, running_var, momentum, eps, batch, cfg->max_points};
 #define LISO_PREP(CC)                                                                                                     \
     do {                                                                                                                  \
         pfn_stats_kernel<CC><<<grid, kPfnThreads, 0, st>>>(feat, pt_off, rows, (double*)partials);                           \
-        pfn_bn_finalize_kernel<CC><<<1, 1024, 0, st>>>((const double*)partials, grid, num_voxels, batch, cfg->max_points,    \
-                                                      weight, gamma, beta, running_mean, running_var, momentum, eps, bn_out, \
-                                                      moments);                                                           \
+        pfn_bn_finalize_kernel<CC><<<1, 1024, 0, st>>>((const double*)partials, grid, a, bn_out, moments);                   \
     } while (0)
     switch (cfg->n_channels) {
         case 3: LISO_PREP(3); break;
@@ -883,9 +990,25 @@
     return check_launch();
 }
 
+int liso_pfn_moments_f64(const float* feat, const int* pt_off, const liso_pillar_cfg* cfg, int batch, double* moments, void* partials,
+                         void* stream) {
+    if (!cfg_ok(cfg, batch) || !feat || !pt_off || !moments || !partials) return LISO_EINVAL;
+    hipStream_t st = (hipStream_t)stream;
+    const int rows = batch * cfg->max_voxels;
+    const int grid = kPfnGrid;
+    switch (cfg->n_channels) {
+        case 3: pfn_stats_kernel<3><<<grid, kPfnThreads, 0, st>>>(feat, pt_off, rows, (double*)partials); break;
+        case 4: pfn_stats_kernel<4><<<grid, kPfnThreads, 0, st>>>(feat, pt_off, rows, (double*)partials); break;
+        default: pfn_stats_kernel<5><<<grid, kPfnThreads, 0, st>>>(feat, pt_off, rows, (double*)partials); break;
+    }
+    pfn_moments_merge_kernel<<<1, 1024, 0, st>>>((const double*)partials, grid, moments);
+    return check_launch();
+}
+
 static int pfn_forward_launch(const float* feat, const int* pt_off, const int* voxel_cell, const liso_pillar_cfg* cfg, int batch,
                               const int* cell_to_voxel, const float* weight, const float* bn_out, void* canvas, int out_bf16,
-                              float* occupancy, int* map_out, int row_base, bool compact, void* stream) {
+                              float* occupancy, int* map_out, int row_base, bool compact, void* stream,
+                              const double* moments = nullptr, const PfnBnArgs* derive = nullptr) {
     if (!cfg_ok(cfg, batch) || !feat || !pt_off || !voxel_cell || !cell_to_voxel || !weight || !bn_out || !canvas || !occupancy)
         return LISO_EINVAL;
     if (out_bf16 != LISO_ELEM_F32 && out_bf16 != LISO_ELEM_BF16 && out_bf16 != LISO_ELEM_F16) return LISO_EINVAL;
@@ -895,10 +1018,13 @@
     const int zero_blocks = (int)((cells + kCellsPerBlock - 1) / kCellsPerBlock);
     const int groups = (rows + kGroup - 1) / kGroup;
     int pfn_blocks = (groups + kPfnThreads / 64 - 1) / (kPfnThreads / 64);
-    if (pfn_blocks > 4096) pfn_blocks = 4096;
+    const int cap_blocks = derive ? 1024 : 4096;
+    if (pfn_blocks > cap_blocks) pfn_blocks = cap_blocks;
     const unsigned grid = (unsigned)(zero_blocks + pfn_blocks);
-#define LISO_FWD_(CC, T, R) pfn_forward_kernel<CC, T, R><<<grid, kPfnThreads, 0, st>>>(feat, pt_off, voxel_cell, rows, cfg->max_points, cells, zero_blocks, cell_to_voxel, weight, bn_out, (T*)canvas, occupancy, map_out, row_base)
-#define LISO_FWD(CC, T) do { if (compact) LISO_FWD_(CC, T, true); else LISO_FWD_(CC, T, false); } while (0)
+    if (derive && (compact || !moments)) return LISO_EINVAL;
+    const PfnBnArgs bn_args = derive ? *derive : PfnBnArgs();
+#define LISO_FWD_(CC, T, R, DV) pfn_forward_kernel<CC, T, R, DV><<<grid, kPfnThreads, 0, st>>>(feat, pt_off, voxel_cell, rows, cfg->max_points, cells, zero_blocks, cell_to_voxel, weight, bn_out, (T*)canvas, occupancy, map_out, row_base, moments, bn_args)
+#define LISO_FWD(CC, T) do { if (compact) LISO_FWD_(CC, T, true, false); else if (derive) LISO_FWD_(CC, T, false, true); else LISO_FWD_(CC, T, false, false); } while (0)
     switch (cfg->n_channels * 3 + out_bf16) {
         case 9: LISO_FWD(3, float); break;
         case 10: LISO_FWD(3, __hip_bfloat16); break;
@@ -922,6 +1048,28 @@
                               0, false, stream);
 }
 
+int liso_pfn_forward_scatter_bn(const float* feat, const int* pt_off, const int* voxel_cell, const liso_pillar_cfg* cfg, int batch,
+                                const int* num_voxels, const int* cell_to_voxel, const double* moments, const float* weight,
+                                const float* gamma, const float* beta, float* running_mean, float* running_var, float momentum,
+                                float eps, int fold, float* bn_out, void* canvas, int out_bf16, float* occupancy, void* stream) {
+    if (!cfg_ok(cfg, batch) || !num_voxels || !moments || !weight || !gamma || !beta || !running_mean || !running_var || !bn_out)
+        return LISO_EINVAL;
+    if (!feat || !pt_off || !voxel_cell || !cell_to_voxel || !canvas || !occupancy) return LISO_EINVAL;
+    if (out_bf16 != LISO_ELEM_F32 && out_bf16 != LISO_ELEM_BF16 && out_bf16 != LISO_ELEM_F16) return LISO_EINVAL;
+    const PfnBnArgs a = {num_voxels, weight, gamma, beta, running_mean, running_var, momentum, eps, batch, cfg->max_points};
+    if (fold)
+        return pfn_forward_launch(feat, pt_off, voxel_cell, cfg, batch, cell_to_voxel, weight, bn_out, canvas, out_bf16, occupancy, nullptr,
+                                  0, false, stream, moments, &a);
+    hipStream_t st = (hipStream_t)stream;
+    switch (cfg->n_channels) {
+        case 3: pfn_bn_derive_kernel<3><<<1, 256, 0, st>>>(moments, a, bn_out); break;
+        case 4: pfn_bn_derive_kernel<4><<<1, 256, 0, st>>>(moments, a, bn_out); break;
+        default: pfn_bn_derive_kernel<5><<<1, 256, 0, st>>>(moments, a, bn_out); break;
+    }
+    return pfn_forward_launch(feat, pt_off, voxel_cell, cfg, batch, cell_to_voxel, weight, bn_out, canvas, out_bf16, occupancy, nullptr, 0,
+                              false, stream);
+}
+
 int liso_pfn_forward_rows(const float* feat, const int* pt_off, const int* voxel_cell, const liso_pillar_cfg* cfg, int batch,
                           const int* cell_to_voxel, const float* weight, const float* bn_out, void* rows, int out_bf16, int row_base,
                           int* cell_to_row, float* occupancy, void* stream) {
@@ -934,6 +1082,14 @@
                       const int* num_voxels, const float* weight, const float* gamma, const float* bn_out,
                       const double* moments, int training, const void* grad_canvas, int grad_bf16, float* grad_weight,
                       float* grad_gamma, float* grad_beta, void* partials, void* stream) {
+    return liso_pfn_backward_tail(feat, pt_off, voxel_cell, cfg, batch, num_voxels, weight, gamma, bn_out, moments, training, grad_canvas,
+                                  grad_bf16, grad_weight, grad_gamma, grad_beta, 0, 0, partials, stream);
+}
+
+int liso_pfn_backward_tail(const float* feat, const int* pt_off, const int* voxel_cell, const liso_pillar_cfg* cfg, int batch,
+                           const int* num_voxels, const float* weight, const float* gamma, const float* bn_out,
+                           const double* moments, int training, const void* grad_canvas, int grad_bf16, float* grad_weight,
+                           float* grad_gamma, float* grad_beta, int merged, int accumulate, void* partials, void* stream) {
     if (!cfg_ok(cfg, batch) || !feat || !pt_off || !voxel_cell || !num_voxels || !weight || !gamma || !bn_out || !grad_canvas ||
         !grad_weight || !grad_gamma || !grad_beta || !partials || (training && !moments))
         return LISO_EINVAL;
@@ -941,17 +1097,24 @@
     hipStream_t st = (hipStream_t)stream;
     const int rows = batch * cfg->max_voxels;
     const int grid = pfn_grid((rows + kGroup - 1) / kGroup);
+    const PfnTailArgs ta = {num_voxels, weight,     gamma, bn_out,          moments,  grad_weight,
+                            grad_gamma, grad_beta, batch, cfg->max_points, training, accumulate ? 1 : 0};
 #define LISO_BWD(CC, T)                                                                                              \
     do {                                                                                                             \
         constexpr int NA_ = CC + 8;                                                                                  \
+        if (merged) {                                                                                                \
+            pfn_backward_kernel<CC, T, true><<<grid, kPfnThreads, 0, st>>>(feat, pt_off, voxel_cell, rows,            \
+                                                                           cfg->max_points, weight, bn_out,         \
+                                                                           (const T*)grad_canvas, (float*)partials); \
+            pfn_backward_tail_kernel<CC><<<kOut / kTailCh, NA_ * kTailCh * 16, 0, st>>>((const float*)partials, grid, ta); \
+            break;                                                                                                   \
+        }                                                                                                            \
         double* tot_ = (double*)((float*)partials + (size_t)kPfnGrid * (11 + 2) * kOut);                             \
         pfn_backward_kernel<CC, T><<<grid, kPfnThreads, 0, st>>>(feat, pt_off, voxel_cell, rows, cfg->max_points,     \
                                                                  weight, bn_out, (const T*)grad_canvas,             \
                                                                  (float*)partials);                                  \
         pfn_backward_reduce_kernel<NA_><<<NA_, 1024, 0, st>>>((const float*)partials, grid, tot_);                    \
-        pfn_backward_finalize_kernel<CC><<<1, 64, 0, st>>>(tot_, num_voxels, batch, cfg->max_points, weight, gamma,   \
-                                                           bn_out, moments, training, grad_weight, grad_gamma,       \
-                                                           grad_beta);                                               \
+        pfn_backward_finalize_kernel<CC><<<1, 64, 0, st>>>(tot_, ta);                                                \
     } while (0)
     switch (cfg->n_channels * 3 + grad_bf16) {
         case 9: LISO_BWD(3, float); break;
diff --git a/liso_amd/networks/pcl_to_feature_grid/pcl_to_feature_grid.py b/liso_amd/networks/pcl_to_feature_grid/pcl_to_feature_grid.py
--- a/liso_amd/networks/pcl_to_feature_grid/pcl_to_feature_grid.py
+++ b/liso_amd/networks/pcl_to_feature_grid/pcl_to_feature_grid.py
@@ -74,6 +74,21 @@
     return pt_off, feat, voxel_cell, num_voxels, cell_to_voxel
 
 
+FOLD_DERIVATION = True
+
+
+def pillar_moments(prep, pcfg, B):
+    pt_off, feat = prep[0], prep[1]
+    lib = L.lib()
+    dev = feat.device
+    with torch.cuda.device(dev):
+        moments = torch.empty(80, dtype=torch.float64, device=dev)
+        partials = torch.empty(lib.liso_pfn_partials_bytes(), dtype=torch.uint8, device=dev)
+        L.check(lib.liso_pfn_moments_f64(L.ptr(feat), L.ptr(pt_off), ctypes.byref(pcfg), B, L.ptr(moments), L.ptr(partials),
+                                         L.stream_ptr()), "pfn_moments")
+    return moments
+
+
 def _pfn_statistics(weight, gamma, beta, running_mean, running_var, points, offsets, pcfg, training, momentum, eps, prep):
     L.require_cuda(points, weight)
     lib = L.lib()
@@ -81,7 +96,7 @@
     B = len(offsets) - 1
     if prep is None:
         prep = pillar_prep(points, offsets, pcfg)
-    pt_off, feat, _, num_voxels, _ = prep
+    pt_off, feat, _, num_voxels, _ = prep = prep[:5]
     weight = weight.contiguous().float()
     with torch.cuda.device(dev):
         bn_out = torch.empty(4 * 64, dtype=torch.float32, device=dev)
@@ -98,13 +113,28 @@
 
     @staticmethod
     def forward(ctx, weight, gamma, beta, running_mean, running_var, points, offsets, pcfg, training, momentum, eps,
-                out_dtype, out=None, prep=None):
+                out_dtype, out=None, prep=None, lean=False):
+        from liso_amd.utils import mfma_conv as MC
+
         code = L.elem_code(out_dtype)
         lib = L.lib()
         dev = points.device
         B = len(offsets) - 1
-        prep, weight, bn_out, moments = _pfn_statistics(weight, gamma, beta, running_mean, running_var, points, offsets, pcfg, training,
-                                                        momentum, eps, prep)
+        lean = bool(lean) and MC.lean_pillar_path()
+        params = (weight, gamma, beta)
+        split_stats = lean and bool(training)
+        if split_stats:
+            L.require_cuda(points, weight)
+            if prep is None:
+                prep = pillar_prep(points, offsets, pcfg)
+            moments = prep[5] if len(prep) > 5 else pillar_moments(prep, pcfg, B)
+            prep = prep[:5]
+            weight = weight.contiguous().float()
+            with torch.cuda.device(dev):
+                bn_out = torch.empty(4 * 64, dtype=torch.float32, device=dev)
+        else:
+            prep, weight, bn_out, moments = _pfn_statistics(weight, gamma, beta, running_mean, running_var, points, offsets, pcfg, training,
+                                                            momentum, eps, prep)
         pt_off, feat, voxel_cell, num_voxels, cell_to_voxel = prep
         with torch.cuda.device(dev):
             st = L.stream_ptr()
@@ -115,13 +145,20 @@
             else:
                 canvas = torch.empty((B, pcfg.gx, pcfg.gy, 64), dtype=out_dtype, device=dev)
                 occupancy = torch.empty((B, 1, pcfg.gx, pcfg.gy), dtype=torch.float32, device=dev)
-            L.check(L.TIMER.launch("pfn_forward_scatter", lambda: lib.liso_pfn_forward_scatter(
-                L.ptr(feat), L.ptr(pt_off), L.ptr(voxel_cell), ctypes.byref(pcfg), B, L.ptr(cell_to_voxel), L.ptr(weight),
-                L.ptr(bn_out), L.ptr(canvas), code, L.ptr(occupancy), st),
+            if split_stats:
+                launch = lambda: lib.liso_pfn_forward_scatter_bn(
+                    L.ptr(feat), L.ptr(pt_off), L.ptr(voxel_cell), ctypes.byref(pcfg), B, L.ptr(num_voxels), L.ptr(cell_to_voxel),
+                    L.ptr(moments), L.ptr(weight), L.ptr(gamma), L.ptr(beta), L.ptr(running_mean), L.ptr(running_var), float(momentum),
+                    float(eps), int(FOLD_DERIVATION), L.ptr(bn_out), L.ptr(canvas), code, L.ptr(occupancy), st)
+            else:
+                launch = lambda: lib.liso_pfn_forward_scatter(
+                    L.ptr(feat), L.ptr(pt_off), L.ptr(voxel_cell), ctypes.byref(pcfg), B, L.ptr(cell_to_voxel), L.ptr(weight),
+                    L.ptr(bn_out), L.ptr(canvas), code, L.ptr(occupancy), st)
+            L.check(L.TIMER.launch("pfn_forward_scatter", launch,
                 units=points.numel() * 4 + canvas.numel() * canvas.element_size() + occupancy.numel() * 4),
                 "pfn_forward_scatter")
         ctx.save_for_backward(feat, pt_off, voxel_cell, num_voxels, weight, gamma, bn_out, moments)
-        ctx.pcfg, ctx.B, ctx.training = pcfg, B, bool(training)
+        ctx.pcfg, ctx.B, ctx.training, ctx.lean, ctx.params = pcfg, B, bool(training), lean, params
         ctx.mark_non_differentiable(occupancy)
         return canvas.permute(0, 3, 1, 2), occupancy
 
@@ -135,16 +172,27 @@
             g = g.float()
         g = g.contiguous()
         F = weight.shape[1]
-        gw = torch.empty((64, F), dtype=torch.float32, device=dev)
-        gg = torch.empty(64, dtype=torch.float32, device=dev)
-        gb = torch.empty(64, dtype=torch.float32, device=dev)
+        direct = False
+        if ctx.lean:
+            from liso_amd.utils import mfma_conv as MC
+
+            targets = [MC._direct_target(p_) for p_ in ctx.params]
+            direct = all(t is not None for t in targets)
+        if direct:
+            gw, gg, gb = targets
+        else:
+            gw = torch.empty((64, F), dtype=torch.float32, device=dev)
+            gg = torch.empty(64, dtype=torch.float32, device=dev)
+            gb = torch.empty(64, dtype=torch.float32, device=dev)
         partials = torch.empty(lib.liso_pfn_partials_bytes(), dtype=torch.uint8, device=dev)
         with torch.cuda.device(dev):
-            L.check(lib.liso_pfn_backward(L.ptr(feat), L.ptr(pt_off), L.ptr(voxel_cell), ctypes.byref(ctx.pcfg), ctx.B,
-                                          L.ptr(num_voxels), L.ptr(weight), L.ptr(gamma), L.ptr(bn_out), L.ptr(moments),
-                                          int(ctx.training), L.ptr(g), L.elem_code(g.dtype), L.ptr(gw), L.ptr(gg),
-                                          L.ptr(gb), L.ptr(partials), L.stream_ptr()), "pfn_backward")
-        return gw, gg, gb, None, None, None, None, None, None, None, None, None, None, None
+            L.check(lib.liso_pfn_backward_tail(L.ptr(feat), L.ptr(pt_off), L.ptr(voxel_cell), ctypes.byref(ctx.pcfg), ctx.B,
+                                               L.ptr(num_voxels), L.ptr(weight), L.ptr(gamma), L.ptr(bn_out), L.ptr(moments),
+                                               int(ctx.training), L.ptr(g), L.elem_code(g.dtype), L.ptr(gw), L.ptr(gg),
+                                               L.ptr(gb), int(ctx.lean), int(direct), L.ptr(partials), L.stream_ptr()), "pfn_backward")
+        if direct:
+            gw = gg = gb = None
+        return gw, gg, gb, None, None, None, None, None, None, None, None, None, None, None, None
 
 
 @torch.no_grad()
@@ -202,6 +250,7 @@
         self.voxel_size, self.pc_range = voxel_size, pc_range
         self.grid = tuple(int(g) for g in cfg.data.img_grid_size)
         self.out_dtype = torch.float32
+        self.lean = False
 
     def _pcfg(self, n_channels):
         c = L.PillarCfg()
@@ -241,8 +290,14 @@
 
     @torch.no_grad()
     def prepare(self, pts):
+        from liso_amd.utils import mfma_conv as MC
+
         cat, offsets = self._cat(pts)
-        return (cat, offsets, pillar_prep(cat, offsets, self._pcfg(cat.shape[1])))
+        pcfg = self._pcfg(cat.shape[1])
+        parts = pillar_prep(cat, offsets, pcfg)
+        if self.lean and MC.lean_pillar_path():
+            parts = (*parts, pillar_moments(parts, pcfg, len(offsets) - 1))
+        return (cat, offsets, parts)
 
     def extract_pts_feat(self, pts, out=None, prep=None, compact=False):
         L.elem_code(self.out_dtype)
@@ -263,7 +318,7 @@
             return canvas, canvas.occupancy
         x, occ = _PillarFeatureScatter.apply(lyr.linear.weight, lyr.norm.weight, lyr.norm.bias, lyr.norm.running_mean,
                                              lyr.norm.running_var, cat, offsets, self._pcfg(C), training,
-                                             lyr.norm.momentum, lyr.norm.eps, self.out_dtype, out, prep)
+                                             lyr.norm.momentum, lyr.norm.eps, self.out_dtype, out, prep, self.lean)
         return x, occ
 
     def forward(self, pcl_t0, img_t0=None, out=None, prep=None, compact=False):
diff --git a/liso_amd/trainer.py b/liso_amd/trainer.py
--- a/liso_amd/trainer.py
+++ b/liso_amd/trainer.py
@@ -184,6 +184,7 @@
                 self._setup_gradient_buckets(2)
         from liso_amd.networks.centerpoint.fused_bn import defer_batch_counters
         self._bn_counters = defer_batch_counters(self.net.model.rpn) + defer_batch_counters(self.net.model.center_head)
+        self.net.model.pfn.lean = device.type == "cuda"
 
     def _setup_gradient_buckets(self, grad_buckets):
         from liso_amd.utils import mfma_conv as MC
@@ -376,7 +377,11 @@
             if self._graph2 is not None:
                 self._graph2.replay()
             if bev.requires_grad:
-                bev.backward(self._static_bev.grad)
+                MC.set_direct_grads(True)
+                try:
+                    bev.backward(self._static_bev.grad)
+                finally:
+                    MC.set_direct_grads(False)
 
         if self.world > 1:
             self._reduce_gradients(rest_of_backward)
diff --git a/liso_amd/utils/mfma_conv.py b/liso_amd/utils/mfma_conv.py
--- a/liso_amd/utils/mfma_conv.py
+++ b/liso_amd/utils/mfma_conv.py
@@ -741,6 +741,19 @@
     global _JOINT_BN_BACKWARD
     prev, _JOINT_BN_BACKWARD = _JOINT_BN_BACKWARD, bool(on)
     return prev
+
+
+_LEAN_PILLAR_PATH = True
+
+
+def set_lean_pillar_path(on):
+    global _LEAN_PILLAR_PATH
+    prev, _LEAN_PILLAR_PATH = _LEAN_PILLAR_PATH, bool(on)
+    return prev
+
+
+def lean_pillar_path():
+    return _LEAN_PILLAR_PATH
 
 
 def bn_group_table(Cs, vec):
```

Result: no change. 1062, median of 6 (+0.5%).
